# ecker-lab/TreeLearn

Hardware: AMD Instinct MI355X
Metric: Mpoints/sec through sparse U-Net fwd (0.1 m voxel, 40x40 m tile) (higher is better)
Workload: dtype bf16; 1 GPU; config2: single 40x40 m tile, voxel 0.1 m, 1890607 points/tile, 7-level 32-ch sparse U-Net fwd (30.1 M params, random init), 1 tile per GPU; points_per_tile=1890607, tiles_in_flight=4

## Files before the change

include/treelearn_hip.h:

```cpp
#ifndef TREELEARN_HIP_H
#define TREELEARN_HIP_H

#include <stdint.h>

#ifdef __cplusplus
extern "C" {
#endif

typedef void* tl_stream_t;

enum {
  TL_OK = 0,
  TL_ERR_ARG = -1,
  TL_ERR_LAUNCH = -2,
  TL_ERR_UNSUPPORTED = -3
};

enum { TL_F32 = 0, TL_BF16 = 1, TL_F16 = 2 };

int tl_version(void);
int tl_set_tuning(const char* key, int64_t value);
const char* tl_error_string(int code);


int tl_voxel_point_coords(const float* xyz, const int64_t* batch_ids, int64_t N, int B, float voxel_size,
                          uint32_t* ws_minmax, int32_t* pcoords, int32_t* maxc, tl_stream_t stream);

#define TL_POINT_COORDS_MAX_PARTS 1024
int tl_voxel_point_coords_one(const float* xyz, const int64_t* batch_ids, int64_t N, float voxel_size, uint32_t* ws, int32_t* pcoords,
                              int32_t* maxc_parts, int* n_parts, tl_stream_t stream);
int tl_bitmap_from_points(const int32_t* pcoords, int64_t N, const int32_t dims[4], uint64_t* bitmap, tl_stream_t stream);

int tl_bitmap_down(const uint64_t* fine, const int32_t fdims[4], const int32_t out_shape[3],
                   uint64_t* coarse, const int32_t cdims[4], tl_stream_t stream);

int64_t tl_scan_ws_words(int64_t nwords);
int tl_bitmap_scan(const uint64_t* bitmap, int64_t nwords, uint32_t* prefix, uint32_t* total, uint32_t* ws, tl_stream_t stream);

int tl_expand_coords(const uint64_t* bitmap, const uint32_t* prefix, const int32_t dims[4], int32_t* coords, tl_stream_t stream);

int tl_point_rank(const int32_t* pcoords, int64_t N, const uint64_t* bitmap, const uint32_t* prefix,
                  const int32_t dims[4], int64_t* v2p, tl_stream_t stream);

int tl_voxel_mean_feats(const float* pf, int C, const int64_t* v2p, int64_t N, int64_t M, int P,
                        int32_t* ws, float* out, tl_stream_t stream);
int tl_voxel_feats(const float* xyz, const float* feats, int F, const int64_t* v2p, int64_t N, int64_t M, int P, int use_coords,
                   int use_feats, int dtype, int32_t* ws, void* out, tl_stream_t stream);


int tl_rulebook_subm(const int32_t* coords, int64_t M, const uint64_t* bitmap, const uint32_t* prefix,
                     const int32_t dims[4], int32_t* nbr, int32_t* compact ,
                     tl_stream_t stream);

int tl_rulebook_down(const int32_t* ccoords, int64_t Mc, const uint64_t* fbitmap, const uint32_t* fprefix,
                     const int32_t fdims[4], int64_t Mf, int32_t* child, int32_t* parent, int32_t* inv, tl_stream_t stream);

int64_t tl_pyramid_ws_words(const int32_t dims0[4], int num_levels, int64_t* level_word_offsets);
int tl_pyramid_build(const int32_t* pcoords, int64_t N, const int32_t dims0[4], const int32_t shape0[3], int num_levels,
                     uint64_t* bitmaps, uint32_t* prefixes, uint32_t* counts, uint32_t* ws, tl_stream_t stream);

typedef struct tl_level {
  int32_t dims[4];
  int64_t n;
  const uint64_t* bitmap;
  const uint32_t* prefix;
  int32_t* coords;
  int32_t* nbr;
  int32_t* compact;
  int32_t* child;
  int32_t* parent;
  int32_t* inv;
  const int32_t* o2n;
  int32_t* inv_packed;
} tl_level;

int tl_rulebooks_build(const tl_level* levels, int num_levels, int32_t* minus_one, int64_t minus_one_words,
                       const int32_t* pcoords, int64_t N, int64_t* v2p, tl_stream_t stream);

#define TL_BLK_HALO_MAX 126
typedef struct tl_blk {
  int32_t* o2n; int32_t* perm; int32_t* coords_new;
  int32_t* unit; int32_t* counter; int32_t* halo; uint32_t* lrb; int32_t* pmask;
  int64_t cap_units;
  int32_t halo_max;
  int32_t reserved;
  int32_t* nn;
} tl_blk;
int64_t tl_blk_ws_words(const int32_t dims[4]);
int tl_blk_build(const uint64_t* bitmap, const uint32_t* prefix, const int32_t dims[4], int64_t n, const tl_blk* out, uint32_t* ws,
                 int phases, tl_stream_t stream);

int tl_rulebook_compact(const int32_t* table, int64_t n, int32_t* compact, tl_stream_t stream);

typedef struct tl_conv_args {
  const void* in;        int64_t in_ld;
  const void* weight;
  const int32_t* table;
  int64_t n_out;         int64_t n_in;
  int32_t K;             int32_t Cin;     int32_t Cout;   int32_t dtype;
  const float* in_scale; const float* in_shift;  int32_t in_relu;  int32_t out_relu;
  const void* residual;  int64_t res_ld;
  const float* out_scale; const float* out_shift;
  void* out;             int64_t out_ld;
  void* out2; int64_t out2_ld; const float* out2_scale; const float* out2_shift; int32_t out2_relu;
  void* out3; int64_t out3_ld; const float* out3_scale; const float* out3_shift; int32_t out3_relu;
  const void* weight_frag;
  int32_t table_one_hot;
  const int32_t* table_compact;
  int32_t in_all_ones;
  int32_t epi_mode;
  double* red_part;
  int32_t* red_nparts;
  const void* bn_x;      int64_t bn_x_ld;
  const float* bn_mean;  const float* bn_rstd;  const float* bn_scale;  const float* bn_shift;  int32_t bn_relu;
  const int32_t* blk_unit; const int32_t* blk_counter; const int32_t* blk_halo; const uint32_t* blk_lrb; const int32_t* blk_pmask;
  const int32_t* table_scatter;
  const void* weight_x3;
} tl_conv_args;

#define TL_EPI_NONE 0
#define TL_EPI_STATS 1
#define TL_EPI_BN_BWD 2
int64_t tl_conv_red_parts(int64_t n_out);

int tl_conv_fwd(const tl_conv_args* args, tl_stream_t stream);
int tl_conv_route(const tl_conv_args* args, char* buf, int cap);

int tl_pack_weight(const float* w_ref, int Cout, int K, int Cin, void* w_packed, int dtype, tl_stream_t stream);
int64_t tl_pack_weight_x3_bytes(int Cout, int K, int Cin);
int tl_pack_weight_x3(const float* w_ref, int Cout, int K, int Cin, void* w_x3, tl_stream_t stream);
int tl_pack_weight_dgrad(const float* w_ref, int Cout, int K, int Cin, int flip, void* w_t, int dtype, tl_stream_t stream);
typedef struct tl_pack_desc {
  const float* src;
  void* dst;
  int32_t Cout, K, Cin, form;
} tl_pack_desc;
int tl_pack_weights_batch(const tl_pack_desc* descs, const int32_t* blocks, int64_t n_blocks, int dtype, tl_stream_t stream);
int tl_pack_weight_frag(const float* w_ref, int Cout, int K, int Cin, void* w_frag, int dtype, tl_stream_t stream);

int64_t tl_conv_wgrad_ws_floats(int64_t n_out, int K, int Cin, int Cout);
int tl_conv_wgrad(const void* x, int64_t x_ld, const void* gout, int64_t g_ld, int dtype, const int32_t* table, int64_t n_out,
                  int64_t n_in, int K, int Cin, int Cout, float* gw, float* ws, tl_stream_t stream);
int tl_conv_wgrad_ref(const void* x, int64_t x_ld, const void* gout, int64_t g_ld, int dtype, const int32_t* table, int64_t n_out,
                      int64_t n_in, int K, int Cin, int Cout, float* gw, float* ws, tl_stream_t stream);

int64_t tl_conv_wgrad_blk_ws_floats(void);
int tl_conv_wgrad_blk(const void* x, int64_t x_ld, const void* gout, int64_t g_ld, int dtype, const int32_t* blk_unit, const int32_t* blk_counter,
                      const int32_t* blk_halo, const uint32_t* blk_lrb, int64_t n, int Cin, int Cout, float* gw, int ref_layout, float* ws,
                      tl_stream_t stream);

int tl_head_mlp(const void* feats, int64_t feats_ld, int dtype, int C, const int64_t* v2p, int64_t N,
                const float* pro_scale, const float* pro_shift,
                const float* w1, const float* b1, const float* w2, const float* b2,
                float* backbone, float* logits, float* offsets, tl_stream_t stream);

int tl_affine_relu(const void* in, int64_t in_ld, void* out, int64_t out_ld, int64_t n, int C, int dtype,
                   const float* scale, const float* shift, int relu, tl_stream_t stream);

int64_t tl_bn_ws_doubles(int64_t n, int C);
int tl_bn_train_stats(const void* x, int64_t ld, int64_t n, int C, int dtype, const float* gamma, const float* beta, float eps,
                      float momentum, double* ws, float* mean, float* rstd, float* scale, float* shift, float* running_mean,
                      float* running_var, int64_t* num_batches_tracked, tl_stream_t stream);
int tl_bn_train_bwd(const void* x, int64_t ld, int x_dtype, const void* dy, int64_t dld, int dy_dtype, int64_t n, int C,
                    const float* mean, const float* rstd, const float* scale, const float* shift, int relu, double* ws,
                    float* dgamma, float* dbeta, void* dx, int64_t xld, const void* dx_add, int64_t dx_add_ld, tl_stream_t stream);

int tl_bn_train_finish(const double* part, int64_t nparts, int64_t n, int C, const float* gamma, const float* beta, float eps, float momentum, float* mean,
                       float* rstd, float* scale, float* shift, float* running_mean, float* running_var, int64_t* num_batches_tracked, tl_stream_t stream);
int tl_bn_train_bwd_from_parts(const void* x, int64_t ld, int x_dtype, const void* g, int64_t gld, int g_dtype, int64_t n, int C, const float* mean,
                               const float* rstd, const float* scale, const float* shift, const double* part, int64_t nparts, float* dgamma, float* dbeta,
                               void* dx, int64_t xld, const void* dx_add, int64_t dx_add_ld, tl_stream_t stream);

int tl_linear_small_f32(const void* x, int64_t x_ld, int dtype, const void* w, int Cin, int Cout, int64_t n, float* out, int64_t out_ld,
                        tl_stream_t stream);

int tl_gather_rows(const void* in, int64_t in_ld, int dtype, int C, int64_t n_rows, const int64_t* idx, int64_t N, void* out, int64_t out_ld, tl_stream_t stream);
int tl_scatter_add_rows(const void* g, int64_t g_ld, int dtype, int C, const int64_t* order, const int64_t* sorted_idx, int64_t N, int64_t n_rows, void* gin,
                        int64_t gin_ld, tl_stream_t stream);

// ... 289 lines not shown
```

treelearn_amd/_hip.py:

```python
import ctypes
import os

import torch

_HERE = os.path.dirname(os.path.abspath(__file__))
LIB_PATH = os.path.join(_HERE, "lib", "libtreelearn_hip.so")

TL_F32, TL_BF16, TL_F16 = 0, 1, 2
TL_OK, TL_ERR_ARG, TL_ERR_UNSUPPORTED = 0, -1, -3
TL_EPI_NONE, TL_EPI_STATS, TL_EPI_BN_BWD = 0, 1, 2
_c = ctypes
_vp, _i64, _i32, _f32 = _c.c_void_p, _c.c_int64, _c.c_int32, _c.c_float


class ConvArgs(_c.Structure):
    _fields_ = [
        ("in_", _vp), ("in_ld", _i64), ("weight", _vp), ("table", _vp),
        ("n_out", _i64), ("n_in", _i64), ("K", _i32), ("Cin", _i32), ("Cout", _i32), ("dtype", _i32),
        ("in_scale", _vp), ("in_shift", _vp), ("in_relu", _i32), ("out_relu", _i32),
        ("residual", _vp), ("res_ld", _i64), ("out_scale", _vp), ("out_shift", _vp),
        ("out", _vp), ("out_ld", _i64),
        ("out2", _vp), ("out2_ld", _i64), ("out2_scale", _vp), ("out2_shift", _vp), ("out2_relu", _i32),
        ("out3", _vp), ("out3_ld", _i64), ("out3_scale", _vp), ("out3_shift", _vp), ("out3_relu", _i32),
        ("weight_frag", _vp), ("table_one_hot", _i32), ("table_compact", _vp),
# ... 63 lines not shown


class StemParams(_c.Structure):
    _fields_ = [(k, _c.c_double) for k in ("first_height", "step", "thickness", "corridor", "start_radius", "search_factor", "search_margin",
                                           "max_rmse", "min_radius", "max_radius", "max_growth", "dbh_height")] + \
               [(k, _i64) for k in ("max_slices", "min_points", "max_misses")]


class CrownParams(_c.Structure):
    _fields_ = [(k, _c.c_double) for k in ("layer", "cell", "min_height")] + [(k, _i64) for k in ("max_layers", "base_percent", "max_gap")]


class SkeletonParams(_c.Structure):
    _fields_ = [(k, _c.c_double) for k in ("voxel", "min_branch", "min_height")] + \
               [(k, _i64) for k in ("reach", "base_reach", "base_layers", "level", "max_voxels")]


class WoodParams(_c.Structure):
    _fields_ = [(k, _c.c_double) for k in ("max_rmse", "min_radius", "max_radius", "max_growth", "dbh_height")] + [("min_points", _i64)]


class LeafwoodParams(_c.Structure):
    _fields_ = [(k, _c.c_double) for k in ("radius", "linearity_min", "planarity_min", "verticality_min", "voxel")] + \
               [(k, _i64) for k in ("min_neighbours", "vote_iters", "vote_percent", "reach", "min_component", "filter")]


_I4 = _i32 * 4
_I3 = _i32 * 3

PROTOTYPES = {
    "tl_version": (_i32, []),
    "tl_error_string": (_c.c_char_p, [_i32]),
    "tl_set_tuning": (_i32, [_c.c_char_p, _i64]),
    "tl_voxel_point_coords": (_i32, [_vp, _vp, _i64, _i32, _f32, _vp, _vp, _vp, _vp]),
    "tl_voxel_point_coords_one": (_i32, [_vp, _vp, _i64, _f32, _vp, _vp, _vp, _c.POINTER(_i32), _vp]),
    "tl_bitmap_from_points": (_i32, [_vp, _i64, _I4, _vp, _vp]),
    "tl_bitmap_down": (_i32, [_vp, _I4, _I3, _vp, _I4, _vp]),
    "tl_scan_ws_words": (_i64, [_i64]),
    "tl_bitmap_scan": (_i32, [_vp, _i64, _vp, _vp, _vp, _vp]),
    "tl_expand_coords": (_i32, [_vp, _vp, _I4, _vp, _vp]),
    "tl_point_rank": (_i32, [_vp, _i64, _vp, _vp, _I4, _vp, _vp]),
    "tl_voxel_mean_feats": (_i32, [_vp, _i32, _vp, _i64, _i64, _i32, _vp, _vp, _vp]),
    "tl_voxel_feats": (_i32, [_vp, _vp, _i32, _vp, _i64, _i64, _i32, _i32, _i32, _i32, _vp, _vp, _vp]),
    "tl_rulebook_subm": (_i32, [_vp, _i64, _vp, _vp, _I4, _vp, _vp, _vp]),
    "tl_rulebook_down": (_i32, [_vp, _i64, _vp, _vp, _I4, _i64, _vp, _vp, _vp, _vp]),
    "tl_rulebook_compact": (_i32, [_vp, _i64, _vp, _vp]),
    "tl_pyramid_ws_words": (_i64, [_I4, _i32, _c.POINTER(_i64)]),
    "tl_pyramid_build": (_i32, [_vp, _i64, _I4, _I3, _i32, _vp, _vp, _vp, _vp, _vp]),
    "tl_rulebooks_build": (_i32, [_c.POINTER(Level), _i32, _vp, _i64, _vp, _i64, _vp, _vp]),
    "tl_blk_ws_words": (_i64, [_I4]),
    "tl_blk_build": (_i32, [_vp, _vp, _I4, _i64, _c.POINTER(Blk), _vp, _i32, _vp]),
    "tl_conv_fwd": (_i32, [_c.POINTER(ConvArgs), _vp]),
    "tl_conv_route": (_i32, [_c.POINTER(ConvArgs), _c.c_char_p, _i32]),
    "tl_conv_red_parts": (_i64, [_i64]),
    "tl_exec_create": (_vp, []),
    "tl_exec_destroy": (None, [_vp]),
    "tl_forward": (_i32, [_vp, _c.POINTER(NetDesc), _c.POINTER(ForwardArgs), _vp]),
    "tl_exec_check": (_i32, [_vp]),
    "tl_exec_profile": (_i32, [_vp, _i32]),
    "tl_exec_profile_read": (_i32, [_vp, _c.POINTER(LaunchRec), _i32]),
    "tl_bn_train_finish": (_i32, [_vp, _i64, _i64, _i32, _vp, _vp, _f32, _f32, _vp, _vp, _vp, _vp, _vp, _vp, _vp, _vp]),
    "tl_bn_train_bwd_from_parts": (_i32, [_vp, _i64, _i32, _vp, _i64, _i32, _i64, _i32, _vp, _vp, _vp, _vp, _vp, _i64, _vp, _vp, _vp, _i64, _vp, _i64, _vp]),
    "tl_pack_weight": (_i32, [_vp, _i32, _i32, _i32, _vp, _i32, _vp]),
    "tl_pack_weight_x3": (_i32, [_vp, _i32, _i32, _i32, _vp, _vp]),
    "tl_pack_weight_x3_bytes": (_i64, [_i32, _i32, _i32]),
    "tl_pack_weight_frag": (_i32, [_vp, _i32, _i32, _i32, _vp, _i32, _vp]),
    "tl_pack_weights_batch": (_i32, [_vp, _vp, _i64, _i32, _vp]),
    "tl_pack_weight_dgrad": (_i32, [_vp, _i32, _i32, _i32, _i32, _vp, _i32, _vp]),
    "tl_conv_wgrad_ws_floats": (_i64, [_i64, _i32, _i32, _i32]),
    "tl_conv_wgrad": (_i32, [_vp, _i64, _vp, _i64, _i32, _vp, _i64, _i64, _i32, _i32, _i32, _vp, _vp, _vp]),
    "tl_conv_wgrad_ref": (_i32, [_vp, _i64, _vp, _i64, _i32, _vp, _i64, _i64, _i32, _i32, _i32, _vp, _vp, _vp]),
    "tl_conv_wgrad_blk_ws_floats": (_i64, []),
    "tl_conv_wgrad_blk": (_i32, [_vp, _i64, _vp, _i64, _i32, _vp, _vp, _vp, _vp, _i64, _i32, _i32, _vp, _i32, _vp, _vp]),
    "tl_head_mlp": (_i32, [_vp, _i64, _i32, _i32, _vp, _i64, _vp, _vp, _vp, _vp, _vp, _vp, _vp, _vp, _vp, _vp]),
    "tl_affine_relu": (_i32, [_vp, _i64, _vp, _i64, _i64, _i32, _i32, _vp, _vp, _i32, _vp]),
    "tl_bn_ws_doubles": (_i64, [_i64, _i32]),
    "tl_bn_train_stats": (_i32, [_vp, _i64, _i64, _i32, _i32, _vp, _vp, _f32, _f32, _vp, _vp, _vp, _vp, _vp, _vp, _vp, _vp, _vp]),
    "tl_bn_train_bwd": (_i32, [_vp, _i64, _i32, _vp, _i64, _i32, _i64, _i32, _vp, _vp, _vp, _vp, _i32, _vp, _vp, _vp, _vp, _i64, _vp, _i64, _vp]),
    "tl_linear_small_f32": (_i32, [_vp, _i64, _i32, _vp, _i32, _i32, _i64, _vp, _i64, _vp]),
    "tl_gather_rows": (_i32, [_vp, _i64, _i32, _i32, _i64, _vp, _i64, _vp, _i64, _vp]),
    "tl_scatter_add_rows": (_i32, [_vp, _i64, _i32, _i32, _vp, _vp, _i64, _i64, _vp, _i64, _vp]),
    "tl_compact_ws_words": (_i64, [_i64]),
    "tl_compact_rows": (_i32, [_vp, _i32, _vp, _i64, _vp, _vp, _vp, _vp]),
    "tl_tile_crop_ws_words": (_i64, [_i64]),
    "tl_tile_crop": (_i32, [_vp, _vp, _vp, _i64, _i32, _vp, _vp, _vp, _vp, _vp, _vp, _vp, _vp, _vp, _vp]),
    "tl_cell_keys": (_i32, [_vp, _i64, _c.c_double, _c.c_double, _vp, _i32, _vp, _vp, _vp]),
    "tl_downsample_ws_words": (_i64, [_i64]),
    "tl_downsample_reduce": (_i32, [_vp, _vp, _vp, _i64, _vp, _vp, _vp, _vp, _vp, _vp]),
    "tl_downsample_reduce_r64": (_i32, [_vp, _vp, _vp, _i64, _vp, _vp, _vp, _vp, _vp, _vp]),
    "tl_group_mean": (_i32, [_vp, _i64, _i32, _vp, _vp, _vp, _vp, _vp, _vp, _vp]),
    "tl_verticality": (_i32, [_vp, _vp, _i64, _c.c_double, _vp, _vp, _vp]),
    "tl_eigen_features": (_i32, [_vp, _vp, _i64, _c.c_double, _vp, _vp, _i64, _vp, _i32, _vp, _vp]),
    "tl_eigen_features_scales": (_i32, [_vp, _vp, _i64, _vp, _i32, _vp, _vp, _i64, _vp, _i32, _vp, _vp]),
    "tl_cluster_ws_bytes": (_i64, [_i64]),
    "tl_cluster_grid": (_i32, [_vp, _i64, _c.c_double, _vp, _vp, _vp, _vp]),
    "tl_hdbscan_ws_bytes": (_i64, [_i64]),
    "tl_hdbscan_mst": (_i32, [_vp, _i64, _i32, _vp, _vp, _vp, _vp, _vp, _vp]),
    "tl_hdbscan_labels_host": (_i32, [_vp, _vp, _vp, _i64, _i32, _vp]),
    "tl_hdbscan_prim_order_host": (_i32, [_vp, _vp, _vp, _i64, _vp, _vp, _vp]),
    "tl_hdbscan_grid_plan_ws_bytes": (_i64, []),
    "tl_hdbscan_grid_plan": (_i32, [_vp, _i64, _vp, _vp, _vp]),
    "tl_hdbscan_grid_ws_bytes": (_i64, [_i64, _vp]),
    "tl_hdbscan_grid_ws_bytes_k": (_i64, [_i64, _vp, _i32]),
    "tl_hdbscan_mst_grid": (_i32, [_vp, _i64, _i32, _vp, _vp, _vp, _vp, _vp, _vp, _vp]),
    "tl_knn_vote": (_i32, [_vp, _vp, _i64, _vp, _i64, _i32, _vp, _vp]),
    "tl_knn_vote_grid": (_i32, [_vp, _vp, _vp, _i64, _vp, _vp, _i64, _c.c_float * 3, _f32, _I3, _vp, _i64, _i32, _vp, _vp]),
# ... 129 lines not shown
```

treelearn_amd/csrc/tl_blk.hip:

```cpp
#include "tl_common.h"

namespace {

constexpr int kBlock = 256;
constexpr int HASH = 2048;
constexpr uint32_t EMPTY = 0xFFFFFFFFu;
constexpr uint32_t KEYMASK = 0x01FFFFFFu;
constexpr int LIST = 128;

struct BlkGrid { int B, BX, BY, BZ, TX, TY; int64_t nblk; };

__device__ __forceinline__ void blk_decode(const BlkGrid& g, int64_t blk, int& b, int& bx, int& by, int& bz) {
  bz = (int)(blk % g.BZ); blk /= g.BZ;
  const int iy = (int)(blk & 3), ix = (int)((blk >> 2) & 3); blk >>= 4;
  const int ty = (int)(blk % g.TY); blk /= g.TY;
  const int tx = (int)(blk % g.TX);
  b = (int)(blk / g.TX);
  bx = tx * 4 + ix; by = ty * 4 + iy;
}

__device__ __forceinline__ uint32_t wg_exclusive_scan(uint32_t v, uint32_t* total) {
  __shared__ uint32_t wsum[kBlock / 64];
  const int lane = threadIdx.x & 63, wid = threadIdx.x >> 6;
  uint32_t inc = v;
// ... 59 lines not shown
  __syncthreads();
  uint32_t base = 0, tot = 0;
  for (int w = 0; w < 16; ++w) { if (w < wid) base += wsum[w]; tot += wsum[w]; }
  uint32_t run = base + inc - s;
  for (int64_t i = lo; i < hi; ++i) { const uint32_t v = in[i]; out[i] = run; run += v; }
  if (tid == 0 && total) *total = tot;
}

__global__ void __launch_bounds__(kBlock) k_blk_order(const uint64_t* __restrict__ bm, const uint32_t* __restrict__ pf, TlDims d, BlkGrid g,
                                                      const uint32_t* __restrict__ cnt, const uint32_t* __restrict__ bstart,
                                                      int32_t* __restrict__ o2n, int32_t* __restrict__ perm, int32_t* __restrict__ coords_new,
                                                      uint32_t* __restrict__ cs) {
  const int lane = threadIdx.x & 63;
  const int64_t blk = (int64_t)blockIdx.x * (kBlock / 64) + (threadIdx.x >> 6);
  if (blk >= g.nblk) return;
  if (cnt[blk] == 0) return;
  int b, bx, by, bz;
  blk_decode(g, blk, b, bx, by, bz);
  const int x = bx * 8 + (lane >> 3), y = by * 8 + (lane & 7);
  const bool valid = x < d.X && y < d.Y;
  const int sh = (bz & 7) * 8;
  uint64_t word = 0; int64_t w = 0;
  if (valid) { w = tl_col_word(d, b, x, y) + (bz >> 3); word = bm[w]; }
  uint32_t byte = (uint32_t)(word >> sh) & 0xFFu;
  const uint32_t pc = __popc(byte);
  uint32_t inc = pc;
  for (int off = 1; off < 64; off <<= 1) {
    const uint32_t t = (uint32_t)__shfl_up((int)inc, off);
    if (lane >= off) inc += t;
  }
  if (!pc) return;
  int newr = (int)(bstart[blk] + inc - pc);
  int old = (int)(pf[w] + __popcll(word & ((1ull << sh) - 1ull)));
  cs[(((int64_t)b * d.X + x) * d.Y + y) * g.BZ + bz] = (uint32_t)newr;
  while (byte) {
    const int zb = __ffs((int)byte) - 1;
    byte &= byte - 1;
    o2n[old] = newr; perm[newr] = old;
    reinterpret_cast<int4*>(coords_new)[newr] = make_int4(b, x, y, bz * 8 + zb);
    ++old; ++newr;
  }
}

struct BlkOut {
  const uint32_t* cs; int BZ;
  const int32_t* coords_new;
  int32_t* unit; int32_t* counter;
  int32_t* halo; uint32_t* lrb; int32_t* pmask; int32_t* nn_out;
  int64_t n; int64_t nchunks; int64_t cap_units; int halo_max;
};

__global__ void __launch_bounds__(kBlock) k_blk_units(const uint64_t* __restrict__ bm, TlDims d, BlkOut p) {
  __shared__ uint32_t s_tab[kBlock / 64][HASH + 64];
  __shared__ uint32_t s_list[kBlock / 64][LIST];
  __shared__ uint32_t s_lslot[kBlock / 64][LIST];
  const int lane = threadIdx.x & 63, wv = threadIdx.x >> 6;
  const int64_t chunk = (int64_t)blockIdx.x * (kBlock / 64) + wv;
  if (chunk >= p.nchunks) return;
  uint32_t* tab = s_tab[wv];
  uint32_t* list = s_list[wv];
  uint32_t* lslot = s_lslot[wv];
  const int64_t base = chunk * 64;
  const int cnt = (int)(p.n - base < 64 ? p.n - base : 64);
  const int64_t r = base + lane;
  const bool rvalid = lane < cnt;

  int nn[27];
#pragma unroll
  for (int k = 0; k < 27; ++k) nn[k] = -1;
  uint32_t pm = 0;
  {
    const int4 c = rvalid ? reinterpret_cast<const int4*>(p.coords_new)[r] : make_int4(0, 0, 0, 0);
    const int z = c.w;
    const bool hz0 = z > 0, hz2 = z + 1 < d.Z;
    const int bA = (hz0 ? z - 1 : z) >> 3, bB = (hz2 ? z + 1 : z) >> 3;
    const bool x0 = hz0 && ((z - 1) >> 6) != (z >> 6), x2 = hz2 && ((z + 1) >> 6) != (z >> 6);
    const int64_t wc0 = rvalid ? tl_col_word(d, c.x, c.y, c.z) : 0;
    const int64_t ci0 = rvalid ? (((int64_t)c.x * d.X + c.y) * d.Y + c.z) * p.BZ : 0;
    const bool xin[3] = {rvalid && c.y > 0, rvalid, rvalid && c.y + 1 < d.X}, yin[3] = {c.z > 0, true, c.z + 1 < d.Y};
    const int zw1 = rvalid ? (z >> 6) : 0, zw0 = (rvalid && x0) ? ((z - 1) >> 6) : zw1, zw2 = (rvalid && x2) ? ((z + 1) >> 6) : zw1;
    bool inb[9];
    uint64_t w1[9];
#pragma unroll
    for (int q = 0; q < 9; ++q) {
      const int dx = q / 3 - 1, dy = q % 3 - 1;
      inb[q] = xin[q / 3] && yin[q % 3];
      w1[q] = bm[wc0 + (inb[q] ? (dx * d.Y + dy) * d.Zw : 0) + zw1];
    }
    uint32_t by3[9];
#pragma unroll
    for (int q = 0; q < 9; ++q) {
      const uint32_t b1 = (uint32_t)(w1[q] >> (z & 56)) & 0xFFu;
      const uint32_t b0 = (uint32_t)(w1[q] >> ((hz0 ? z - 1 : z) & 56)) & 0xFFu, b2 = (uint32_t)(w1[q] >> ((hz2 ? z + 1 : z) & 56)) & 0xFFu;
      by3[q] = b0 | (b1 << 8) | (b2 << 16);
    }
    if (__any(x0 || x2)) {
#pragma unroll
      for (int q = 0; q < 9; ++q) {
        const int dx = q / 3 - 1, dy = q % 3 - 1;
        const int64_t wcq = wc0 + (inb[q] ? (dx * d.Y + dy) * d.Zw : 0);
        const uint64_t a0 = bm[wcq + zw0], a2 = bm[wcq + zw2];
        if (x0) by3[q] = (by3[q] & ~0xFFu) | ((uint32_t)(a0 >> ((z - 1) & 56)) & 0xFFu);
        if (x2) by3[q] = (by3[q] & ~0xFF0000u) | (((uint32_t)(a2 >> ((z + 1) & 56)) & 0xFFu) << 16);
      }
    }
    bool p0[9], p1[9], p2[9];
    uint32_t sA[9], sB[9];
#pragma unroll
    for (int q = 0; q < 9; ++q) {
      const int dx = q / 3 - 1, dy = q % 3 - 1;
      p0[q] = inb[q] && hz0 && ((by3[q] >> ((z - 1) & 7)) & 1u);
      p1[q] = inb[q] && ((by3[q] >> (8 + (z & 7))) & 1u);
      p2[q] = inb[q] && hz2 && ((by3[q] >> (16 + ((z + 1) & 7))) & 1u);
      const bool any = p0[q] || p1[q] || p2[q];
      const int64_t ciq = ci0 + (inb[q] ? (dx * d.Y + dy) * p.BZ : 0);
      sA[q] = p.cs[any ? ciq + bA : 0];
      sB[q] = p.cs[(any && bB != bA) ? ciq + bB : 0];
    }
    auto rowid = [](uint32_t byte, int zz, uint32_t start) __attribute__((always_inline)) {
      return (int)(start + __popc(byte & ((1u << (zz & 7)) - 1u)));
    };
#pragma unroll
    for (int q = 0; q < 9; ++q) {
      const uint32_t b_ = bB != bA ? sB[q] : sA[q];
      if (p0[q]) { nn[3 * q] = rowid(by3[q] & 0xFFu, z - 1, sA[q]); pm |= 1u << (3 * q); }
      if (p1[q]) { nn[3 * q + 1] = rowid((by3[q] >> 8) & 0xFFu, z, (z >> 3) == bA ? sA[q] : b_); pm |= 2u << (3 * q); }
      if (p2[q]) { nn[3 * q + 2] = rowid((by3[q] >> 16) & 0xFFu, z + 1, b_); pm |= 4u << (3 * q); }
    }
    if (rvalid) {
      p.pmask[r] = (int32_t)pm;
      if (p.nn_out) {
#pragma unroll
        for (int k = 0; k < 27; ++k) p.nn_out[(int64_t)k * p.n + r] = nn[k];
      }
    }
  }

  int nref = __popc(pm);
  for (int off = 32; off > 0; off >>= 1) nref += __shfl_xor(nref, off);
  const int TS = nref <= 360 ? 512 : (nref <= 720 ? 1024 : HASH);
  const int tshift = nref <= 360 ? 23 : (nref <= 720 ? 22 : 21);
  auto hs = [&](int v) __attribute__((always_inline)) { return ((uint32_t)v * 2654435761u) >> tshift; };

  int st_a[8], st_e[8];
  int sp = 1;
  st_a[0] = 0; st_e[0] = cnt;
  bool first = true;
  while (sp > 0) {
    --sp;
    const int a = st_a[sp], e = st_e[sp];
    const int lo = (int)base + a, hi = (int)base + e;
    for (int i = lane; i < TS; i += 64) tab[i] = EMPTY;
    __builtin_amdgcn_fence(__ATOMIC_ACQ_REL, "workgroup");
    const bool inr = lane >= a && lane < e;
    uint32_t outm = 0;
#pragma unroll
    for (int k = 0; k < 27; ++k) {
      const int v = nn[k];
      const bool out = inr && v >= 0 && (v < lo || v >= hi);
      outm |= out ? (1u << k) : 0u;
      tab[out ? hs(v) : (uint32_t)TS] = (uint32_t)v;
    }
    __builtin_amdgcn_fence(__ATOMIC_ACQ_REL, "workgroup");
    uint32_t lost = 0;
#pragma unroll
    for (int k = 0; k < 27; ++k) {
      const uint32_t cur = tab[hs(nn[k])];
      lost |= (((outm >> k) & 1u) && cur != (uint32_t)nn[k]) ? (1u << k) : 0u;
    }
    if (__any(lost != 0)) {
#pragma unroll
      for (int k = 0; k < 27; ++k) {
        bool todo = (lost >> k) & 1u;
        if (__any(todo)) {
          uint32_t s_ = hs(nn[k]);
          while (__any(todo)) {
            if (todo) {
              s_ = (s_ + 1) & (uint32_t)(TS - 1);
              if (tab[s_] == EMPTY) tab[s_] = (uint32_t)nn[k];
            }
            __builtin_amdgcn_fence(__ATOMIC_ACQ_REL, "workgroup");
            if (todo && tab[s_] == (uint32_t)nn[k]) todo = false;
            __builtin_amdgcn_fence(__ATOMIC_ACQ_REL, "workgroup");
          }
        }
      }
    }
    int H = 0;
    for (int i0 = 0; i0 < TS; i0 += 512) {
      uint32_t sv[8];
#pragma unroll
      for (int q = 0; q < 8; ++q) sv[q] = tab[i0 + q * 64 + lane];
#pragma unroll
      for (int q = 0; q < 8; ++q) {
        const unsigned long long m = __ballot(sv[q] != EMPTY);
        if (sv[q] != EMPTY) {
          const int at = H + __popcll(m & ((1ull << lane) - 1ull));
          if (at < LIST) { list[at] = sv[q]; lslot[at] = (uint32_t)(i0 + q * 64 + lane); }
        }
        H += __popcll(m);
      }
    }
    if (H > p.halo_max && e - a > 1) {
      const int mid = a + (e - a) / 2;
      st_a[sp] = mid; st_e[sp] = e; ++sp;
      st_a[sp] = a; st_e[sp] = mid; ++sp;
      continue;
    }
    int u;
    if (first) u = (int)chunk;
    else {
      int t = 0;
      if (lane == 0) t = atomicAdd(p.counter, 1);
      u = __shfl(t, 0);
    }
    first = false;
    if (u >= p.cap_units || H > LIST - 2) {
      if (lane == 0) atomicMax(p.counter + 1, 1);
      continue;
    }
    __builtin_amdgcn_fence(__ATOMIC_ACQ_REL, "workgroup");
    {
      const uint32_t k0 = lane < H ? list[lane] : EMPTY, s0 = lane < H ? lslot[lane] : (uint32_t)TS;
      int r0 = 0;
      const int H16 = (H + 15) & ~15;
      if (H <= 64) {
        for (int i = 0; i < H; ++i) r0 += (uint32_t)__builtin_amdgcn_readlane((int)k0, i) < k0 ? 1 : 0;
        if (lane < H) p.halo[(int64_t)lo * 32 + r0] = (int32_t)k0;
        tab[s0] = k0 | ((uint32_t)r0 << 25);
        if (lane >= H && lane < H16) p.halo[(int64_t)lo * 32 + lane] = -1;
      } else {
        const uint32_t k1 = lane + 64 < H ? list[lane + 64] : EMPTY, s1 = lane + 64 < H ? lslot[lane + 64] : (uint32_t)TS;
        int r1 = 0;
        for (int i = 0; i < 64; ++i) {
          const uint32_t b = (uint32_t)__builtin_amdgcn_readlane((int)k0, i);
          r0 += b < k0 ? 1 : 0; r1 += b < k1 ? 1 : 0;
        }
        for (int i = 64; i < H; ++i) {
          const uint32_t b = (uint32_t)__builtin_amdgcn_readlane((int)k1, i - 64);
          r0 += b < k0 ? 1 : 0; r1 += b < k1 ? 1 : 0;
        }
        p.halo[(int64_t)lo * 32 + r0] = (int32_t)k0;
        tab[s0] = k0 | ((uint32_t)r0 << 25);
        if (lane + 64 < H) p.halo[(int64_t)lo * 32 + r1] = (int32_t)k1;
        tab[s1] = k1 | ((uint32_t)r1 << 25);
        if (lane + 64 >= H && lane + 64 < H16) p.halo[(int64_t)lo * 32 + lane + 64] = -1;
      }
    }
    __builtin_amdgcn_fence(__ATOMIC_ACQ_REL, "workgroup");
    {
      uint32_t wds[9];
#pragma unroll
      for (int q = 0; q < 9; ++q) wds[q] = 0;
      uint32_t miss = 0;
      uint32_t cur[27];
#pragma unroll
      for (int k = 0; k < 27; ++k) cur[k] = tab[hs(nn[k])];
#pragma unroll
      for (int k = 0; k < 27; ++k) miss |= (((outm >> k) & 1u) && (cur[k] & KEYMASK) != (uint32_t)nn[k]) ? (1u << k) : 0u;
      if (__any(miss != 0)) {
#pragma unroll
        for (int k = 0; k < 27; ++k) {
          bool todo = (miss >> k) & 1u;
          if (__any(todo)) {
            uint32_t s_ = hs(nn[k]);
            while (__any(todo)) {
              if (todo) {
                s_ = (s_ + 1) & (uint32_t)(TS - 1);
                const uint32_t c_ = tab[s_];
                if ((c_ & KEYMASK) == (uint32_t)nn[k]) { cur[k] = c_; todo = false; }
              }
            }
          }
        }
      }
#pragma unroll
      for (int k = 0; k < 27; ++k) {
        const int v = nn[k];
        const bool out = (outm >> k) & 1u;
        const int pos = out ? 64 + (int)(cur[k] >> 25) : ((inr && v >= 0) ? v - lo : 191);
        const uint32_t val = (uint32_t)(pos * 4 + ((pos >> 2) & 3));
        wds[k / 3] |= val << ((k % 3) * 10);
      }
      if (inr) {
        uint32_t* dst = p.lrb + r * 9;
#pragma unroll
        for (int q = 0; q < 9; ++q) dst[q] = wds[q];
      }
    }
    if (lane == 0) reinterpret_cast<int4*>(p.unit)[u] = make_int4(lo, e - a, H, 0);
    __builtin_amdgcn_fence(__ATOMIC_ACQ_REL, "workgroup");
  }
}

__global__ void __launch_bounds__(kBlock) k_blk_tail_rank(int32_t* __restrict__ unit, const int32_t* __restrict__ counter, int nchunks, int64_t cap_units) {
  __shared__ int keys[kBlock];
  const int m = counter[0] - nchunks;
  if (m <= 1 || (int64_t)nchunks + 2 * (int64_t)m > cap_units) return;
  const int4* u = reinterpret_cast<const int4*>(unit) + nchunks;
  int4* tmp = reinterpret_cast<int4*>(unit) + (cap_units - m);
  for (int t0 = blockIdx.x * kBlock; t0 < m; t0 += gridDim.x * kBlock) {
    const int t = t0 + threadIdx.x;
    const int4 me = t < m ? u[t] : make_int4(0, 0, 0, 0);
    int rank = 0;
    for (int j0 = 0; j0 < m; j0 += kBlock) {
      keys[threadIdx.x] = j0 + (int)threadIdx.x < m ? u[j0 + threadIdx.x].x : 0x7FFFFFFF;
      __syncthreads();
      const int lim = m - j0 < kBlock ? m - j0 : kBlock;
      for (int j = 0; j < lim; ++j) rank += keys[j] < me.x ? 1 : 0;
      __syncthreads();
    }
    if (t < m) tmp[rank] = me;
  }
}
__global__ void __launch_bounds__(kBlock) k_blk_tail_copy(int32_t* __restrict__ unit, const int32_t* __restrict__ counter, int nchunks, int64_t cap_units) {
  const int m = counter[0] - nchunks;
  if (m <= 1 || (int64_t)nchunks + 2 * (int64_t)m > cap_units) return;
  const int4* tmp = reinterpret_cast<const int4*>(unit) + (cap_units - m);
  for (int t = blockIdx.x * kBlock + threadIdx.x; t < m; t += gridDim.x * kBlock) reinterpret_cast<int4*>(unit)[nchunks + t] = tmp[t];
}

__global__ void k_blk_init(int32_t* counter, int32_t nchunks) {
  if (threadIdx.x == 0) { counter[0] = nchunks; counter[1] = 0; }
}

}

extern "C" {

int64_t tl_blk_ws_words(const int32_t dims[4]) {
  if (!dims) return -1;
  const int64_t nblk = (int64_t)dims[0] * ((dims[1] + 31) / 32) * ((dims[2] + 31) / 32) * 16 * ((dims[3] + 7) / 8);
  const int64_t ncb = (int64_t)dims[0] * dims[1] * dims[2] * ((dims[3] + 7) / 8);
  return 2 * nblk + 2 * ((nblk + 255) / 256) + 8 + ncb;
}

int tl_blk_build(const uint64_t* bitmap, const uint32_t* prefix, const int32_t dims[4], int64_t n, const tl_blk* o, uint32_t* ws,
                 int phases, tl_stream_t stream) {
  if (!bitmap || !prefix || !dims || !o || !ws || n <= 0 || n >= (1 << 25) || !(phases & 3)) return TL_ERR_ARG;
  if (!o->o2n || !o->perm || !o->coords_new || !o->unit || !o->counter || !o->halo || !o->lrb || !o->pmask) return TL_ERR_ARG;
  if (o->halo_max < 26 || o->halo_max > TL_BLK_HALO_MAX || o->cap_units < (n + 63) / 64) return TL_ERR_ARG;
  if (((uintptr_t)o->unit) % 16 || ((uintptr_t)o->coords_new) % 16) return TL_ERR_ARG;
  const TlDims d = tl_dims(dims);
  BlkGrid g;
// ... 30 lines not shown
```

treelearn_amd/csrc/tl_common.h:

```cpp
#pragma once
#include <hip/hip_runtime.h>
#include <stdint.h>
#include <atomic>
#include <typeinfo>
#include "../../include/treelearn_hip.h"

#define TL_CHECK_LAUNCH()                                   \
  do {                                                      \
    if (hipGetLastError() != hipSuccess) return TL_ERR_LAUNCH; \
  } while (0)

static inline hipStream_t tl_s(tl_stream_t s) { return reinterpret_cast<hipStream_t>(s); }

struct TlAttrOnce {
  std::atomic<uint64_t> done[4];
};
static inline bool tl_lds_attr(TlAttrOnce& once, const void* kernel, int bytes) {
  int dev = 0;
  if (hipGetDevice(&dev) != hipSuccess) return false;
  std::atomic<uint64_t>& w = once.done[(dev >> 6) & 3];
  const uint64_t bit = 1ull << (dev & 63);
  if (w.load(std::memory_order_acquire) & bit) return true;
  if (hipFuncSetAttribute(kernel, hipFuncAttributeMaxDynamicSharedMemorySize, bytes) != hipSuccess) return false;
  w.fetch_or(bit, std::memory_order_release);
  return true;
}

struct TlRoute;
extern thread_local TlRoute* tl_route_armed;
template <auto Kernel> struct TlKernelTag {};
int tl_route_record(TlRoute* r, const char* tag, bool f16, dim3 grid, dim3 block, size_t lds);
#ifdef TL_F16_BUILD
constexpr bool kTlF16Build = true;
#else
constexpr bool kTlF16Build = false;
#endif

template <auto Kernel, class... A>
int tl_launch(dim3 grid, dim3 block, size_t lds, hipStream_t s, A... args) {
  if (TlRoute* r = tl_route_armed) return tl_route_record(r, typeid(TlKernelTag<Kernel>).name(), kTlF16Build, grid, block, lds);
  Kernel<<<grid, block, lds, s>>>(args...);
  return hipGetLastError() == hipSuccess ? TL_OK : TL_ERR_LAUNCH;
}
template <auto Kernel, class... A>
int tl_launch_lds(dim3 grid, dim3 block, size_t lds, hipStream_t s, A... args) {
  if (TlRoute* r = tl_route_armed) return tl_route_record(r, typeid(TlKernelTag<Kernel>).name(), kTlF16Build, grid, block, lds);
  static TlAttrOnce attr_once;
  if (!tl_lds_attr(attr_once, reinterpret_cast<const void*>(Kernel), 160 * 1024)) return TL_ERR_LAUNCH;
  Kernel<<<grid, block, lds, s>>>(args...);
  return hipGetLastError() == hipSuccess ? TL_OK : TL_ERR_LAUNCH;
}

static inline int64_t tl_cdiv(int64_t a, int64_t b) { return (a + b - 1) / b; }

static inline unsigned tl_grid(int64_t work_items, int block) {
  int64_t g = tl_cdiv(work_items, block);
  if (g < 1) g = 1;
  if (g > 256 * 16) g = 256 * 16;
  return (unsigned)g;
}

struct TlDims {
  int B, X, Y, Z, Zw;
};
static inline TlDims tl_dims(const int32_t d[4]) {
  TlDims r{d[0], d[1], d[2], d[3], (d[3] + 63) >> 6};
  return r;
}
__host__ __device__ static inline int64_t tl_nwords(const TlDims& d) { return (int64_t)d.B * d.X * d.Y * d.Zw; }

__device__ __forceinline__ int64_t tl_col_word(const TlDims& d, int b, int x, int y) {
  return (((int64_t)b * d.X + x) * d.Y + y) * d.Zw;
}

__device__ __forceinline__ int tl_rank_at(const uint64_t* __restrict__ bm, const uint32_t* __restrict__ pf,
                                          int64_t wc, int z) {
  const int64_t w = wc + (z >> 6);
  const uint64_t word = bm[w];
  const uint64_t bit = 1ull << (z & 63);
  if (!(word & bit)) return -1;
  return (int)(pf[w] + __popcll(word & (bit - 1)));
}

bool tl_conv_one_hot_direct_enabled(int64_t n_out);
// ... 1 lines not shown
```

treelearn_amd/csrc/tl_conv.hip:

```cpp
#include "tl_conv_internal.h"
#include <cxxabi.h>
#include <stdio.h>
#include <stdlib.h>
#include <string.h>

struct TlRoute {
  char text[1024] = "";
  int len = 0;
  bool truncated = false;
};
thread_local TlRoute* tl_route_armed = nullptr;

int tl_route_record(TlRoute* r, const char* tag, bool f16, dim3 grid, dim3 block, size_t lds) {
  int status = 0;
  char* full = abi::__cxa_demangle(tag, nullptr, nullptr, &status);
  struct Free { char* p; ~Free() { free(p); } } guard{full};
  const char* b = (status == 0 && full) ? strstr(full, "&(") : nullptr;
  b = b ? b + 2 : tag;
  const char* e = b;
  for (int depth = 0; *e; ++e) {
    if (!strncmp(e, "(anonymous namespace)", 21)) { e += 20; continue; }
    if (depth == 0 && (*e == ' ' || *e == ':')) b = e + 1;
    if (depth == 0 && *e == '(') break;
    depth += (*e == '<') - (*e == '>');
    if (depth == 0 && *e == '>') { ++e; break; }
  }
  char dims[2][40];
  const dim3 d[2] = {grid, block};
  for (int i = 0; i < 2; ++i) {
    if (d[i].y == 1 && d[i].z == 1) snprintf(dims[i], sizeof dims[i], "%u", d[i].x);
    else snprintf(dims[i], sizeof dims[i], "(%u, %u, %u)", d[i].x, d[i].y, d[i].z);
  }
  const int room = (int)sizeof r->text - r->len;
  const int n = snprintf(r->text + r->len, (size_t)room, "%s%.*s%s<<<%s, %s, %zu>>>", r->len ? " + " : "", (int)(e - b), b, f16 ? "/f16" : "", dims[0], dims[1], lds);
  if (n < 0 || n >= room) { r->truncated = true; r->text[r->len] = 0; return TL_OK; }
  r->len += n;
  return TL_OK;
}

static int64_t g_small_rows = 16384;
extern int g_small_mode;
extern int g_wgrad_dense;
extern int64_t g_wgrad_dense_min_rows;
extern int g_wgrad_rows;
extern int g_wgrad_dma;
static int g_stream = 1;
static int g_streamq = 1;
static int g_streamq_x3 = 1;
static int g_direct = 1;
static int g_direct_oh = 1;
static int g_blk = 1;
static int g_up = 1;

bool tl_conv_one_hot_direct_enabled(int64_t n_out) { return g_direct && g_direct_oh && n_out > g_small_rows; }

namespace {

struct ConvAlign {
  bool in16, in8;
  bool w16, w4;
  bool in_ld8, in_ld4;
  bool out_vec;
  bool in_aff16;
  bool out_aff16, out_aff4;
  bool res_ld8, res_ld4;
  bool vec_ok() const { return in_ld8 && in16 && w16; }
  bool aligned() const { return in_ld4 && in16 && w16 && in_aff16; }
};

bool ptr_al(const void* p, unsigned bytes) { return ((uintptr_t)p) % bytes == 0; }

ConvAlign conv_align(const tl_conv_args* a) {
  ConvAlign c;
  c.in16 = ptr_al(a->in, 16); c.in8 = ptr_al(a->in, 8);
  c.w16 = ptr_al(a->weight, 16); c.w4 = ptr_al(a->weight, 4);
  c.in_ld8 = a->in_ld % 8 == 0; c.in_ld4 = a->in_ld % 4 == 0;
  c.out_vec = a->out_ld % 8 == 0 && ptr_al(a->out, 16) && (!a->out2 || (a->out2_ld % 8 == 0 && ptr_al(a->out2, 16))) && (!a->out3 || (a->out3_ld % 8 == 0 && ptr_al(a->out3, 16)));
  c.in_aff16 = !a->in_scale || (ptr_al(a->in_scale, 16) && ptr_al(a->in_shift, 16));
  c.out_aff16 = !a->out_scale || (ptr_al(a->out_scale, 16) && ptr_al(a->out_shift, 16));
  c.out_aff4 = !a->out_scale || (ptr_al(a->out_scale, 4) && ptr_al(a->out_shift, 4));
  c.res_ld8 = !a->residual || (a->res_ld % 8 == 0 && ptr_al(a->residual, 16));
  c.res_ld4 = !a->residual || (a->res_ld % 4 == 0 && ptr_al(a->residual, 16));
  return c;
}

struct Conv {
  const tl_conv_args* a;
  ConvP p;
  ConvAlign al;
  const TlConvH16* L;
  int dt;
  bool f16, train, has_blk;
  hipStream_t s;
  bool mult32() const { return a->Cin % 32 == 0 && a->Cout % 32 == 0; }
  bool no_prologue() const { return !a->in_scale && !a->in_relu; }
};

constexpr int TL_NEXT = 1;
int or_next(int rc) { return rc == TL_ERR_UNSUPPORTED ? TL_NEXT : rc; }

int validate(const tl_conv_args* a, bool has_blk) {
  if (!a->table && a->K != 1 && !has_blk && !(a->in_all_ones && a->blk_pmask)) return TL_ERR_ARG;
  if ((a->in_scale == nullptr) != (a->in_shift == nullptr)) return TL_ERR_ARG;
  if ((a->out_scale == nullptr) != (a->out_shift == nullptr)) return TL_ERR_ARG;
  if (a->dtype != TL_F32 && a->dtype != TL_BF16 && a->dtype != TL_F16) return TL_ERR_ARG;
  if ((a->out2_scale == nullptr) != (a->out2_shift == nullptr) || (a->out3_scale == nullptr) != (a->out3_shift == nullptr)) return TL_ERR_ARG;
  if (a->epi_mode != TL_EPI_NONE) {
    if ((a->epi_mode != TL_EPI_STATS && a->epi_mode != TL_EPI_BN_BWD) || !a->red_part || ((uintptr_t)a->red_part) % 8) return TL_ERR_ARG;
    if (a->epi_mode == TL_EPI_BN_BWD) {
      if (!a->bn_x || !a->bn_mean || !a->bn_rstd || !a->bn_scale || !a->bn_shift) return TL_ERR_ARG;
      if (a->bn_x_ld % 8 || !ptr_al(a->bn_x, 16) || !ptr_al(a->bn_mean, 16) || !ptr_al(a->bn_rstd, 16) || !ptr_al(a->bn_scale, 16) || !ptr_al(a->bn_shift, 16)) return TL_ERR_UNSUPPORTED;
    }
  }
  return TL_OK;
}

ConvP fill_convp(const tl_conv_args* a, bool has_blk) {
  ConvP p;
  p.in = a->in; p.in_ld = a->in_ld; p.w = a->weight; p.w_frag = a->weight_frag;
  p.w_x3 = (a->dtype == TL_F32 && a->Cin % 32 == 0 && ptr_al(a->weight_x3, 16)) ? a->weight_x3 : nullptr;
  p.table = a->table; p.ctab = (a->K == 27) ? a->table_compact : nullptr; p.n_out = a->n_out; p.n_in = a->n_in;
  p.K = a->K; p.Cin = a->Cin; p.Cout = a->Cout; p.in_scale = a->in_scale; p.in_shift = a->in_shift;
  p.in_relu = a->in_relu; p.out_relu = a->out_relu; p.res = a->residual; p.res_ld = a->res_ld;
  p.out_scale = a->out_scale; p.out_shift = a->out_shift; p.out = a->out; p.out_ld = a->out_ld;
  p.out2 = a->out2; p.out2_ld = a->out2_ld; p.out2_scale = a->out2_scale; p.out2_shift = a->out2_shift; p.out2_relu = a->out2_relu;
  p.out3 = a->out3; p.out3_ld = a->out3_ld; p.out3_scale = a->out3_scale; p.out3_shift = a->out3_shift; p.out3_relu = a->out3_relu;
  p.nblk = (int)tl_cdiv(a->n_out, TL_CONV_TILE_ROWS);
  p.one_hot = a->table != nullptr ? a->table_one_hot : 0;
  p.blk_unit = has_blk ? a->blk_unit : nullptr; p.blk_counter = a->blk_counter; p.blk_halo = a->blk_halo; p.blk_lrb = a->blk_lrb;
  p.blk_pmask = a->K == 27 ? a->blk_pmask : nullptr;
  p.epi_mode = a->epi_mode; p.red_part = a->red_part; p.red_nparts = a->red_nparts; p.bn_x = a->bn_x; p.bn_x_ld = a->bn_x_ld;
  p.bn_mean = a->bn_mean; p.bn_rstd = a->bn_rstd; p.bn_scale = a->bn_scale; p.bn_shift = a->bn_shift; p.bn_relu = a->bn_relu;
  return p;
}

int rung_packed_one_hot(Conv& c) {
  if (c.p.one_hot != 2) return TL_NEXT;
  const tl_conv_args* a = c.a;
  const bool shape = a->K == 8 && a->Cin == 64 && a->Cout == 32 && !c.train && c.no_prologue() && g_direct && g_direct_oh;
  if (!shape || !(c.dt == TL_BF16 || (c.dt == TL_F32 && c.p.w_x3))) return TL_ERR_UNSUPPORTED;
  return c.L->direct(c.p, c.dt, c.s);
}

int rung_ones27(Conv& c) {
  const tl_conv_args* a = c.a;
  if (!(a->in_all_ones && !c.train && c.al.out_vec && (g_direct || !a->table) && c.al.w4 && !a->residual)) return TL_NEXT;
  return or_next(c.L->ones27(c.p, c.dt, c.s));
}

int rung_blk(Conv& c) {
  const tl_conv_args* a = c.a;
  if (!(c.has_blk && c.dt == TL_BF16 && g_blk && c.al.vec_ok() && c.al.out_vec && c.al.res_ld8 && c.al.out_aff4 && (!a->in_relu || a->in_scale))) return TL_NEXT;
  return or_next(c.L->blk(c.p, c.s));
}

int rung_blk_x3(Conv& c) {
  if (!(c.has_blk && c.a->dtype == TL_F32 && c.p.w_x3 && g_blk && !c.train)) return TL_NEXT;
  return or_next(tl_launch_conv_blk_x3(c.p, c.s));
}

int rung_needs_table(Conv& c) { return (!c.a->table && c.a->K != 1) ? TL_ERR_UNSUPPORTED : TL_NEXT; }

int rung_up(Conv& c) {
  const tl_conv_args* a = c.a;
  if (!(a->table_scatter && c.p.one_hot && g_up && !c.train && c.dt == TL_BF16 && c.al.vec_ok() && c.al.out_vec && c.al.out_aff16)) return TL_NEXT;
  return or_next(c.L->up(c.p, a->table_scatter, c.s));
}

int rung_in4(Conv& c) {
  const tl_conv_args* a = c.a;
  if (!(c.dt == TL_BF16 && a->Cin == 4 && a->Cout == 32 && g_direct && c.al.out_vec && c.al.in8 && c.al.w16 && c.al.res_ld8)) return TL_NEXT;
  return or_next(c.L->direct(c.p, TL_BF16, c.s));
}

int rung_tinycin(Conv& c) {
  const tl_conv_args* a = c.a;
  if (!(!c.train && a->Cin <= 8 && a->Cout % 8 == 0 && a->Cout <= 64 && c.no_prologue() && c.al.out_vec)) return TL_NEXT;
  return c.L->tinycin(c.p, c.dt, c.s);
}

int rung_small(Conv& c) {
  if (!c.train && c.al.vec_ok() && c.a->n_out <= g_small_rows && c.mult32()) return c.L->small(c.p, c.dt, c.s);
  if (c.train && c.a->n_out <= g_small_rows) return TL_ERR_UNSUPPORTED;
  return TL_NEXT;
}

int rung_wide_x3_split(Conv& c) {
  const tl_conv_args* a = c.a;
  if (!(c.p.w_x3 && a->Cin >= 256)) return TL_NEXT;
  const ConvP p = c.p;
  c.p.w_x3 = nullptr;
  if (!(c.dt == TL_F32 && !c.train && g_stream && c.al.aligned() && c.al.out_vec && a->Cin % 64 == 0 && a->Cout % 32 == 0 && c.no_prologue() && !a->residual &&
        !a->out2 && !a->out3 && a->n_out > g_small_rows && c.al.out_aff16))
    return TL_NEXT;
  ConvP p1 = p;
  p1.Cin = a->Cin / 2; p1.out_scale = nullptr; p1.out_shift = nullptr; p1.out_relu = 0;
  const int rc1 = c.L->stream(p1, TL_F32, c.s);
  if (rc1 != TL_OK) return or_next(rc1);
  ConvP p2 = p;
  p2.Cin = a->Cin / 2; p2.in = static_cast<const float*>(a->in) + a->Cin / 2;
  p2.w_x3 = static_cast<const char*>(p.w_x3) + (size_t)a->K * a->Cout * (a->Cin / 2) * 4;
  p2.res = a->out; p2.res_ld = a->out_ld;
  return c.L->stream(p2, TL_F32, c.s);
}

bool f32_vec(const Conv& c) { return c.dt == TL_F32 && c.al.aligned() && c.al.out_vec && c.mult32() && c.no_prologue() && c.al.res_ld4 && c.al.out_aff16; }
int rung_f32_direct(Conv& c) { return f32_vec(c) && g_direct ? or_next(c.L->direct(c.p, TL_F32, c.s)) : TL_NEXT; }
int rung_f32_streamq_x3(Conv& c) {
  if (!(f32_vec(c) && g_stream && g_streamq && g_streamq_x3 && c.p.w_x3 && !c.train && c.a->n_out > g_small_rows)) return TL_NEXT;
  return or_next(tl_launch_conv_streamq_x3(c.p, c.s));
}
int rung_f32_stream(Conv& c) { return f32_vec(c) && g_stream ? or_next(c.L->stream(c.p, TL_F32, c.s)) : TL_NEXT; }

int rung_f32_train_ends(Conv& c) { return (c.train && c.dt == TL_F32) ? TL_ERR_UNSUPPORTED : TL_NEXT; }

int rung_f32_small(Conv& c) {
  if (!(c.dt == TL_F32 && c.al.vec_ok() && c.a->n_out <= 4 * g_small_rows && c.mult32() && c.no_prologue())) return TL_NEXT;
  return c.L->small(c.p, c.dt, c.s);
}

int rung_f32_tile(Conv& c) {
  if (!(c.dt == TL_F32 && c.al.aligned() && c.mult32() && c.a->Cout <= 224)) return TL_NEXT;
  return tl_launch_conv_mfma_f32(c.p, c.s);
}

bool h16_vec(const Conv& c) {
  return c.dt == TL_BF16 && c.al.aligned() && c.al.vec_ok() && c.al.out_vec && c.mult32() && c.a->Cout <= 224 && c.al.res_ld8 && c.al.out_aff16;
}
int rung_h16_one_hot_direct(Conv& c) {
  if (!(h16_vec(c) && c.p.one_hot && g_direct && g_direct_oh && c.a->K == 8 && c.a->Cin == 64 && c.a->Cout == 32)) return TL_NEXT;
  return or_next(c.L->direct(c.p, TL_BF16, c.s));
}
int rung_h16_one_hot_stream(Conv& c) {
  return h16_vec(c) && c.p.one_hot && g_stream && c.a->K == 8 ? or_next(c.L->stream(c.p, TL_BF16, c.s)) : TL_NEXT;
}
int rung_h16_direct(Conv& c) { return h16_vec(c) && g_direct ? or_next(c.L->direct(c.p, TL_BF16, c.s)) : TL_NEXT; }
int rung_h16_streamq(Conv& c) { return h16_vec(c) && g_stream && g_streamq ? or_next(c.L->streamq(c.p, c.s)) : TL_NEXT; }
int rung_h16_stream(Conv& c) { return h16_vec(c) && g_stream ? or_next(c.L->stream(c.p, TL_BF16, c.s)) : TL_NEXT; }
int rung_h16_tile(Conv& c) {
  if (!h16_vec(c)) return TL_NEXT;
  return c.train ? TL_ERR_UNSUPPORTED : c.L->bf16(c.p, c.s);
}

int rung_scalar_only(Conv& c) { return (c.train || c.f16) ? TL_ERR_UNSUPPORTED : TL_NEXT; }
int rung_tinycout(Conv& c) { return or_next(tl_launch_conv_tinycout(c.p, c.dt, c.s)); }
int rung_generic(Conv& c) { return tl_launch_conv_generic(c.p, c.dt, c.s); }

constexpr int (*kLadder[])(Conv&) = {
    rung_packed_one_hot, rung_ones27, rung_blk, rung_blk_x3, rung_needs_table, rung_up, rung_in4, rung_tinycin, rung_small, rung_wide_x3_split,
    rung_f32_direct, rung_f32_streamq_x3, rung_f32_stream, rung_f32_train_ends, rung_f32_small, rung_f32_tile,
    rung_h16_one_hot_direct, rung_h16_one_hot_stream, rung_h16_direct, rung_h16_streamq, rung_h16_stream, rung_h16_tile,
    rung_scalar_only, rung_tinycout, rung_generic,
};

}

extern "C" {

int tl_set_tuning(const char* key, int64_t value) {
  if (!key) return TL_ERR_ARG;
  if (!strcmp(key, "direct")) { g_direct = (int)value; return TL_OK; }
  if (!strcmp(key, "blk")) { g_blk = (int)value; return TL_OK; }
  if (!strcmp(key, "up")) { g_up = (int)value; return TL_OK; }
  if (!strcmp(key, "direct_oh")) { g_direct_oh = (int)value; return TL_OK; }
  if (!strcmp(key, "stream")) { g_stream = (int)value; return TL_OK; }
  if (!strcmp(key, "streamq")) { g_streamq = (int)value; return TL_OK; }
  if (!strcmp(key, "streamq_x3")) { if (value != 0 && value != 1) return TL_ERR_ARG; g_streamq_x3 = (int)value; return TL_OK; }
  if (!strcmp(key, "small_rows")) { g_small_rows = value; return TL_OK; }
  if (!strcmp(key, "small_mode")) { g_small_mode = (int)value; return TL_OK; }
  if (!strcmp(key, "wgrad_dense")) { g_wgrad_dense = (int)value; return TL_OK; }
  if (!strcmp(key, "wgrad_rows")) { g_wgrad_rows = (int)value; return TL_OK; }
  if (!strcmp(key, "wgrad_dma")) { g_wgrad_dma = (int)value; return TL_OK; }
  if (!strcmp(key, "wgrad_dense_min_rows")) { g_wgrad_dense_min_rows = value; return TL_OK; }
  return TL_ERR_ARG;
}

int tl_conv_fwd(const tl_conv_args* a, tl_stream_t stream) {
  if (!a || !a->in || !a->weight || !a->out || a->n_out <= 0 || a->K <= 0 || a->K > 27 || a->Cin <= 0 || a->Cout <= 0) return TL_ERR_ARG;
  const bool has_blk = a->blk_unit && a->blk_counter && a->blk_halo && a->blk_lrb && a->K == 27;
  const int bad = validate(a, has_blk);
  if (bad != TL_OK) return bad;
  Conv c;
  c.a = a; c.p = fill_convp(a, has_blk); c.al = conv_align(a); c.has_blk = has_blk; c.s = tl_s(stream);
  c.f16 = a->dtype == TL_F16;
  c.dt = c.f16 ? TL_BF16 : a->dtype;
  c.L = c.f16 ? &kTlConvF16 : &kTlConvBf16;
  c.train = a->epi_mode != TL_EPI_NONE;
  if (c.train && a->red_nparts) *a->red_nparts = 0;
  for (auto rung : kLadder) {
    const int rc = rung(c);
    if (rc != TL_NEXT) return rc;
  }
  return TL_ERR_UNSUPPORTED;
}

int tl_conv_route(const tl_conv_args* a, char* buf, int cap) {
  if (!buf || cap <= 0) return TL_ERR_ARG;
  TlRoute r;
  struct Armed {
    explicit Armed(TlRoute* q) { tl_route_armed = q; }
    ~Armed() { tl_route_armed = nullptr; }
  } armed(&r);
  const int rc = tl_conv_fwd(a, nullptr);
  snprintf(buf, (size_t)cap, "%s", r.text);
  return (r.truncated || r.len >= cap) ? TL_ERR_ARG : rc;
}

int64_t tl_conv_red_parts(int64_t n_out) {
  const int64_t a = tl_cdiv(n_out > 0 ? n_out : 1, 256);
  return a > 2048 ? a : 2048;
}

}
```

treelearn_amd/csrc/tl_conv_blk.hip:

```cpp
#include "tl_conv_internal.h"
#include <atomic>

namespace {

typedef __attribute__((address_space(3))) void* lds_ptr;
static __device__ __forceinline__ u32x4 lds_r128(unsigned a) { u32x4 v; asm volatile("ds_read_b128 %0, %1" : "=v"(v) : "v"(a)); return v; }
#define TL_LGKM(N) asm volatile("s_waitcnt lgkmcnt(%0)" ::"n"(N) : "memory")
#define TL_KEEP(x) asm volatile("" : "+v"(x))
typedef int i32x4 __attribute__((ext_vector_type(4)));
static __device__ __forceinline__ i32x4 s_load4(const void* ptr) { i32x4 v; asm volatile("s_load_dwordx4 %0, %1, 0x0" : "=s"(v) : "s"(ptr)); return v; }
#define TL_SWAIT(d) asm volatile("s_waitcnt lgkmcnt(0)" : "+s"(d) : : "memory")

constexpr int WS_B = 27 * 32 * 64;
constexpr int AFF_B = 4 * 2 * 32 * 4;
constexpr int STAGE_B = 192 * 64;
constexpr int HCH = 8;
struct RbRow { u32x4 a, b; uint32_t c; };
static __device__ __forceinline__ uint32_t rb_word(const RbRow& r, int w) { return w < 4 ? r.a[w] : (w < 8 ? r.b[w - 4] : r.c); }

typedef float f32x2 __attribute__((ext_vector_type(2)));
typedef short s16x2 __attribute__((ext_vector_type(2)));

template <int W, bool RES, int NV, bool TR = false, bool PRO = false>
__global__ void __launch_bounds__(W * 64) k_conv_blk(ConvP p) {
// ... 319 lines not shown
          sc[q] = __uint_as_float(s0[q]); sc[q + 4] = __uint_as_float(s1[q]);
          sh[q] = __uint_as_float(h0[q]); sh[q + 4] = __uint_as_float(h1[q]);
        }
      }
#pragma unroll
      for (int it = 0; it < 4; ++it) {
        float z[8];
#pragma unroll
        for (int q = 0; q < 8; ++q) z[q] = y[it][q];
        if (aff_on[v]) {
#pragma unroll
          for (int q = 0; q < 8; ++q) z[q] = fmaf(z[q], sc[q], sh[q]);
        }
        if (relu_on[v]) {
#pragma unroll
          for (int q = 0; q < 8; ++q) z[q] = fmaxf(z[q], 0.f);
        }
        const u32x4 o = {pack_bf16x2(z[0], z[1]), pack_bf16x2(z[2], z[3]), pack_bf16x2(z[4], z[5]), pack_bf16x2(z[6], z[7])};
        const int rr_ = (lane >> 2) + 16 * it;
        const unsigned off = rr_ < nown ? (unsigned)(row0 + rr_) * o_ldb[v] + (unsigned)((lane & 3) * 16) : 0xFFFFFFFFu;
        __builtin_amdgcn_raw_buffer_store_b128(__builtin_bit_cast(__attribute__((__vector_size__(4 * sizeof(unsigned)))) unsigned, o), ro[v], (int)off, 0, 0);
      }
    }
    }
    dc = d1; d1 = d2; d2 = desc_fin(d3r, u + 3 * nw);
  }
  if constexpr (TR) {
    double* Ds = reinterpret_cast<double*>(smem + WS_B + AFF_B + W * STAGE_B);
    double d0[8], d1_[8];
#pragma unroll
    for (int q = 0; q < 8; ++q) { d0[q] = (double)ts0[q]; d1_[q] = (double)ts1[q]; }
#pragma unroll
    for (int off = 4; off < 64; off <<= 1)
#pragma unroll
      for (int q = 0; q < 8; ++q) { d0[q] += __shfl_xor(d0[q], off, 64); d1_[q] += __shfl_xor(d1_[q], off, 64); }
    if (lane < 4) {
#pragma unroll
      for (int q = 0; q < 8; ++q) { Ds[(wv * 2 + 0) * 32 + lane * 8 + q] = d0[q]; Ds[(wv * 2 + 1) * 32 + lane * 8 + q] = d1_[q]; }
    }
    __syncthreads();
    if (tid < 64) {
      double t = 0.0;
      for (int w = 0; w < W; ++w) t += Ds[(w * 2 + (tid >> 5)) * 32 + (tid & 31)];
      p.red_part[(int64_t)blockIdx.x * 64 + tid] = t;
    }
  }
}

template <int W, bool RES, int NV, bool TR = false, bool PRO = false>
int launch_blk(const ConvP& p, hipStream_t s) {
  constexpr size_t lds = (size_t)WS_B + AFF_B + (size_t)W * STAGE_B + (TR ? (size_t)W * 2 * 32 * 8 : 0);
  static_assert(lds <= 160 * 1024, "LDS budget");
  if (TR && p.red_nparts) *p.red_nparts = 256;
  return tl_launch_lds<k_conv_blk<W, RES, NV, TR, PRO>>(256, W * 64, lds, s, p);
}

}

int TL_H16(tl_launch_conv_blk)(const ConvP& p, hipStream_t s) {
  if (!p.blk_unit || !p.blk_counter || !p.blk_halo || !p.blk_lrb) return TL_ERR_UNSUPPORTED;
  if (p.K != 27 || p.Cin != 32 || p.Cout != 32 || p.n_in != p.n_out) return TL_ERR_UNSUPPORTED;
  const bool pro = p.in_scale || p.in_relu;
  if (p.n_out >= (1 << 25)) return TL_ERR_UNSUPPORTED;
  auto big = [&](int64_t ld) { return (p.n_out - 1) * ld * 2 + 64 >= 0x7FFFFFFFll * 2; };
  if (big(p.in_ld) || big(p.out_ld) || (p.out2 && big(p.out2_ld)) || (p.out3 && big(p.out3_ld)) || (p.res && big(p.res_ld))) return TL_ERR_UNSUPPORTED;
  if (p.out3 && !p.out2) return TL_ERR_UNSUPPORTED;
  if (p.epi_mode != TL_EPI_NONE) {
    if (p.out2 || p.out_scale || p.out_relu || p.out_ld % 8 || ((uintptr_t)p.out) % 16) return TL_ERR_UNSUPPORTED;
    if (pro && p.epi_mode != TL_EPI_STATS) return TL_ERR_UNSUPPORTED;
    return pro ? launch_blk<8, false, 1, true, true>(p, s) : launch_blk<8, false, 1, true>(p, s);
  }
  const int nv = p.out3 ? 3 : p.out2 ? 2 : 1;
  if (pro) {
    if (nv != 1) return TL_ERR_UNSUPPORTED;
    return p.res ? launch_blk<8, true, 1, false, true>(p, s) : launch_blk<8, false, 1, false, true>(p, s);
  }
  if (p.res) {
    switch (nv) {
      case 1: return launch_blk<8, true, 1>(p, s);
      case 2: return launch_blk<8, true, 2>(p, s);
      default: return launch_blk<8, true, 3>(p, s);
    }
  }
  switch (nv) {
    case 1: return launch_blk<8, false, 1>(p, s);
    case 2: return launch_blk<8, false, 2>(p, s);
    default: return launch_blk<8, false, 3>(p, s);
  }
}
```

treelearn_amd/csrc/tl_conv_blk_x3.hip:

```cpp
#include "tl_conv_internal.h"
#include <atomic>

namespace {

typedef __attribute__((address_space(3))) void* lds_ptr;
static __device__ __forceinline__ u32x4 lds_r128(unsigned a) { u32x4 v; asm volatile("ds_read_b128 %0, %1" : "=v"(v) : "v"(a)); return v; }
#define TL_LGKM(N) asm volatile("s_waitcnt lgkmcnt(%0)" ::"n"(N) : "memory")
#define TL_KEEP(x) asm volatile("" : "+v"(x))
typedef int i32x4 __attribute__((ext_vector_type(4)));
typedef uint32_t u32x2 __attribute__((ext_vector_type(2)));
static __device__ __forceinline__ i32x4 s_load4(const void* ptr) { i32x4 v; asm volatile("s_load_dwordx4 %0, %1, 0x0" : "=s"(v) : "s"(ptr)); return v; }
#define TL_SWAIT(d) asm volatile("s_waitcnt lgkmcnt(0)" : "+s"(d) : : "memory")

constexpr int WS_B = 27 * 32 * 64;
constexpr int AFF_B = 4 * 2 * 32 * 4;
constexpr int STAGE_B = 192 * 64;
constexpr int HCH = 8;
struct RbRow { u32x4 a, b; uint32_t c; };
static __device__ __forceinline__ uint32_t rb_word(const RbRow& r, int w) { return w < 4 ? r.a[w] : (w < 8 ? r.b[w - 4] : r.c); }

struct X3P {
  int slice;
  int part;
  int chunk, nchunks;
// ... 264 lines not shown
    }
    if constexpr (RES) {
#pragma unroll
      for (int it = 0; it < 4; ++it) {
        TL_KEEP(rres[it][0]); TL_KEEP(rres[it][1]);
#pragma unroll
        for (int q = 0; q < 4; ++q) { y[it][q] += __uint_as_float(rres[it][0][q]); y[it][q + 4] += __uint_as_float(rres[it][1][q]); }
      }
    }
    stage_unit(d1, hcur);
#pragma unroll
    for (int v = 0; v < NV; ++v) {
      float sc[8], sh[8];
      if (aff_on[v]) {
        const u32x4 s0 = lds_r128(aff_a + (unsigned)(v * 256)), s1 = lds_r128(aff_a + (unsigned)(v * 256 + 16));
        const u32x4 h0 = lds_r128(aff_a + (unsigned)(v * 256 + 128)), h1 = lds_r128(aff_a + (unsigned)(v * 256 + 144));
        TL_LGKM(0);
#pragma unroll
        for (int q = 0; q < 4; ++q) {
          sc[q] = __uint_as_float(s0[q]); sc[q + 4] = __uint_as_float(s1[q]);
          sh[q] = __uint_as_float(h0[q]); sh[q + 4] = __uint_as_float(h1[q]);
        }
      }
#pragma unroll
      for (int it = 0; it < 4; ++it) {
        float z[8];
#pragma unroll
        for (int q = 0; q < 8; ++q) z[q] = y[it][q];
        if (aff_on[v]) {
#pragma unroll
          for (int q = 0; q < 8; ++q) z[q] = fmaf(z[q], sc[q], sh[q]);
        }
        if (relu_on[v]) {
#pragma unroll
          for (int q = 0; q < 8; ++q) z[q] = fmaxf(z[q], 0.f);
        }
        typedef __attribute__((__vector_size__(4 * sizeof(unsigned)))) unsigned uv4;
        const uv4 o0 = {__float_as_uint(z[0]), __float_as_uint(z[1]), __float_as_uint(z[2]), __float_as_uint(z[3])};
        const uv4 o1 = {__float_as_uint(z[4]), __float_as_uint(z[5]), __float_as_uint(z[6]), __float_as_uint(z[7])};
        const int rr_ = (lane >> 2) + 16 * it;
        const unsigned off = rr_ < nown ? (unsigned)(row0 + rr_) * o_ldb[v] + (unsigned)((lane & 3) * 32) : 0xFFFFFFFFu;
        __builtin_amdgcn_raw_buffer_store_b128(o0, ro[v], (int)off, 0, 0);
        __builtin_amdgcn_raw_buffer_store_b128(o1, ro[v], (int)(off == 0xFFFFFFFFu ? off : off + 16u), 0, 0);
      }
    }
    dc = d1; d1 = d2; d2 = desc_fin(d3r, u + 3 * nw);
  }
}

template <int W, bool RES, int NV>
int launch_x3(const ConvP& p, const X3P& xp, hipStream_t s) {
  constexpr size_t lds = (size_t)WS_B + AFF_B + (size_t)W * STAGE_B;
  static_assert(lds <= 160 * 1024, "LDS budget");
  return tl_launch_lds<k_conv_blk_x3<W, RES, NV>>(256, W * 64, lds, s, p, xp);
}

}

int tl_launch_conv_blk_x3(const ConvP& p, hipStream_t s) {
  if (!p.blk_unit || !p.blk_counter || !p.blk_halo || !p.blk_lrb || !p.w_x3) return TL_ERR_UNSUPPORTED;
  if (p.K != 27 || p.Cin != 32 || p.Cout != 32 || p.n_in != p.n_out || p.epi_mode != TL_EPI_NONE || p.out3) return TL_ERR_UNSUPPORTED;
  if (p.n_out >= (1 << 25)) return TL_ERR_UNSUPPORTED;
  if (p.in_relu && !p.in_scale) return TL_ERR_UNSUPPORTED;
  auto big = [&](int64_t ld) { return (p.n_out - 1) * ld * 4 + 128 >= 0x7FFFFFFFll * 2; };
  if (big(p.in_ld) || big(p.out_ld) || (p.out2 && big(p.out2_ld)) || (p.res && big(p.res_ld))) return TL_ERR_UNSUPPORTED;
  auto al16 = [](const void* q, int64_t ld) { return ((uintptr_t)q) % 16 == 0 && ld % 4 == 0; };
  if (!al16(p.in, p.in_ld) || !al16(p.out, p.out_ld) || (p.out2 && !al16(p.out2, p.out2_ld)) || (p.res && !al16(p.res, p.res_ld)) || ((uintptr_t)p.w_x3) % 16) return TL_ERR_UNSUPPORTED;
  ConvP a = p;
  a.res = nullptr; a.res_ld = 0; a.out_scale = a.out_shift = nullptr; a.out_relu = 0; a.out2 = nullptr; a.out2_scale = a.out2_shift = nullptr; a.out2_relu = 0;
  ConvP b = p;
  b.in = static_cast<const float*>(p.in) + 16;
  if (p.in_scale) { b.in_scale = p.in_scale + 16; b.in_shift = p.in_shift + 16; }
  const int rc = launch_x3<8, false, 1>(a, X3P{0, 0, 0, 1}, s);
  if (rc != TL_OK) return rc;
  const X3P xb{1, 1, 0, 1};
  if (p.res) return p.out2 ? launch_x3<8, true, 2>(b, xb, s) : launch_x3<8, true, 1>(b, xb, s);
  return p.out2 ? launch_x3<8, false, 2>(b, xb, s) : launch_x3<8, false, 1>(b, xb, s);
}
```

treelearn_amd/csrc/tl_conv_direct.hip:

```cpp
#include "tl_conv_internal.h"
#include <atomic>

namespace {


template <bool BF16, int K, int NB, int UN, int G, int WAVES, bool CT = false, bool TR = false, bool OH = false, bool X3 = false>
__global__ void __launch_bounds__(WAVES * 64) k_conv_direct(ConvP p, int ntiles, int walk) {
  static_assert(!X3 || (!BF16 && !TR), "the split-bf16 contraction: fp32 rows, inference");
  constexpr int EB = BF16 ? 2 : 4;
  constexpr int UB = 32 * EB;
  constexpr int NJ = UB / 32;
  constexpr int SLOTS = UB / 16;
  constexpr int COUT = NB * 32;
  constexpr int NG = (K + G - 1) / G;
  constexpr int EP = COUT + 4;
  extern __shared__ __attribute__((aligned(16))) char smem[];
  char* Ws = smem;
  float* Es = reinterpret_cast<float*>(smem + (size_t)K * UN * COUT * UB);
  double* Ds = reinterpret_cast<double*>(smem + (size_t)K * UN * COUT * UB + (size_t)WAVES * 32 * EP * 4);

  const int tid = threadIdx.x, lane = tid & 63, wv = tid >> 6;
  const int fi = lane & 31, fh = lane >> 5;
  auto swz_of = [](int n) { return BF16 ? ((n >> 2) & 3) : ((n >> 1) & 7); };

// ... 368 lines not shown
__global__ void __launch_bounds__(256) k_conv_ones27(ConvP p) {
  __shared__ __attribute__((aligned(16))) float S[27][32];
  for (int e = threadIdx.x; e < 27 * 32; e += 256) {
    float t = 0.f;
    if constexpr (BF16) {
      const uint16_t* w = (const uint16_t*)p.w;
      for (int c = 0; c < p.Cin; ++c) t += bf16_lo((uint32_t)w[(int64_t)e * p.Cin + c]);
    } else {
      const float* w = (const float*)p.w;
      for (int c = 0; c < p.Cin; ++c) t += w[(int64_t)e * p.Cin + c];
    }
    S[e >> 5][e & 31] = t;
  }
  __syncthreads();
  const int32_t* mask = p.blk_pmask ? p.blk_pmask : p.ctab + (int64_t)9 * p.n_out;
  const int64_t total = p.n_out * 4;
  for (int64_t t = (int64_t)blockIdx.x * 256 + threadIdx.x; t < total; t += (int64_t)gridDim.x * 256) {
    const int64_t row = t >> 2; const int c0 = (int)(t & 3) * 8;
    uint32_t m = (uint32_t)mask[row];
    float v[8] = {0.f, 0.f, 0.f, 0.f, 0.f, 0.f, 0.f, 0.f};
    while (m) {
      const int k = __builtin_ctz(m); m &= m - 1;
      const f32x4 a = *reinterpret_cast<const f32x4*>(&S[k][c0]), b = *reinterpret_cast<const f32x4*>(&S[k][c0 + 4]);
#pragma unroll
      for (int q = 0; q < 4; ++q) { v[q] += a[q]; v[q + 4] += b[q]; }
    }
    epi_views8<BF16>(p, row, c0, v);
  }
}

template <bool BF16, int K, int NB, int UN, int G, int WAVES, bool CT = false, bool TR = false, bool OH = false, bool X3 = false>
int launch(const ConvP& p_, hipStream_t s) {
  ConvP p = p_;
  if constexpr (X3) {
    if (p.epi_mode != TL_EPI_NONE) return TL_ERR_UNSUPPORTED;
    p.w = p.w_x3;
  }
  if constexpr (!TR && BF16) {
    if (p.epi_mode != TL_EPI_NONE) return launch<BF16, K, NB, UN, G, WAVES, CT, true, OH>(p, s);
  } else if constexpr (!TR) {
    if (p.epi_mode != TL_EPI_NONE) return TL_ERR_UNSUPPORTED;
  }
  if constexpr (TR && NB >= 3) return TL_ERR_UNSUPPORTED;
  else {
  constexpr int UB = BF16 ? 64 : 128;
  const size_t lds = (size_t)K * UN * NB * 32 * UB + (size_t)WAVES * 32 * (NB * 32 + 4) * 4 + (TR ? (size_t)WAVES * 2 * NB * 32 * 8 : 0);
  if (lds > 160 * 1024) return TL_ERR_UNSUPPORTED;
  const int ntiles = (int)tl_cdiv(p.n_out, 32);
  const int per_cu = (int)((160 * 1024) / lds) < 1 ? 1 : (int)((160 * 1024) / lds);
  int grid = 256 * (per_cu > 2 ? 2 : per_cu);
  const int need = (int)tl_cdiv(ntiles, WAVES);
  if (grid > need) grid = need;
  if (p.red_nparts) *p.red_nparts = grid;
  return tl_launch_lds<k_conv_direct<BF16, K, NB, UN, G, WAVES, CT, TR, OH, X3>>(grid, WAVES * 64, lds, s, p, ntiles, 0);
  }
}

template <bool BF16, int K, int G>
int dispatch(const ConvP& p, hipStream_t s) {
  const int nb = p.Cout / 32, un = p.Cin / 32;
  const size_t wbytes = (size_t)K * p.Cout * p.Cin * (BF16 ? 2 : 4);
  if constexpr (BF16 && K == 27) {
    if (p.ctab && nb == 1 && un == 1) return launch<true, 27, 1, 1, G, 16, true>(p, s);
    if (p.ctab && nb == 1 && un == 2) return launch<true, 27, 1, 2, G, 8, true>(p, s);
  }
  if constexpr (BF16 && K == 8) {
    if (p.one_hot && nb == 1 && un == 2) return launch<true, 8, 1, 2, G, 16, false, false, true>(p, s);
  }
  if constexpr (BF16 && K == 1) {
    if (nb == 2 && un == 4) return launch<true, 1, 2, 4, 1, 16>(p, s);
    if (nb == 3 && un == 6) return launch<true, 1, 3, 6, 1, 8>(p, s);
    if (nb == 4 && un == 8) return launch<true, 1, 4, 8, 1, 8>(p, s);
  }
  if constexpr (!BF16 && K == 1) {
    if (nb == 2 && un == 4 && p.epi_mode == TL_EPI_NONE) {
      if (p.w_x3) return launch<false, 1, 2, 4, 1, 8, false, false, false, true>(p, s);
      return launch<false, 1, 2, 4, 1, 8>(p, s);
    }
  }
  if constexpr (!BF16 && K == 8) {
    if (p.one_hot && p.w_x3 && p.epi_mode == TL_EPI_NONE && nb == 1 && un == 2) return launch<false, 8, 1, 2, G, 12, false, false, true, true>(p, s);
  }
#define TL_D(NB_, UN_)                                                                                               \
  if (nb == NB_ && un == UN_) {                                                                                      \
    if constexpr (BF16) return wbytes <= 64 * 1024 ? launch<true, K, NB_, UN_, G, 16>(p, s) : launch<true, K, NB_, UN_, G, 8>(p, s); \
    else {                                                                                                           \
      if (p.w_x3 && p.epi_mode == TL_EPI_NONE)        \
        return launch<false, K, NB_, UN_, (G > 2 ? 2 : G), (K == 27 && NB_ == 1 && UN_ == 1 ? 11 : 8), false, false, false, true>(p, s);         \
      return launch<false, K, NB_, UN_, (G > 2 ? 2 : G), 8>(p, s);                                                   \
    }                                                                                                                \
  }
  TL_D(1, 1) TL_D(1, 2) TL_D(2, 1) TL_D(2, 2) TL_D(2, 3) TL_D(3, 2) TL_D(1, 3) TL_D(3, 1)
#undef TL_D
  return TL_ERR_UNSUPPORTED;
}

}

int TL_H16(tl_launch_conv_ones27)(const ConvP& p, int dtype, hipStream_t s) {
  if (p.K != 27 || p.Cout != 32 || (!p.ctab && !p.blk_pmask) || p.Cin <= 0 || p.Cin > 64 || p.in_scale || p.in_relu || p.epi_mode != TL_EPI_NONE) return TL_ERR_UNSUPPORTED;
  const unsigned g = tl_grid(p.n_out * 4, 256);
  if (dtype == TL_BF16) return tl_launch<k_conv_ones27<true>>(g, 256, 0, s, p);
  return tl_launch<k_conv_ones27<false>>(g, 256, 0, s, p);
}


int TL_H16(tl_launch_conv_direct)(const ConvP& p, int dtype, hipStream_t s) {
  if (p.in_scale || p.in_relu) return TL_ERR_UNSUPPORTED;
  if (p.one_hot == 2 && !(p.K == 8 && p.Cin == 64 && p.Cout == 32 && p.epi_mode == TL_EPI_NONE && (dtype == TL_BF16 || p.w_x3))) return TL_ERR_UNSUPPORTED;
  const int eb = dtype == TL_BF16 ? 2 : 4;
  if (dtype == TL_BF16 && p.Cin == 4 && p.Cout == 32 && p.K <= 28 && p.table && p.in_ld % 4 == 0 && (int64_t)p.n_in * p.in_ld * 2 < 0xFFFF0000ll) {
    const int ntiles = (int)tl_cdiv(p.n_out, 32);
    int grid = (int)tl_cdiv(ntiles, 8);
    if (grid > 2048) grid = 2048;
    if (p.red_nparts) *p.red_nparts = grid;
    const bool ct = p.ctab && p.K == 27;
    if (p.epi_mode != TL_EPI_NONE) return ct ? tl_launch<k_conv_in4<8, true, true>>(grid, 512, 0, s, p, ntiles) : tl_launch<k_conv_in4<8, false, true>>(grid, 512, 0, s, p, ntiles);
    return ct ? tl_launch<k_conv_in4<8, true>>(grid, 512, 0, s, p, ntiles) : tl_launch<k_conv_in4<8>>(grid, 512, 0, s, p, ntiles);
  }
  if (p.Cin % 32 || p.Cout % 32) return TL_ERR_UNSUPPORTED;
  const int64_t ld_b = p.in_ld * eb, in_bytes = (p.n_in - 1) * ld_b + (int64_t)p.Cin * eb;
  if (!(in_bytes > 0 && in_bytes + 2 * ld_b < 0xFFFFFFFFll)) return TL_ERR_UNSUPPORTED;
  if ((size_t)p.K * p.Cout * p.Cin * eb > 112 * 1024) return TL_ERR_UNSUPPORTED;
  if (dtype == TL_BF16) {
    switch (p.K) {
      case 27: return dispatch<true, 27, 3>(p, s);
      case 8: return dispatch<true, 8, 2>(p, s);
      case 1: return dispatch<true, 1, 1>(p, s);
    }
  } else {
    switch (p.K) {
      case 27: return dispatch<false, 27, 3>(p, s);
      case 8: return dispatch<false, 8, 2>(p, s);
      case 1: return dispatch<false, 1, 1>(p, s);
    }
  }
  return TL_ERR_UNSUPPORTED;
}
```

treelearn_amd/csrc/tl_conv_stream.hip:

```cpp
#include "tl_conv_internal.h"
#include <atomic>

namespace {

constexpr int WAVES = 8;
constexpr int NT = WAVES * 64;

template <bool BF16, int K, int NB, int UN, int RB, bool OH, bool X3>
constexpr int stream_epi_ahead() {
  constexpr bool exact_f32 = !BF16 && !X3;
  constexpr bool f32_64_64 = exact_f32 && K == 27 && NB == 2 && UN == 2, f32_192_96 = exact_f32 && K == 27 && NB == 3 && UN == 6;
  constexpr bool f32_96_64_k8 = exact_f32 && K == 8 && NB == 2 && UN == 3;
  constexpr bool x3_128_128 = X3 && K == 27 && NB == 4 && UN == 4, x3_64_96_k8 = X3 && K == 8 && NB == 3 && UN == 2;
  constexpr bool oh_128_96 = BF16 && OH && K == 8 && NB == 3 && UN == 4;
  if (f32_64_64 || f32_192_96 || f32_96_64_k8 || x3_128_128 || x3_64_96_k8 || oh_128_96) return 0;
  if (NB == 3 && RB == 1) return 1;
  return epi_pd<BF16>(RB * NB);
}

template <bool BF16, int K, int NB, int UN, int DA, int RB, int OCC, bool OH = false, bool X3 = false>
__global__ void __launch_bounds__(NT, OCC) k_conv_stream(ConvP p) {
  static_assert(!X3 || !BF16, "the split-bf16 contraction reads fp32 rows");
  constexpr int EB = BF16 ? 2 : 4, UB = 32 * EB, NJ = UB / 32, SLOTS = UB / 16;
  constexpr int COUT = NB * 32, CIN = UN * 32;
// ... 154 lines not shown
          const int slot = c * SLOTS + 2 * j + fh;
          const u32x4 bf = *reinterpret_cast<const u32x4*>(bl + nb * 32 * BROW + slot * 16);
#pragma unroll
          for (int rb = 0; rb < RB; ++rb) {
            if constexpr (OH) {
              const u32x4 z = {0u, 0u, 0u, 0u};
              mma16<BF16>(acc[rb][nb], idx[k][rb] >= 0 ? a1[rb][c][j] : z, bf);
            } else mma16<BF16>(acc[rb][nb], a[k % DA][rb][c][j], bf);
          }
        }
      }
    if constexpr (!OH) { if (k + DA < K) issue_a(k + DA, a[k % DA]); }
    if (k + 1 < K) __syncthreads();
  }

  if constexpr (PD > 0) {
    if (p.epi_mode == TL_EPI_NONE) {
      epi_wave_tail_lds<BF16, WAVES, EP, NB, RB, false, PD>(p, Es, Af, tid, r0, acc);
      return;
    }
  }
  __syncthreads();
  float* ew = Es + wv * 32 * EP;
  float red0[NB], red1[NB];
#pragma unroll
  for (int nb = 0; nb < NB; ++nb) { red0[nb] = 0.f; red1[nb] = 0.f; }
#pragma unroll
  for (int rb = 0; rb < RB; ++rb)
#pragma unroll
    for (int nb = 0; nb < NB; ++nb) {
#pragma unroll
      for (int r = 0; r < 16; ++r) ew[((r & 3) + 8 * (r >> 2) + 4 * fh) * EP + fi] = acc[rb][nb][r];
      __builtin_amdgcn_fence(__ATOMIC_RELEASE, "wavefront");
      __builtin_amdgcn_wave_barrier();
      epi_block32<BF16, EP>(p, ew, lane, r0 + rb * 32, nb * 32, red0[nb], red1[nb]);
      __builtin_amdgcn_fence(__ATOMIC_RELEASE, "wavefront");
      __builtin_amdgcn_wave_barrier();
    }
  if (p.epi_mode != TL_EPI_NONE) epi_finish_wg<WAVES, EP, NB>(p, Es, tid, red0, red1);
}

template <bool BF16, int K, int NB, int UN, int DA, int RB, bool OH = false, bool X3 = false>
int launch(ConvP p, hipStream_t s) {
  if constexpr (X3) p.w = p.w_x3;
  constexpr int EB = BF16 ? 2 : 4;
  constexpr int BPTL = (NB * 32 * UN * (BF16 ? 4 : 8) + NT - 1) / NT;
  constexpr int VG = RB * NB * 16 + DA * RB * UN * (BF16 ? 8 : 16) + (K <= 8 ? 8 : 27) * RB + 4 * BPTL * (DA > 2 ? DA - 1 : 1) + 20;
  constexpr int OCC = (OH && X3) ? 2 : ((VG <= 120 || (X3 && NB * UN <= 4)) ? 4 : 2);
  const size_t wt = 2 * (size_t)NB * 32 * (UN * 32 * EB + 16), ep = (size_t)WAVES * 32 * 36 * 4;
  const size_t lds = (wt > ep ? wt : ep) + (stream_epi_ahead<BF16, K, NB, UN, RB, OH, X3>() > 0 ? 6 * (size_t)NB * 32 * 4 : 0);
  if (lds > 160 * 1024) return TL_ERR_UNSUPPORTED;
  p.nblk = (int)tl_cdiv(p.n_out, WAVES * 32 * RB);
  if (p.red_nparts) *p.red_nparts = p.nblk;
  return tl_launch_lds<k_conv_stream<BF16, K, NB, UN, DA, RB, OCC, OH, X3>>(p.nblk, NT, lds, s, p);
}

template <bool BF16, int K>
int dispatch(const ConvP& p, hipStream_t s) {
  const int nb = p.Cout / 32, un = p.Cin / 32;
  if constexpr (BF16 && K == 8) {
    if (p.one_hot) {
      if (nb == 2 && un == 3) return launch<true, 8, 2, 3, 1, 1, true>(p, s);
      if (nb == 1 && un == 2) return launch<true, 8, 1, 2, 1, 1, true>(p, s);
      if (nb == 3 && un == 4) return launch<true, 8, 3, 4, 1, 1, true>(p, s);
    }
  }
  if constexpr (!BF16 && K == 8) {
    if (p.one_hot == 1 && p.w_x3 && p.epi_mode == TL_EPI_NONE) {
      if (nb == 2 && un == 3) return launch<false, 8, 2, 3, 1, 1, true, true>(p, s);
      if (nb == 3 && un == 4) return launch<false, 8, 3, 4, 1, 1, true, true>(p, s);
    }
  }
  if constexpr (BF16 && K == 8) {
    if (!p.one_hot && nb == 2 && un == 1) return launch<true, 8, 2, 1, 3, 2>(p, s);
  }
#define TL_S(NB_, UN_, DB_, RB_, DF_)                                                                \
  if (nb == NB_ && un == UN_) {                                                                      \
    if constexpr (BF16) return launch<true, K, NB_, UN_, DB_, RB_>(p, s);                            \
    else {                                                                                           \
      if (p.w_x3) return launch<false, K, NB_, UN_, 1, 1, false, true>(p, s);    \
      return launch<false, K, NB_, UN_, DF_, 1>(p, s);                                               \
    }                                                                                                \
  }
  TL_S(2, 2, 3, 1, 2) TL_S(2, 4, 2, 1, 1) TL_S(3, 3, 1, 2, 1) TL_S(3, 6, 1, 1, 1) TL_S(4, 4, 2, 1, 1) TL_S(2, 3, 3, 1, 1) TL_S(3, 2, 3, 1, 2)
  TL_S(3, 4, 2, 1, 1) TL_S(4, 3, 2, 1, 1) TL_S(1, 2, 3, 1, 2) TL_S(2, 1, 3, 1, 2) TL_S(1, 1, 3, 1, 2)
#undef TL_S
  return TL_ERR_UNSUPPORTED;
}

}

int TL_H16(tl_launch_conv_stream)(const ConvP& p, int dtype, hipStream_t s) {
  if (p.in_scale || p.in_relu) return TL_ERR_UNSUPPORTED;
  const int eb = dtype == TL_BF16 ? 2 : 4;
  const int64_t ld_b = p.in_ld * eb, in_bytes = (p.n_in - 1) * ld_b + (int64_t)p.Cin * eb;
  if (!(in_bytes > 0 && in_bytes + 2 * ld_b < 0xFFFFFFFFll)) return TL_ERR_UNSUPPORTED;
  if (dtype == TL_BF16) {
    switch (p.K) {
      case 27: return dispatch<true, 27>(p, s);
      case 8: return dispatch<true, 8>(p, s);
    }
  } else {
    switch (p.K) {
      case 27: return dispatch<false, 27>(p, s);
      case 8: return dispatch<false, 8>(p, s);
    }
// ... 4 lines not shown
```

treelearn_amd/csrc/tl_conv_streamq.hip:

```cpp
#include "tl_conv_internal.h"
#include <atomic>
#include <type_traits>

namespace {

template <int CTRL>
static __device__ __forceinline__ uint32_t qperm(uint32_t v) {
  return (uint32_t)__builtin_amdgcn_mov_dpp((int)v, CTRL, 0xf, 0xf, true);
}

static __device__ __forceinline__ void quad_transpose(const u32x4 (&S)[4], u32x4 (&F)[4], bool o0, bool o1) {
  u32x4 T[4];
#pragma unroll
  for (int i1 = 0; i1 < 2; ++i1)
#pragma unroll
    for (int d = 0; d < 4; ++d) {
      const uint32_t P = S[2 * i1][d], Q = S[2 * i1 + 1][d];
      const uint32_t Pn = qperm<0xB1>(P), Qn = qperm<0xB1>(Q);
      T[2 * i1][d] = o0 ? Qn : P;
      T[2 * i1 + 1][d] = o0 ? Q : Pn;
    }
#pragma unroll
  for (int x0 = 0; x0 < 2; ++x0)
#pragma unroll
// ... 203 lines not shown
    const char* bl = Bs + (k & 1) * COUT * BROW + fi * BROW + fh * 64;
#pragma unroll
    for (int pp = 0; pp < PN; ++pp)
#pragma unroll
      for (int s = 0; s < 4; ++s)
#pragma unroll
        for (int nb = 0; nb < NB; ++nb) {
          const u32x4 bf = *reinterpret_cast<const u32x4*>(bl + nb * 32 * BROW + (pp * 8 + s) * 16);
#pragma unroll
          for (int rb = 0; rb < RB; ++rb) {
            mma16<true>(acc[rb][nb], F[rb][pp][s], bf);
          }
        }
    if (k + DA < KV) { issue_a(k + DA, a[k % DA]); if (k + DA + 1 < KV) read_idx(k + DA + 1); }
    if (k + 1 < KV) __syncthreads();
  }
  }

  if constexpr (PD > 0) {
    if (p.epi_mode == TL_EPI_NONE) {
      epi_wave_tail_lds<!X3, W, EP, NB, RB, true, PD>(p, Es, Af, tid, r0, acc);
      return;
    }
  }
  __syncthreads();
  float* ew = Es + wv * 32 * EP;
  float red0[NB], red1[NB];
#pragma unroll
  for (int nb = 0; nb < NB; ++nb) { red0[nb] = 0.f; red1[nb] = 0.f; }
#pragma unroll
  for (int rb = 0; rb < RB; ++rb)
#pragma unroll
    for (int nb = 0; nb < NB; ++nb) {
#pragma unroll
      for (int r = 0; r < 16; ++r) ew[(2 * (r >> 2) + fh + 8 * (r & 3)) * EP + fi] = acc[rb][nb][r];
      __builtin_amdgcn_fence(__ATOMIC_RELEASE, "wavefront");
      __builtin_amdgcn_wave_barrier();
      epi_block32<!X3, EP>(p, ew, lane, r0 + rb * 32, nb * 32, red0[nb], red1[nb]);
      __builtin_amdgcn_fence(__ATOMIC_RELEASE, "wavefront");
      __builtin_amdgcn_wave_barrier();
    }
  if (p.epi_mode != TL_EPI_NONE) epi_finish_wg<W, EP, NB>(p, Es, tid, red0, red1);
}

template <int K, int NB, int PN, int DA, int W = 8, int RB = 1, int SP = 1, bool X3 = false, bool UL = false>
int launch(ConvP p, hipStream_t s) {
  constexpr int OCC = 2;
  if constexpr (X3) p.w = p.w_x3;
  const size_t wt = 2 * (size_t)NB * 32 * (PN * 128 + 16) + (size_t)W * K * 32 * RB * 4, ep = (size_t)W * 32 * 36 * 4;
  const size_t lds = (wt > ep ? wt : ep) + (streamq_epi_ahead<K, NB, PN, RB, X3>() > 0 ? 6 * (size_t)NB * 32 * 4 : 0);
  if (lds > 160 * 1024) return TL_ERR_UNSUPPORTED;
  p.nblk = (int)tl_cdiv(p.n_out, W * 32 * RB);
  if (p.red_nparts) *p.red_nparts = p.nblk;
  return tl_launch_lds<k_conv_streamq<K, NB, PN, DA, W, RB, OCC, SP, X3, UL>>(p.nblk, W * 64, lds, s, p);
}

}

int TL_H16(tl_launch_conv_streamq)(const ConvP& p, hipStream_t s) {
  if (p.in_scale || p.in_relu || p.Cin % 64 || p.Cout % 32) return TL_ERR_UNSUPPORTED;
  const int64_t ld_b = p.in_ld * 2, in_bytes = (p.n_in - 1) * ld_b + (int64_t)p.Cin * 2;
  if (!(in_bytes > 0 && in_bytes + 2 * ld_b < 0xFFFFFFFFll)) return TL_ERR_UNSUPPORTED;
  const int nb = p.Cout / 32, pn = p.Cin / 64;
  if (p.K == 27) {
    if (nb == 2 && pn == 1) return launch<27, 2, 1, 2>(p, s);
    if (nb == 2 && pn == 2) return launch<27, 2, 2, 2>(p, s);
    if (nb == 4 && pn == 2) return launch<27, 4, 2, 2>(p, s);
    if (nb == 4 && pn == 1) return launch<27, 4, 1, 2>(p, s);
    if (nb == 3 && pn == 3) return launch<27, 3, 3, 2>(p, s);
    if (nb == 4 && pn == 4) return launch<27, 4, 2, 2, 8, 1, 2>(p, s);
  } else if (p.K == 8) {
    if (nb == 3 && pn == 1) return launch<8, 3, 1, 2>(p, s);
  }
  return TL_ERR_UNSUPPORTED;
}

#ifndef TL_F16_BUILD
int tl_launch_conv_streamq_x3(const ConvP& p, hipStream_t s) {
  if (!p.w_x3 || p.in_scale || p.in_relu || p.Cin % 32 || p.Cout % 32 || p.K != 27 || p.epi_mode != TL_EPI_NONE || p.Cin >= 256) return TL_ERR_UNSUPPORTED;
  const int64_t ld_b = p.in_ld * 4, in_bytes = (p.n_in - 1) * ld_b + (int64_t)p.Cin * 4;
  if (!(in_bytes > 0 && in_bytes + 2 * ld_b < 0xFFFFFFFFll) || ((uintptr_t)p.w_x3) % 16) return TL_ERR_UNSUPPORTED;
  const int nb = p.Cout / 32, pn = p.Cin / 32;
  if (nb == 2 && pn == 2) return launch<27, 2, 2, 1, 8, 1, 1, true, true>(p, s);
  if (nb == 2 && pn == 4) return launch<27, 2, 2, 1, 8, 1, 2, true>(p, s);
  if (nb == 3 && pn == 6) return launch<27, 3, 3, 2, 8, 1, 2, true>(p, s);
  return TL_ERR_UNSUPPORTED;
}
#endif
```

treelearn_amd/csrc/tl_exec.hip:

```cpp
#include <string.h>
#include <vector>

#include "tl_common.h"
#include "tl_arena.h"

namespace {

constexpr int64_t kCompactMinRows = 65536;
constexpr int64_t kBlkMinRows = 16384;
constexpr int64_t kBlkMaxRows = (1 << 25) - 64;
constexpr size_t kHostBytes = 64 + (size_t)TL_POINT_COORDS_MAX_PARTS * 16;

struct Ten {
  int64_t off = -1;
  int64_t ld = 0, n = 0;
  int C = 0;
  int64_t own_off = -1, own_bytes = 0;
};

struct ViewReq {
  const Ten* dst = nullptr;
  tl_affine aff{nullptr, nullptr};
  int relu = 0;
};

struct Table {
  const int32_t* table = nullptr;
  const int32_t* compact = nullptr;
  const int32_t* scatter = nullptr;
  bool blk = false;
  int one_hot = 0;
};

struct LevelG {
  int32_t dims[4];
  int64_t n = 0;
  int64_t coords = -1, nbr = -1, ct = -1, child = -1, inv = -1, invp = -1;
};

}

struct tl_exec {
  int32_t* host = nullptr;
  hipEvent_t ev_main = nullptr, ev_side = nullptr, ev_flag = nullptr;
  bool flag_in_flight = false;
  bool profile = false;
  std::vector<hipEvent_t> pev;
  std::vector<tl_launch_rec> recs;
  hipStream_t prof_stream = nullptr;
};

namespace {

struct Run {
  tl_exec* ex;
  const tl_net_desc* net;
  tl_forward_args* a;
  hipStream_t s;
  Arena ar;
  int esize;
  int rc = TL_OK;
  int launches = 0;
  int nl;
  LevelG lv[TL_MAX_LEVELS];
  bool blocked = false;
  int64_t g0 = 0;
  int64_t o_unit = -1, o_counter = -1, o_halo = -1, o_lrb = -1, o_pmask = -1, o_nn = -1;

  const int32_t* gw(int64_t word_off) const { return word_off < 0 ? nullptr : reinterpret_cast<const int32_t*>(ar.at(g0 + 4 * word_off)); }

  Ten alloc(int64_t n, int C) {
    Ten t;
    t.n = n; t.C = C; t.ld = C; t.own_bytes = n * C * esize; t.own_off = t.off = ar.take(t.own_bytes);
    return t;
  }
  void release(Ten& t) {
    if (t.own_off >= 0) ar.give(t.own_off, t.own_bytes);
    t.own_off = -1;
  }
  Ten cols(const Ten& t, int c0, int C) const {
    Ten v;
    v.off = t.off + (int64_t)c0 * esize; v.ld = t.ld; v.n = t.n; v.C = C;
    return v;
  }

  Table subm(int li) const {
    Table t;
    if (li == 0 && blocked) { t.blk = true; return t; }
    t.table = gw(lv[li].nbr); t.compact = gw(lv[li].ct);
    return t;
  }
  Table down(int li) const { Table t; t.table = gw(lv[li].child); return t; }
  Table up(int li) const {
    Table t;
    t.scatter = gw(lv[li].child);
    if (lv[li].invp >= 0) { t.table = gw(lv[li].invp); t.one_hot = 2; }
    else { t.table = gw(lv[li].inv); t.one_hot = 1; }
    return t;
  }

  void conv(int level, int kind, const Ten& x, const tl_weight& w, const Table& tb, int64_t n_out, const ViewReq* views, int nviews, Ten* outs,
            const Ten* residual = nullptr, tl_affine in_aff = {nullptr, nullptr}, int in_relu = 0, int all_ones = 0, int split_part = -1, int split_cin = 0) {
    for (int i = 0; i < nviews; ++i) outs[i] = views[i].dst ? *views[i].dst : alloc(n_out, w.Cout);
    if (rc != TL_OK) return;
    ++launches;
    if (ar.dry) return;
    tl_conv_args c{};
    c.in = ar.at(x.off); c.in_ld = x.ld; c.weight = w.w; c.weight_frag = w.frag; c.weight_x3 = w.x3;
    c.table = tb.table; c.table_compact = tb.compact; c.table_one_hot = tb.one_hot; c.table_scatter = tb.scatter;
    if (tb.blk) {
      c.blk_unit = gw(o_unit); c.blk_counter = gw(o_counter); c.blk_halo = gw(o_halo);
      c.blk_lrb = reinterpret_cast<const uint32_t*>(gw(o_lrb)); c.blk_pmask = gw(o_pmask);
    }
    c.in_all_ones = all_ones;
    c.n_out = n_out; c.n_in = x.n; c.K = w.K; c.Cin = w.Cin; c.Cout = w.Cout; c.dtype = net->dtype;
    c.in_scale = in_aff.scale; c.in_shift = in_aff.shift; c.in_relu = in_relu;
    if (residual) { c.residual = ar.at(residual->off); c.res_ld = residual->ld; }
    c.out = ar.at(outs[0].off); c.out_ld = outs[0].ld; c.out_scale = views[0].aff.scale; c.out_shift = views[0].aff.shift; c.out_relu = views[0].relu;
    if (nviews > 1) { c.out2 = ar.at(outs[1].off); c.out2_ld = outs[1].ld; c.out2_scale = views[1].aff.scale; c.out2_shift = views[1].aff.shift; c.out2_relu = views[1].relu; }
    if (nviews > 2) { c.out3 = ar.at(outs[2].off); c.out3_ld = outs[2].ld; c.out3_scale = views[2].aff.scale; c.out3_shift = views[2].aff.shift; c.out3_relu = views[2].relu; }
    const bool prof = ex->profile;
    if (prof) {
      hipEvent_t e0 = nullptr, e1 = nullptr;
      if (hipEventCreate(&e0) != hipSuccess || hipEventCreate(&e1) != hipSuccess) { rc = TL_ERR_LAUNCH; return; }
      ex->pev.push_back(e0); ex->pev.push_back(e1);
      tl_launch_rec r{};
      r.level = level; r.kind = kind; r.K = w.K; r.Cin = w.Cin; r.Cout = w.Cout; r.residual = residual != nullptr; r.esize = esize;
      r.split_part = split_part; r.split_cin = split_cin; r.in_prologue = in_aff.scale != nullptr || in_relu; r.n_out = n_out; r.n_in = x.n;
      ex->recs.push_back(r);
      if (hipEventRecord(e0, s) != hipSuccess) rc = TL_ERR_LAUNCH;
    }
    const int r = tl_conv_fwd(&c, s);
    if (prof && hipEventRecord(ex->pev.back(), s) != hipSuccess) rc = TL_ERR_LAUNCH;
    if (r != TL_OK) rc = r;
  }

  static ViewReq RAW(const Ten* dst = nullptr) { ViewReq v; v.dst = dst; return v; }
  static ViewReq ACT(const tl_affine& aff, const Ten* dst = nullptr) { ViewReq v; v.dst = dst; v.aff = aff; v.relu = 1; return v; }

  void res_block(int li, const tl_res_desc& b, const Ten& x_raw, const Ten& x_act, const ViewReq* views, int nviews, Ten* outs) {
    const Table nb = subm(li);
    const int64_t n = lv[li].n;
    Ten t, res;
    const ViewReq v1 = ACT(b.bn3);
    conv(li, 0, x_act, b.w1, nb, n, &v1, 1, &t);
    const bool has1x1 = b.w1x1.w != nullptr;
    if (has1x1) { const ViewReq vr = RAW(); conv(li, 3, x_raw, b.w1x1, Table{}, n, &vr, 1, &res); }
    conv(li, 0, t, b.w2, nb, n, views, nviews, outs, has1x1 ? &res : &x_raw);
    release(t);
    if (has1x1) release(res);
  }

  void ublock(int li, Ten x_raw, Ten x_act, const ViewReq* views, int nviews, Ten* outs) {
    const tl_ublock_desc& u = net->u[li];
    const int64_t n = lv[li].n;
    const int C = u.C;
    Ten o2[3];
    { const ViewReq v[2] = {RAW(), ACT(u.blocks[1].bn0)}; res_block(li, u.blocks[0], x_raw, x_act, v, 2, o2); }
    release(x_raw); release(x_act);
    x_raw = o2[0]; x_act = o2[1];
    if (!u.deeper) {
      res_block(li, u.blocks[1], x_raw, x_act, views, nviews, outs);
      release(x_raw); release(x_act);
      return;
    }
    Ten cat_raw = alloc(n, 2 * C), cat_act = alloc(n, 2 * C);
    const Ten cr_l = cols(cat_raw, 0, C), cr_r = cols(cat_raw, C, C), ca_l = cols(cat_act, 0, C), ca_r = cols(cat_act, C, C);
    Ten o3[3];
    { const ViewReq v[3] = {RAW(&cr_l), ACT(u.bn_cat_l, &ca_l), ACT(u.bn_down)}; res_block(li, u.blocks[1], x_raw, x_act, v, 3, o3); }
    release(x_raw); release(x_act);
    Ten xd = o3[2], d[2];
    { const ViewReq v[2] = {RAW(), ACT(net->u[li + 1].blocks[0].bn0)}; conv(li, 1, xd, u.wd, down(li), lv[li + 1].n, v, 2, d); }
    release(xd);
// ... 5 lines not shown
    { const ViewReq v[2] = {RAW(), ACT(u.tail[1].bn0)}; res_block(li, u.tail[0], cat_raw, cat_act, v, 2, y); }
    release(cat_raw); release(cat_act);
    res_block(li, u.tail[1], y[0], y[1], views, nviews, outs);
    release(y[0]); release(y[1]);
  }

  void l1_block(const tl_res_desc& b, const Ten& x, const tl_affine& in_aff, const ViewReq* views, int nviews, Ten* outs) {
    const Table nb = subm(0);
    const int64_t n = lv[0].n;
    Ten t, res;
    const ViewReq v1 = ACT(b.bn3);
    conv(0, 0, x, b.w1, nb, n, &v1, 1, &t, nullptr, in_aff, 1);
    const bool has1x1 = b.w1x1.w != nullptr;
    if (has1x1) { const ViewReq vr = RAW(); conv(0, 3, x, b.w1x1, Table{}, n, &vr, 1, &res); }
    conv(0, 0, t, b.w2, nb, n, views, nviews, outs, has1x1 ? &res : &x);
    release(t);
    if (has1x1) release(res);
  }
  void l1_staged(Ten x_raw, const ViewReq* views, int nviews, Ten* outs) {
    const tl_ublock_desc& u = net->u[0];
    const int64_t n = lv[0].n;
    const int C = u.C;
    const Table nb = subm(0);
    Ten x1;
    { const ViewReq v = RAW(); l1_block(u.blocks[0], x_raw, u.blocks[0].bn0, &v, 1, &x1); }
    release(x_raw);
    Ten cat_raw = alloc(n, 2 * C);
    const Ten cr_l = cols(cat_raw, 0, C), cr_r = cols(cat_raw, C, C);
    Ten o2[2];
    { const ViewReq v[2] = {RAW(&cr_l), ACT(u.bn_down)}; l1_block(u.blocks[1], x1, u.blocks[1].bn0, v, 2, o2); }
    release(x1);
    Ten xd = o2[1], d[2];
    { const ViewReq v[2] = {RAW(), ACT(net->u[1].blocks[0].bn0)}; conv(0, 1, xd, u.wd, down(0), lv[1].n, v, 2, d); }
    release(xd);
    Ten e_act;
    { const ViewReq v = ACT(u.bn_up); ublock(1, d[0], d[1], &v, 1, &e_act); }
    { const ViewReq v = RAW(&cr_r); Ten o; conv(0, 2, e_act, u.wu, up(0), n, &v, 1, &o); }
    release(e_act);
    const tl_res_desc& b = u.tail[0];
    Ten part, t, res, y;
    { const ViewReq v = RAW(); conv(0, 0, cr_l, b.w1_half[0], nb, n, &v, 1, &part, nullptr, u.bn_cat_l, 1, 0, 0, 2 * C); }
    { const ViewReq v = ACT(b.bn3); conv(0, 0, cr_r, b.w1_half[1], nb, n, &v, 1, &t, &part, u.bn_cat_r, 1, 0, 1, 2 * C); }
    release(part);
    { const ViewReq v = RAW(); conv(0, 3, cat_raw, b.w1x1, Table{}, n, &v, 1, &res); }
    { const ViewReq v = RAW(); conv(0, 0, t, b.w2, nb, n, &v, 1, &y, &res); }
    release(t); release(res); release(cat_raw);
    l1_block(u.tail[1], y, u.tail[1].bn0, views, nviews, outs);
    release(y);
  }

  void network() {
    const int64_t n1 = lv[0].n;
    const bool feats = net->use_coords || net->use_feats;
    Ten ones = alloc(n1, net->in_channels);
    if (feats) {
      const int64_t ws_bytes = 4 * n1 * net->max_points_per_voxel, o_ws = ar.take(ws_bytes);
      if (!ar.dry) {
        const int r = tl_voxel_feats(a->xyz, a->point_feats, net->in_channels - 3, reinterpret_cast<const int64_t*>(gw(o_v2p)), a->N, n1, net->max_points_per_voxel,
                                     net->use_coords, net->use_feats, net->dtype, reinterpret_cast<int32_t*>(ar.at(o_ws)), ar.at(ones.off), s);
        if (r != TL_OK) rc = r;
      }
      ar.give(o_ws, ws_bytes);
    } else if (!ar.dry) {
      hipError_t e;
      if (net->dtype == TL_F32) e = hipMemsetD32Async((hipDeviceptr_t)ar.at(ones.off), 0x3F800000, n1 * net->in_channels, s);
      else e = hipMemsetD16Async((hipDeviceptr_t)ar.at(ones.off), net->dtype == TL_BF16 ? 0x3F80 : 0x3C00, n1 * net->in_channels, s);
      if (e != hipSuccess) rc = TL_ERR_LAUNCH;
    }
    Ten xs[2], x;
    const ViewReq out = RAW();
    if (blocked) {
      const ViewReq v = RAW();
      Table tin = subm(0);
      if (feats) { tin = Table{}; tin.table = gw(o_nn); }
      conv(0, 4, ones, net->w_in, tin, n1, &v, 1, xs, nullptr, {nullptr, nullptr}, 0, feats ? 0 : 1);
      release(ones);
      l1_staged(xs[0], &out, 1, &x);
    } else {
      const ViewReq v[2] = {RAW(), ACT(net->u[0].blocks[0].bn0)};
      conv(0, 4, ones, net->w_in, subm(0), n1, v, 2, xs, nullptr, {nullptr, nullptr}, 0, feats ? 0 : 1);
      release(ones);
      ublock(0, xs[0], xs[1], &out, 1, &x);
    }
    if (rc == TL_OK && !ar.dry) {
      const int r = tl_head_mlp(ar.at(x.off), x.ld, net->dtype, x.C, reinterpret_cast<const int64_t*>(gw(o_v2p)), a->N, net->out_bn.scale, net->out_bn.shift,
                                net->head_w1, net->head_b1, net->head_w2, net->head_b2, a->backbone, a->logits, a->offsets, s);
      if (r != TL_OK) rc = r;
    }
    release(x);
  }
  int64_t o_v2p = -1;
};

inline int64_t al64(int64_t w) { return (w + 63) & ~int64_t(63); }

inline bool weight_is(const tl_weight& w, int K, int Cin, int Cout) { return w.w && w.K == K && w.Cin == Cin && w.Cout == Cout; }
inline bool affine_ok(const tl_affine& a) { return a.scale && a.shift; }

inline bool res_ok(const tl_res_desc& b, int Cin, int C) {
  if (!affine_ok(b.bn0) || !affine_ok(b.bn3) || !weight_is(b.w1, 27, Cin, C) || !weight_is(b.w2, 27, C, C)) return false;
  if (Cin != C ? !weight_is(b.w1x1, 1, Cin, C) : b.w1x1.w != nullptr) return false;
  for (int h = 0; h < 2; ++h)
    if (b.w1_half[h].w && !(Cin == 2 * C && weight_is(b.w1_half[h], 27, C, C))) return false;
  return (b.w1_half[0].w == nullptr) == (b.w1_half[1].w == nullptr);
}

inline bool net_ok(const tl_net_desc* net) {
  const int nl = net->num_levels;
  if (!weight_is(net->w_in, 27, net->in_channels, net->u[0].C)) return false;
  if (net->u[0].C != 8 && net->u[0].C != 16 && net->u[0].C != 32 && net->u[0].C != 64) return false;
  if (!affine_ok(net->out_bn) || !net->head_w1 || !net->head_b1 || !net->head_w2 || !net->head_b2) return false;
  for (int l = 0; l < nl; ++l) {
    const tl_ublock_desc& u = net->u[l];
    if (u.C <= 0 || (u.deeper != 0) != (l + 1 < nl)) return false;
    if (!res_ok(u.blocks[0], u.C, u.C) || !res_ok(u.blocks[1], u.C, u.C)) return false;
    if (!u.deeper) continue;
    const int Cd = net->u[l + 1].C;
    if (!affine_ok(u.bn_down) || !affine_ok(u.bn_up) || !affine_ok(u.bn_cat_l) || !affine_ok(u.bn_cat_r)) return false;
    if (!weight_is(u.wd, 8, u.C, Cd) || !weight_is(u.wu, 8, Cd, u.C)) return false;
    if (!res_ok(u.tail[0], 2 * u.C, u.C) || !res_ok(u.tail[1], u.C, u.C)) return false;
  }
  return true;
}

}

extern "C" {

tl_exec* tl_exec_create(void) {
  tl_exec* ex = new (std::nothrow) tl_exec();
  if (!ex) return nullptr;
  if (hipHostMalloc(reinterpret_cast<void**>(&ex->host), kHostBytes, hipHostMallocDefault) != hipSuccess || (memset(ex->host, 0, kHostBytes), false) ||
      hipEventCreateWithFlags(&ex->ev_main, hipEventDisableTiming) != hipSuccess || hipEventCreateWithFlags(&ex->ev_side, hipEventDisableTiming) != hipSuccess ||
      hipEventCreateWithFlags(&ex->ev_flag, hipEventDisableTiming) != hipSuccess) {
    tl_exec_destroy(ex);
    return nullptr;
  }
// ... 80 lines not shown
  ex->flag_in_flight = false;
  if (ex->host[3]) return TL_ERR_EXTENT;
  if (ex->host[8]) {
    ex->host[8] = 0;
    return TL_ERR_BLK;
  }
  const int32_t extent[3] = {ex->host[0] + 1, ex->host[1] + 1, ex->host[2] + 1};
  int32_t shape[TL_MAX_LEVELS][3];
  for (int j = 0; j < 3; ++j) {
    shape[0][j] = net->has_shape ? net->spatial_shape[j] : extent[j];
    if (extent[j] > shape[0][j]) return TL_ERR_EXTENT;
  }
  for (int l = 1; l < nl; ++l)
    for (int j = 0; j < 3; ++j) {
      shape[l][j] = shape[l - 1][j] / 2;
      if (shape[l][j] <= 0) return TL_ERR_REACH_ZERO;
    }

  int64_t nw[TL_MAX_LEVELS], woff[TL_MAX_LEVELS + 1];
  {
    int32_t d[4] = {a->B, extent[0], extent[1], extent[2]};
    woff[0] = 0;
    for (int l = 0; l < nl; ++l) {
      for (int j = 0; j < 4; ++j) R.lv[l].dims[j] = d[j];
      nw[l] = tl_nwords(tl_dims(d));
      woff[l + 1] = woff[l] + nw[l];
      for (int j = 1; j < 4; ++j) d[j] = (d[j] + 1) / 2;
    }
  }
  const int64_t tw = woff[nl];
  const int64_t n_ws = tl_pyramid_ws_words(R.lv[0].dims, nl, nullptr);
  if (n_ws < 0) return TL_ERR_ARG;
  const int64_t o_pyr = R.ar.take(4 * (3 * tw + 8 + n_ws));
  if (R.ar.peak > R.ar.cap) { a->needed_bytes = R.ar.peak * 2; return TL_ERR_ARENA; }
  char* p0 = R.ar.at(o_pyr);
  rc = tl_pyramid_build(pcoords, N, R.lv[0].dims, shape[0], nl, reinterpret_cast<uint64_t*>(p0), reinterpret_cast<uint32_t*>(p0 + 8 * tw),
                        reinterpret_cast<uint32_t*>(p0 + 12 * tw), reinterpret_cast<uint32_t*>(p0 + 12 * tw + 32), stream);
  if (rc != TL_OK) return rc;
  if (hipMemcpyAsync(ex->host, p0 + 12 * tw, 4 * nl, hipMemcpyDeviceToHost, s) != hipSuccess || hipStreamSynchronize(s) != hipSuccess) return TL_ERR_LAUNCH;
  for (int l = 0; l < nl; ++l) {
    R.lv[l].n = a->level_n[l] = (int64_t)(uint32_t)ex->host[l];
    if (R.lv[l].n <= 0) return TL_ERR_REACH_ZERO;
  }

  const int64_t n1 = R.lv[0].n;
  const tl_ublock_desc& u0 = net->u[0];
  const bool x3_l1 = u0.blocks[0].w1.x3 && u0.blocks[0].w2.x3 && u0.blocks[1].w1.x3 && u0.blocks[1].w2.x3 && u0.tail[0].w1_half[0].x3 && u0.tail[0].w1_half[1].x3 &&
                     u0.tail[0].w2.x3 && u0.tail[1].w1.x3 && u0.tail[1].w2.x3;
  R.blocked = net->blocked && (net->dtype != TL_F32 || x3_l1) && u0.C == 32 && u0.deeper && u0.tail[0].w1_half[0].w && u0.tail[0].w1_half[1].w &&
              n1 >= kBlkMinRows && n1 <= kBlkMaxRows;
  a->blocked_used = R.blocked;
  int64_t cur = 0;
  auto take = [&](int64_t words) { const int64_t o = cur; cur += al64(words); return o; };
  R.o_v2p = take(2 * N);
  for (int l = 0; l < nl; ++l) {
    LevelG& v = R.lv[l];
    const bool skip = R.blocked && l == 0;
    if (!skip) { v.coords = take(4 * v.n); v.nbr = take(27 * v.n); }
    if (!skip && v.n >= kCompactMinRows) v.ct = take(10 * v.n);
    if (l + 1 < nl) v.child = take(8 * R.lv[l + 1].n);
  }
  int64_t o_o2n = -1, o_perm = -1, o_cnew = -1, o_bws = -1;
  if (R.blocked) {
    const int64_t nbws = tl_blk_ws_words(R.lv[0].dims);
    o_o2n = take(n1); o_perm = take(n1); o_cnew = take(4 * n1); R.o_unit = take(4 * n1); R.o_counter = take(64); R.o_halo = take(32 * n1);
    R.o_lrb = take(9 * n1); R.o_pmask = take(n1); o_bws = take(nbws);
    if (feats) R.o_nn = take(27 * n1);
  }
  const bool packed0 = nl > 1 && net->u[0].C == 32 && net->u[1].C == 64 && (net->dtype != TL_F32 || net->u[0].wu.x3) && tl_conv_one_hot_direct_enabled(n1);
  const int64_t o_m1 = cur;
  for (int l = 0; l + 1 < nl; ++l) {
    if (l == 0 && packed0) R.lv[l].invp = take(R.lv[l].n);
    else R.lv[l].inv = take(8 * R.lv[l].n);
  }
  const int64_t o_m1_end = cur;
  R.g0 = R.ar.take(4 * cur);

  {
    Run D = R;
    D.ar.dry = true; D.ar.base = nullptr;
    D.network();
    a->needed_bytes = D.ar.peak;
    if (D.ar.peak > R.ar.cap) return TL_ERR_ARENA;
  }

  auto W = [&](int64_t word_off) { return word_off < 0 ? nullptr : reinterpret_cast<int32_t*>(R.ar.at(R.g0 + 4 * word_off)); };
  tl_level arr[TL_MAX_LEVELS];
  for (int l = 0; l < nl; ++l) {
    LevelG& v = R.lv[l];
    tl_level& t = arr[l];
    for (int j = 0; j < 4; ++j) t.dims[j] = v.dims[j];
    t.n = v.n;
    t.bitmap = reinterpret_cast<const uint64_t*>(p0 + 8 * woff[l]); t.prefix = reinterpret_cast<const uint32_t*>(p0 + 8 * tw + 4 * woff[l]);
    t.coords = W(v.coords); t.nbr = W(v.nbr); t.compact = W(v.ct); t.child = W(v.child); t.parent = nullptr; t.inv = W(v.inv); t.inv_packed = W(v.invp); t.o2n = nullptr;
  }
  hipStream_t side = s;
  struct Join {
    tl_exec* ex; hipStream_t s; hipStream_t* side; bool done = false;
    int join() {
      if (done || *side == s) return TL_OK;
      done = true;
      return (hipEventRecord(ex->ev_side, *side) == hipSuccess && hipStreamWaitEvent(s, ex->ev_side, 0) == hipSuccess) ? TL_OK : TL_ERR_LAUNCH;
    }
    ~Join() { (void)join(); }
  } joiner{ex, s, &side};
  if (R.blocked) {
    tl_blk bk{};
    bk.o2n = W(o_o2n); bk.perm = W(o_perm); bk.coords_new = W(o_cnew); bk.unit = W(R.o_unit); bk.counter = W(R.o_counter); bk.halo = W(R.o_halo);
    bk.lrb = reinterpret_cast<uint32_t*>(W(R.o_lrb)); bk.pmask = W(R.o_pmask); bk.cap_units = n1; bk.halo_max = TL_BLK_HALO_MAX; bk.nn = W(R.o_nn);
    rc = tl_blk_build(arr[0].bitmap, arr[0].prefix, R.lv[0].dims, n1, &bk, reinterpret_cast<uint32_t*>(W(o_bws)), 1, stream);
    if (rc != TL_OK) return rc;
    arr[0].o2n = bk.o2n;
    if (a->side_stream && tl_s(a->side_stream) != s) {
      side = tl_s(a->side_stream);
      if (hipEventRecord(ex->ev_main, s) != hipSuccess || hipStreamWaitEvent(side, ex->ev_main, 0) != hipSuccess) return TL_ERR_LAUNCH;
    }
    rc = tl_blk_build(arr[0].bitmap, arr[0].prefix, R.lv[0].dims, n1, &bk, reinterpret_cast<uint32_t*>(W(o_bws)), 2, reinterpret_cast<tl_stream_t>(side));
    if (rc != TL_OK) return rc;
  }
  rc = tl_rulebooks_build(arr, nl, W(o_m1), o_m1_end - o_m1, pcoords, N, reinterpret_cast<int64_t*>(W(R.o_v2p)), stream);
  if (rc != TL_OK) return rc;
  if (joiner.join() != TL_OK) return TL_ERR_LAUNCH;
  if (R.blocked) {
    if (hipMemcpyAsync(ex->host + 8, W(R.o_counter) + 1, 4, hipMemcpyDeviceToHost, s) != hipSuccess || hipEventRecord(ex->ev_flag, s) != hipSuccess) return TL_ERR_LAUNCH;
    ex->flag_in_flight = true;
  }

  R.network();
// ... 6 lines not shown
```

treelearn_amd/csrc/tl_voxel.hip:

```cpp
#include "tl_scan.h"

namespace {

constexpr int kBlock = 256;

__device__ __forceinline__ uint32_t enc_f32(float f) {
  uint32_t u = __float_as_uint(f);
  return u ^ ((u >> 31) ? 0xFFFFFFFFu : 0x80000000u);
}
__device__ __forceinline__ float dec_f32(uint32_t u) {
  return __uint_as_float((u & 0x80000000u) ? (u ^ 0x80000000u) : ~u);
}

__global__ void k_init_minmax(uint32_t* __restrict__ mm, int B, int32_t* __restrict__ maxc) {
  const int i = blockIdx.x * blockDim.x + threadIdx.x;
  if (i < B * 6) mm[i] = ((i % 6) < 3) ? 0xFFFFFFFFu : 0u;
  if (i < 4) maxc[i] = 0;
}

__global__ void __launch_bounds__(kBlock) k_minmax(const float* __restrict__ xyz, const int64_t* __restrict__ bid,
                                                   int64_t N_all, int B, uint32_t* __restrict__ mm) {
  uint32_t lo[3] = {0xFFFFFFFFu, 0xFFFFFFFFu, 0xFFFFFFFFu}, hi[3] = {0u, 0u, 0u};
  int cb = -1;
  auto flush = [&]() {
// ... 381 lines not shown
    int64_t row = pf[i];
    while (w) {
      const int bit = __ffsll((unsigned long long)w) - 1;
      reinterpret_cast<int4*>(coords)[row++] = make_int4(b, x, y, zw * 64 + bit);
      w &= w - 1;
    }
  }
}

__global__ void __launch_bounds__(kBlock) k_expand_coords(const uint64_t* __restrict__ bm, const uint32_t* __restrict__ pf, TlDims d,
                                                          int32_t* __restrict__ coords) {
  expand_coords_body(bm, pf, d, coords, (int64_t)blockIdx.x * blockDim.x + threadIdx.x, (int64_t)gridDim.x * blockDim.x);
}

__global__ void __launch_bounds__(kBlock) k_point_rank(const int32_t* __restrict__ pc, int64_t N, const uint64_t* __restrict__ bm,
                                                       const uint32_t* __restrict__ pf, TlDims d, int64_t* __restrict__ v2p,
                                                       const int32_t* __restrict__ o2n) {
  for (int64_t i = (int64_t)blockIdx.x * blockDim.x + threadIdx.x; i < N; i += (int64_t)gridDim.x * blockDim.x) {
    const int4 c = reinterpret_cast<const int4*>(pc)[i];
    int r = -1;
    if (c.x >= 0 && c.x < d.B && c.y < d.X && c.z < d.Y && c.w < d.Z) r = tl_rank_at(bm, pf, tl_col_word(d, c.x, c.y, c.z), c.w);
    if (o2n && r >= 0) r = o2n[r];
    v2p[i] = r;
  }
}

__device__ __forceinline__ void rulebook_subm_body(const int32_t* __restrict__ coords, int64_t M, const uint64_t* __restrict__ bm,
                                                   const uint32_t* __restrict__ pf, const TlDims& d, int32_t* __restrict__ nbr,
                                                   int32_t* __restrict__ compact, int64_t first, int64_t stride) {
  for (int64_t i = first; i < M; i += stride) {
    const int4 c = reinterpret_cast<const int4*>(coords)[i];
    uint32_t cmask = 0;
#pragma unroll
    for (int dx = -1; dx <= 1; ++dx) {
#pragma unroll
      for (int dy = -1; dy <= 1; ++dy) {
        const int x = c.y + dx, y = c.z + dy;
        const int tap0 = (dx + 1) * 9 + (dy + 1) * 3;
        int r0 = -1, r1 = -1, r2 = -1;
        if (x >= 0 && x < d.X && y >= 0 && y < d.Y) {
          const int64_t wc = tl_col_word(d, c.x, x, y);
          const int z = c.w;
          const int64_t w = wc + (z >> 6);
          const uint64_t word = bm[w];
          const uint32_t base = pf[w];
          const int bit = z & 63;
          const uint64_t below = (1ull << bit) - 1;
          if (word & (1ull << bit)) r1 = (int)(base + __popcll(word & below));
          if (bit > 0) { if (word & (1ull << (bit - 1))) r0 = (int)(base + __popcll(word & (below >> 1))); }
          else if (z > 0) r0 = tl_rank_at(bm, pf, wc, z - 1);
          if (bit < 63) { if (word & (2ull << bit)) r2 = (int)(base + __popcll(word & ((below << 1) | 1ull))); }
          else if (z + 1 < d.Z) r2 = tl_rank_at(bm, pf, wc, z + 1);
        }
        nbr[(int64_t)(tap0 + 0) * M + i] = r0;
        nbr[(int64_t)(tap0 + 1) * M + i] = r1;
        nbr[(int64_t)(tap0 + 2) * M + i] = r2;
        if (compact) {
          compact[(int64_t)(tap0 / 3) * M + i] = r0 >= 0 ? r0 : (r1 >= 0 ? r1 : r2);
          cmask |= ((r0 >= 0 ? 1u : 0u) | (r1 >= 0 ? 2u : 0u) | (r2 >= 0 ? 4u : 0u)) << tap0;
        }
      }
    }
    if (compact) compact[(int64_t)9 * M + i] = (int32_t)cmask;
  }
}

__global__ void __launch_bounds__(kBlock) k_rulebook_subm(const int32_t* __restrict__ coords, int64_t M, const uint64_t* __restrict__ bm,
                                                          const uint32_t* __restrict__ pf, TlDims d, int32_t* __restrict__ nbr,
                                                          int32_t* __restrict__ compact) {
  rulebook_subm_body(coords, M, bm, pf, d, nbr, compact, (int64_t)blockIdx.x * blockDim.x + threadIdx.x, (int64_t)gridDim.x * blockDim.x);
}

__device__ __forceinline__ void rulebook_down_body(const int32_t* __restrict__ cc, int64_t Mc, const uint64_t* __restrict__ fbm,
                                                   const uint32_t* __restrict__ fpf, const TlDims& f, int64_t Mf, int32_t* __restrict__ child,
                                                   int32_t* __restrict__ parent, int32_t* __restrict__ inv, int64_t first, int64_t stride,
                                                   const int32_t* __restrict__ fo2n = nullptr, int32_t* __restrict__ invp = nullptr) {
  for (int64_t q = first; q < Mc; q += stride) {
    const int4 c = reinterpret_cast<const int4*>(cc)[q];
#pragma unroll
    for (int k = 0; k < 8; ++k) {
      const int x = 2 * c.y + (k >> 2), y = 2 * c.z + ((k >> 1) & 1), z = 2 * c.w + (k & 1);
      int r = -1;
      if (x < f.X && y < f.Y && z < f.Z) r = tl_rank_at(fbm, fpf, tl_col_word(f, c.x, x, y), z);
      if (fo2n && r >= 0) r = fo2n[r];
      child[(int64_t)k * Mc + q] = r;
      if (r >= 0) {
        if (parent) parent[r] = (int)q;
        if (inv) inv[(int64_t)k * Mf + r] = (int)q;
        if (invp) invp[r] = (int)((q << 3) | k);
      }
    }
  }
}

__global__ void __launch_bounds__(kBlock) k_rulebook_down(const int32_t* __restrict__ cc, int64_t Mc, const uint64_t* __restrict__ fbm,
                                                          const uint32_t* __restrict__ fpf, TlDims f, int64_t Mf,
                                                          int32_t* __restrict__ child, int32_t* __restrict__ parent, int32_t* __restrict__ inv,
                                                          const int32_t* __restrict__ fo2n, int32_t* __restrict__ invp) {
  rulebook_down_body(cc, Mc, fbm, fpf, f, Mf, child, parent, inv, (int64_t)blockIdx.x * blockDim.x + threadIdx.x, (int64_t)gridDim.x * blockDim.x, fo2n, invp);
}

struct LevelPack {
  int nl;
  int first[kPyrMaxLevels + 1];
  TlDims d[kPyrMaxLevels];
  int64_t n[kPyrMaxLevels];
  const uint64_t* bm[kPyrMaxLevels];
  const uint32_t* pf[kPyrMaxLevels];
  int32_t* coords[kPyrMaxLevels];
// ... 153 lines not shown
  ScanPack sp;
  sp.nl = 1; sp.first[0] = 0; sp.first[1] = (int)tl_cdiv(nwords, kScanTile); sp.off[0] = 0; sp.nw[0] = nwords;
  hipStream_t s = tl_s(stream);
  k_scan_partials_multi<<<(unsigned)sp.first[1], kBlock, 0, s>>>(bitmap, sp, ws);
  k_scan_blocks_multi<<<1, kBlock, 0, s>>>(ws, sp, total);
  k_scan_final_multi<<<(unsigned)sp.first[1], kBlock, 0, s>>>(bitmap, sp, ws, prefix);
  TL_CHECK_LAUNCH();
  return TL_OK;
}

int tl_expand_coords(const uint64_t* bitmap, const uint32_t* prefix, const int32_t dims[4], int32_t* coords, tl_stream_t stream) {
  if (!bitmap || !prefix || !dims || !coords) return TL_ERR_ARG;
  const TlDims d = tl_dims(dims);
  k_expand_coords<<<tl_grid(tl_nwords(d), kBlock), kBlock, 0, tl_s(stream)>>>(bitmap, prefix, d, coords);
  TL_CHECK_LAUNCH();
  return TL_OK;
}

int tl_point_rank(const int32_t* pcoords, int64_t N, const uint64_t* bitmap, const uint32_t* prefix, const int32_t dims[4],
                  int64_t* v2p, tl_stream_t stream) {
  if (!pcoords || !bitmap || !prefix || !dims || !v2p || N <= 0) return TL_ERR_ARG;
  k_point_rank<<<tl_grid(N, kBlock), kBlock, 0, tl_s(stream)>>>(pcoords, N, bitmap, prefix, tl_dims(dims), v2p, nullptr);
  TL_CHECK_LAUNCH();
  return TL_OK;
}

int tl_voxel_mean_feats(const float* pf, int C, const int64_t* v2p, int64_t N, int64_t M, int P, int32_t* ws, float* out,
                        tl_stream_t stream) {
  if (!pf || !v2p || !ws || !out || C <= 0 || C > 64 || N <= 0 || M <= 0 || P <= 0 || N > 0x7FFFFFFE) return TL_ERR_ARG;
  hipStream_t s = tl_s(stream);
  k_fill_i32<<<tl_grid(M * P, kBlock), kBlock, 0, s>>>(ws, M * P, 0x7FFFFFFF);
  for (int r = 0; r < P; ++r) k_first_points<<<tl_grid(N, kBlock), kBlock, 0, s>>>(v2p, N, P, r, ws);
  k_mean_feats<<<tl_grid(M * C, kBlock), kBlock, 0, s>>>(pf, C, M, P, ws, out);
  TL_CHECK_LAUNCH();
  return TL_OK;
}

int tl_voxel_feats(const float* xyz, const float* feats, int F, const int64_t* v2p, int64_t N, int64_t M, int P, int use_coords, int use_feats,
                   int dtype, int32_t* ws, void* out, tl_stream_t stream) {
  if (!xyz || !feats || !v2p || !ws || !out || F <= 0 || F > 5 || N <= 0 || M <= 0 || P <= 0 || N > 0x7FFFFFFE) return TL_ERR_ARG;
  hipStream_t s = tl_s(stream);
  k_fill_i32<<<tl_grid(M * P, kBlock), kBlock, 0, s>>>(ws, M * P, 0x7FFFFFFF);
  for (int r = 0; r < P; ++r) k_first_points<<<tl_grid(N, kBlock), kBlock, 0, s>>>(v2p, N, P, r, ws);
  if (dtype == TL_F32) k_voxel_feats<float><<<tl_grid(M, kBlock), kBlock, 0, s>>>(xyz, feats, F, M, P, ws, use_coords, use_feats, static_cast<float*>(out));
  else if (dtype == TL_BF16) k_voxel_feats<__bf16><<<tl_grid(M, kBlock), kBlock, 0, s>>>(xyz, feats, F, M, P, ws, use_coords, use_feats, static_cast<__bf16*>(out));
  else if (dtype == TL_F16) k_voxel_feats<_Float16><<<tl_grid(M, kBlock), kBlock, 0, s>>>(xyz, feats, F, M, P, ws, use_coords, use_feats, static_cast<_Float16*>(out));
  else return TL_ERR_ARG;
  TL_CHECK_LAUNCH();
  return TL_OK;
}

int tl_rulebook_subm(const int32_t* coords, int64_t M, const uint64_t* bitmap, const uint32_t* prefix, const int32_t dims[4],
                     int32_t* nbr, int32_t* compact, tl_stream_t stream) {
  if (!coords || !bitmap || !prefix || !dims || !nbr || M <= 0) return TL_ERR_ARG;
  k_rulebook_subm<<<tl_grid(M, kBlock), kBlock, 0, tl_s(stream)>>>(coords, M, bitmap, prefix, tl_dims(dims), nbr, compact);
  TL_CHECK_LAUNCH();
  return TL_OK;
}

int tl_rulebook_down(const int32_t* ccoords, int64_t Mc, const uint64_t* fbitmap, const uint32_t* fprefix, const int32_t fdims[4],
                     int64_t Mf, int32_t* child, int32_t* parent, int32_t* inv, tl_stream_t stream) {
  if (!ccoords || !fbitmap || !fprefix || !fdims || !child || !parent || !inv || Mc <= 0 || Mf <= 0) return TL_ERR_ARG;
  hipStream_t s = tl_s(stream);
  if (hipMemsetAsync(parent, 0xFF, Mf * 4, s) != hipSuccess) return TL_ERR_LAUNCH;
  if (hipMemsetAsync(inv, 0xFF, Mf * 8 * 4, s) != hipSuccess) return TL_ERR_LAUNCH;
  k_rulebook_down<<<tl_grid(Mc, kBlock), kBlock, 0, s>>>(ccoords, Mc, fbitmap, fprefix, tl_dims(fdims), Mf, child, parent, inv, nullptr, nullptr);
  TL_CHECK_LAUNCH();
  return TL_OK;
}

int64_t tl_pyramid_ws_words(const int32_t dims0[4], int num_levels, int64_t* level_word_offsets) {
  if (!dims0 || num_levels < 1 || num_levels > kPyrMaxLevels) return -1;
  int32_t d[4] = {dims0[0], dims0[1], dims0[2], dims0[3]};
  int64_t off = 0, ws = 0;
  for (int l = 0; l < num_levels; ++l) {
    const int64_t nw = tl_nwords(tl_dims(d));
    if (level_word_offsets) level_word_offsets[l] = off;
    off += nw;
    ws += tl_scan_ws_words(nw);
    for (int j = 1; j < 4; ++j) d[j] = (d[j] + 1) / 2;
  }
  if (level_word_offsets) level_word_offsets[num_levels] = off;
  {
    int32_t d0[4] = {dims0[0], dims0[1], dims0[2], dims0[3]};
    ws += 4 + 16 * tl_nwords(tl_dims(d0));
  }
  return ws;
}

int tl_pyramid_build(const int32_t* pcoords, int64_t N, const int32_t dims0[4], const int32_t shape0[3], int num_levels,
                     uint64_t* bitmaps, uint32_t* prefixes, uint32_t* counts, uint32_t* ws, tl_stream_t stream) {
  if (!pcoords || !dims0 || !shape0 || !bitmaps || !prefixes || !counts || !ws || N <= 0 || num_levels < 1 || num_levels > kPyrMaxLevels)
    return TL_ERR_ARG;
  hipStream_t s = tl_s(stream);
  TlDims d[kPyrMaxLevels];
  int out[kPyrMaxLevels][3];
  int64_t off[kPyrMaxLevels + 1];
  int32_t dd[4] = {dims0[0], dims0[1], dims0[2], dims0[3]};
  int sh[3] = {shape0[0], shape0[1], shape0[2]};
  off[0] = 0;
  for (int l = 0; l < num_levels; ++l) {
    d[l] = tl_dims(dd);
    for (int j = 0; j < 3; ++j) out[l][j] = sh[j];
    off[l + 1] = off[l] + tl_nwords(d[l]);
    for (int j = 1; j < 4; ++j) dd[j] = (dd[j] + 1) / 2;
    for (int j = 0; j < 3; ++j) sh[j] /= 2;
  }
  {
    int64_t scan_ws = 0;
    for (int l2 = 0; l2 < num_levels; ++l2) scan_ws += tl_scan_ws_words(tl_nwords(d[l2]));
    uint8_t* bytes = reinterpret_cast<uint8_t*>((reinterpret_cast<uintptr_t>(ws + scan_ws) + 15) & ~uintptr_t(15));
    const int64_t nw0 = tl_nwords(d[0]);
    if (hipMemsetAsync(bytes, 0, nw0 * 64, s) != hipSuccess) return TL_ERR_LAUNCH;
    k_set_bytes<<<tl_grid(N, kBlock), kBlock, 0, s>>>(pcoords, N, d[0], bytes);
    k_bytes_to_bits<<<tl_grid(nw0, kBlock), kBlock, 0, s>>>(bytes, nw0, bitmaps);
  }
  int l = 0;
  ScanPack sp;
  sp.first[0] = 0;
  for (; l < num_levels; ++l) {
    const int64_t nw = tl_nwords(d[l]);
    if (l > 0 && nw <= kPyrSmallWords) break;
    if (l > 0)
      k_bitmap_down<<<tl_grid(nw, kBlock), kBlock, 0, s>>>(bitmaps + off[l - 1], d[l - 1], out[l][0], out[l][1], out[l][2], bitmaps + off[l], d[l]);
    sp.off[l] = off[l]; sp.nw[l] = nw; sp.first[l + 1] = sp.first[l] + (int)tl_cdiv(nw, kScanTile);
  }
  sp.nl = l;
  k_scan_partials_multi<<<(unsigned)sp.first[l], kBlock, 0, s>>>(bitmaps, sp, ws);
  k_scan_blocks_multi<<<1, kBlock, 0, s>>>(ws, sp, counts);
  k_scan_final_multi<<<(unsigned)sp.first[l], kBlock, 0, s>>>(bitmaps, sp, ws, prefixes);
  if (l < num_levels) {
    PyrSmall p;
    p.nl = num_levels - l; p.first = l;
    p.d[0] = d[l - 1]; p.off[0] = off[l - 1];
    for (int j = 0; j < p.nl; ++j) {
      p.d[j + 1] = d[l + j]; p.off[j + 1] = off[l + j];
      for (int k = 0; k < 3; ++k) p.out[j][k] = out[l + j][k];
    }
    k_pyramid_small<<<1, kPyrBlock, 0, s>>>(bitmaps, prefixes, counts, p);
  }
  TL_CHECK_LAUNCH();
  return TL_OK;
}

int tl_rulebooks_build(const tl_level* lv, int num_levels, int32_t* minus_one, int64_t minus_one_words,
                       const int32_t* pcoords, int64_t N, int64_t* v2p, tl_stream_t stream) {
  if (!lv || num_levels < 1 || num_levels > kPyrMaxLevels) return TL_ERR_ARG;
  for (int l = 0; l < num_levels; ++l) {
    if (!lv[l].bitmap || !lv[l].prefix || lv[l].n <= 0) return TL_ERR_ARG;
    if ((!lv[l].coords || !lv[l].nbr) && !lv[l].o2n) return TL_ERR_ARG;
    if (lv[l].nbr && !lv[l].coords) return TL_ERR_ARG;
    if (l > 0 && !lv[l].coords) return TL_ERR_ARG;
    if (l + 1 < num_levels && (!lv[l].child || (!lv[l].inv && !lv[l].inv_packed))) return TL_ERR_ARG;
    if (lv[l].inv_packed && lv[l].n >= (1ll << 28)) return TL_ERR_ARG;
  }
  hipStream_t s = tl_s(stream);
  auto inside = [&](const int32_t* q, int64_t words) { return minus_one && q >= minus_one && q + words <= minus_one + minus_one_words; };
  if (minus_one && minus_one_words > 0 && hipMemsetAsync(minus_one, 0xFF, minus_one_words * 4, s) != hipSuccess) return TL_ERR_LAUNCH;
  for (int l = 0; l + 1 < num_levels; ++l) {
    if (lv[l].parent && !inside(lv[l].parent, lv[l].n) && hipMemsetAsync(lv[l].parent, 0xFF, lv[l].n * 4, s) != hipSuccess) return TL_ERR_LAUNCH;
    if (lv[l].inv && !inside(lv[l].inv, lv[l].n * 8) && hipMemsetAsync(lv[l].inv, 0xFF, lv[l].n * 32, s) != hipSuccess) return TL_ERR_LAUNCH;
    if (lv[l].inv_packed && !inside(lv[l].inv_packed, lv[l].n) && hipMemsetAsync(lv[l].inv_packed, 0xFF, lv[l].n * 4, s) != hipSuccess) return TL_ERR_LAUNCH;
  }
  int small = num_levels;
  for (int l = num_levels - 1; l >= 1; --l) {
    if (tl_nwords(tl_dims(lv[l].dims)) <= kPyrSmallWords && lv[l].n <= 64 * kPyrSmallWords && !lv[l].compact && !lv[l].o2n && !lv[l - 1].o2n &&
        !lv[l].inv_packed && !lv[l - 1].inv_packed) small = l; else break;
  }
  if (num_levels - small < 2) small = num_levels;
  for (int l = 0; l < small; ++l) {
    const TlDims d = tl_dims(lv[l].dims);
    if (lv[l].coords) k_expand_coords<<<tl_grid(tl_nwords(d), kBlock), kBlock, 0, s>>>(lv[l].bitmap, lv[l].prefix, d, lv[l].coords);
    if (lv[l].nbr) k_rulebook_subm<<<tl_grid(lv[l].n, kBlock), kBlock, 0, s>>>(lv[l].coords, lv[l].n, lv[l].bitmap, lv[l].prefix, d, lv[l].nbr, lv[l].compact);
  }
  LevelPack p;
  p.nl = num_levels - small;
  if (p.nl > 0) {
    for (int j = 0; j < p.nl; ++j) {
      const tl_level& v = lv[small + j];
      p.d[j] = tl_dims(v.dims); p.n[j] = v.n; p.bm[j] = v.bitmap; p.pf[j] = v.prefix; p.coords[j] = v.coords; p.nbr[j] = v.nbr;
      p.child[j] = v.child; p.parent[j] = v.parent; p.inv[j] = v.inv;
    }
    p.first[0] = 0;
    for (int j = 0; j < p.nl; ++j) p.first[j + 1] = p.first[j] + (int)tl_cdiv(tl_nwords(p.d[j]), kBlock);
    k_expand_coords_multi<<<p.first[p.nl], kBlock, 0, s>>>(p);
    for (int j = 0; j < p.nl; ++j) p.first[j + 1] = p.first[j] + (int)tl_cdiv(p.n[j], kBlock);
    k_rulebook_subm_multi<<<p.first[p.nl], kBlock, 0, s>>>(p);
  }
  for (int l = 0; l + 1 < num_levels && l < small; ++l) {
    const tl_level &f = lv[l], &c = lv[l + 1];
    k_rulebook_down<<<tl_grid(c.n, kBlock), kBlock, 0, s>>>(c.coords, c.n, f.bitmap, f.prefix, tl_dims(f.dims), f.n, f.child, f.parent, f.inv, f.o2n, f.inv_packed);
  }
  if (p.nl > 1) {
    p.nl -= 1;
    for (int j = 0; j < p.nl; ++j) p.first[j + 1] = p.first[j] + (int)tl_cdiv(p.n[j + 1], kBlock);
    k_rulebook_down_multi<<<p.first[p.nl], kBlock, 0, s>>>(p);
  }
  if (v2p) {
    if (!pcoords || N <= 0) return TL_ERR_ARG;
    k_point_rank<<<tl_grid(N, kBlock), kBlock, 0, s>>>(pcoords, N, lv[0].bitmap, lv[0].prefix, tl_dims(lv[0].dims), v2p, lv[0].o2n);
  }
  TL_CHECK_LAUNCH();
  return TL_OK;
}

int tl_rulebook_compact(const int32_t* table, int64_t n, int32_t* compact, tl_stream_t stream) {
  if (!table || !compact || n <= 0) return TL_ERR_ARG;
  k_table_compact<<<tl_grid(n, kBlock), kBlock, 0, tl_s(stream)>>>(table, n, compact);
  TL_CHECK_LAUNCH();
  return TL_OK;
}

}
```

treelearn_amd/model/engine.py:

```python
import os

import torch
from torch import nn

from .. import ops
from ..geometry import BlockedRulebook, TileGeometry


def _bn_affine(bn: nn.BatchNorm1d):
    scale = bn.weight.detach().float() / torch.sqrt(bn.running_var.detach().float() + bn.eps)
    shift = bn.bias.detach().float() - bn.running_mean.detach().float() * scale
    return scale.contiguous(), shift.contiguous()


class View:
    __slots__ = ("buf", "scale", "shift", "relu")

    def __init__(self, scale=None, shift=None, relu=False, buf=None):
        self.buf, self.scale, self.shift, self.relu = buf, scale, shift, relu


RAW = lambda buf=None: View(buf=buf)
ACT = lambda aff, buf=None: View(aff[0], aff[1], True, buf)

# ... 70 lines not shown
        t = ops.conv_fwd(cat_raw[:, C:], b.w1_halves[1], nbr, n, in_scale=self.bn_cat_r[0], in_shift=self.bn_cat_r[1], in_relu=True, residual=part,
                         out_scale=b.bn3[0], out_shift=b.bn3[1], out_relu=True, split=(1, 2 * C))
        res = ops.conv_fwd(cat_raw, b.w1x1, None, n)
        (y,) = _conv_views(t, b.w2, nbr, n, [RAW()], residual=res)
        return block(self.tail[1], y, self.tail[1].bn0, views)

    def run(self, x_raw, x_act, geom: TileGeometry, li, views):
        lv = geom.levels[li]
        n, C = lv.n, self.C
        nb = len(self.blocks)
        for i, b in enumerate(self.blocks[:-1]):
            x_raw, x_act = b.run(x_raw, x_act, lv.nbr, n, [RAW(), ACT(self.blocks[i + 1].bn0)])
        if not self.deeper:
            return self.blocks[-1].run(x_raw, x_act, lv.nbr, n, views)
        cat_raw = torch.empty((n, 2 * C), dtype=x_raw.dtype, device=x_raw.device)
        cat_act = torch.empty((n, 2 * C), dtype=x_raw.dtype, device=x_raw.device)
        _, _, xd = self.blocks[-1].run(x_raw, x_act, lv.nbr, n,
                                       [RAW(cat_raw[:, :C]), ACT(self.bn_cat_l, cat_act[:, :C]), ACT(self.bn_down)])
        nxt = geom.levels[li + 1]
        d_raw, d_act = _conv_views(xd, self.wd, lv.child, nxt.n, [RAW(), ACT(self.u.blocks[0].bn0)])
        (e_act,) = self.u.run(d_raw, d_act, geom, li + 1, [ACT(self.bn_up)])
        _conv_views(e_act, self.wu, lv.inv, n, [RAW(cat_raw[:, C:]), ACT(self.bn_cat_r, cat_act[:, C:])], one_hot=True, scatter=lv.child)
        y_raw, y_act = self.tail[0].run(cat_raw, cat_act, lv.nbr, n, [RAW(), ACT(self.tail[1].bn0)])
        return self.tail[1].run(y_raw, y_act, lv.nbr, n, views)


class InferencePlan:
    def __init__(self, model, dtype, x3=False):
        self.dtype = dtype
        self.device = model.input_conv[0].weight.device
        self.x3 = bool(x3) and dtype == torch.float32
        self._exec = None
        prev, ops.PACK_X3 = ops.PACK_X3, self.x3
        try:
            self.w_in = ops.pack_weight(model.input_conv[0].weight, dtype)
            self.unet = _U(model.unet, dtype)
        finally:
            ops.PACK_X3 = prev
        self.so, self.ho = _bn_affine(model.output_layer[0])
        w1, b1 = [], []
        for mlp in (model.semantic_linear, model.offset_linear):
            lin, bn = mlp[0], mlp[1]
            s, h = _bn_affine(bn)
            w1.append(lin.weight.detach().float() * s[:, None])
            b1.append(lin.bias.detach().float() * s + h)
        self.w1 = torch.stack(w1).contiguous(); self.b1 = torch.stack(b1).contiguous()
        self.w2 = torch.cat([model.semantic_linear[3].weight.detach().float(), model.offset_linear[3].weight.detach().float()]).contiguous()
        self.b2 = torch.cat([model.semantic_linear[3].bias.detach().float(), model.offset_linear[3].bias.detach().float()]).contiguous()

    def supports_blocked(self):
        ok_dtype = self.dtype != torch.float32 or (self.x3 and os.environ.get("TL_BLK_X3", "1") != "0")
        return ok_dtype and self.unet.C == 32 and os.environ.get("TL_BLK", "1") != "0"

    def run(self, voxel_feats, geom: TileGeometry, want_backbone=True, all_ones=False):
        lv = geom.levels[0]
        vf = voxel_feats.to(self.dtype).contiguous()
        ones = all_ones and (os.environ.get("TL_NO_ONES_TABLE") != "1" or (geom.blocked and lv.nbr_ref is None))
        staged = (geom.blocked and self.unet.deeper and self.unet.C == 32 and self.unet.tail[0].w1_halves is not None
                  and os.environ.get("TL_BLK_PRO", "1") != "0")
        in_views = [RAW()] if staged else [RAW(), ACT(self.unet.blocks[0].bn0)]
        if geom.blocked and not ones:
            if lv.nbr_ref is None:
                raise RuntimeError("a blocked geometry needs ref_table=True when the input features are not all ones")
            xs = _conv_views(vf.index_select(0, lv.nbr.o2n.long()), self.w_in, lv.nbr_ref, lv.n, in_views)
            perm = lv.nbr.perm.long()
            xs = [t.index_select(0, perm) for t in xs]
        else:
            xs = _conv_views(vf, self.w_in, lv.nbr, lv.n, in_views, all_ones=ones)
        if staged:
            (x,) = self.unet.run_l1_staged(xs[0], geom, [RAW()])
        else:
            (x,) = self.unet.run(xs[0], xs[1], geom, 0, [RAW()])
        if x.shape[1] in ops.HEAD_WIDTHS:
            return ops.head_mlp(x, geom.v2p, self.so, self.ho, self.w1, self.b1, self.w2, self.b2, want_backbone)
        bb = ops.affine_relu(x, self.so, self.ho, True).float().index_select(0, geom.v2p)
        h = torch.relu(torch.einsum("nc,moc->mno", bb, self.w1) + self.b1[:, None, :])
        logits = h[0] @ self.w2[:2].T + self.b2[:2]
        offsets = h[1] @ self.w2[2:].T + self.b2[2:]
        return (bb if want_backbone else None), logits, offsets
```

treelearn_amd/ops.py:

```python
import ctypes

import os

import torch

from . import _hip
from .geometry import BlockedRulebook

PROFILE = None
BLK_LAUNCHES = 0

HEAD_WIDTHS = (8, 16, 32, 64)
PACK_X3 = False


def pack_weight(w_ref: torch.Tensor, dtype: torch.dtype) -> torch.Tensor:
    L = _hip.lib()
    w = w_ref.detach().contiguous().float()
    _hip.require_cuda(w, "weight")
    co, ci = w.shape[0], w.shape[-1]
    K = w.numel() // (co * ci)
    out = torch.empty((K, co, ci), dtype=dtype, device=w.device)
    _hip.check(L.tl_pack_weight(_hip.ptr(w), co, K, ci, _hip.ptr(out), _hip.dtype_code(dtype), _hip.stream()), "tl_pack_weight")
    if co % 32 == 0 and ci % 32 == 0 and K > 1:
# ... 69 lines not shown
    a.table_compact = _hip.ptr(getattr(table, "_tl_compact", None)) if (table is not None and os.environ.get("TL_NO_COMPACT") != "1") else None
    a.n_out = n_out; a.n_in = x.shape[0]
    a.K = K; a.Cin = Cin; a.Cout = Cout; a.dtype = _hip.dtype_code(x.dtype)
    a.in_scale = in_scale.data_ptr() if in_scale is not None else None
    a.in_shift = in_shift.data_ptr() if in_shift is not None else None
    a.in_relu = int(bool(in_relu)); a.out_relu = int(bool(out_relu))
    if residual is not None:
        if residual.dtype != x.dtype or residual.stride(1) != 1:
            raise ValueError("bad residual view")
        a.residual = residual.data_ptr(); a.res_ld = residual.stride(0)
    else:
        a.residual = None; a.res_ld = 0
    a.out_scale = out_scale.data_ptr() if out_scale is not None else None
    a.out_shift = out_shift.data_ptr() if out_shift is not None else None
    a.out = out.data_ptr(); a.out_ld = out.stride(0)
    for name, spec in (("out2", out2), ("out3", out3)):
        if spec is None:
            setattr(a, name, None); setattr(a, name + "_ld", 0); setattr(a, name + "_scale", None); setattr(a, name + "_shift", None); setattr(a, name + "_relu", 0)
            continue
        t, sc, sh, relu = spec
        if t.dtype != x.dtype or t.stride(1) != 1 or t.shape[0] != n_out or t.shape[1] != Cout:
            raise ValueError(f"bad {name} view")
        setattr(a, name, t.data_ptr()); setattr(a, name + "_ld", t.stride(0))
        setattr(a, name + "_scale", sc.data_ptr() if sc is not None else None)
        setattr(a, name + "_shift", sh.data_ptr() if sh is not None else None)
        setattr(a, name + "_relu", int(bool(relu)))
    parts = nparts = None
    if epi is not None:
        parts = torch.empty((int(L.tl_conv_red_parts(n_out)), 2, Cout), dtype=torch.float64, device=x.device)
        nparts = ctypes.c_int32(0)
        a.red_part = parts.data_ptr(); a.red_nparts = ctypes.pointer(nparts)
        if epi == "stats":
            a.epi_mode = _hip.TL_EPI_STATS
        else:
            _, xb, st, relu = epi
            if xb.dtype != x.dtype or xb.stride(1) != 1 or xb.shape[0] != n_out or xb.shape[1] != Cout:
                raise ValueError("bad BatchNorm input view for the bn_bwd epilogue")
            a.epi_mode = _hip.TL_EPI_BN_BWD
            a.bn_x = xb.data_ptr(); a.bn_x_ld = xb.stride(0)
            a.bn_mean = st[0].data_ptr(); a.bn_rstd = st[1].data_ptr(); a.bn_scale = st[2].data_ptr(); a.bn_shift = st[3].data_ptr()
            a.bn_relu = int(bool(relu))
    return a, out, parts, nparts, blk


def conv_route(*args, **kwargs) -> str:
    a = _conv_args(*args, **kwargs)[0]
    buf = ctypes.create_string_buffer(1024)
    rc = _hip.lib().tl_conv_route(ctypes.byref(a), buf, len(buf))
    if rc != _hip.TL_ERR_UNSUPPORTED or a.epi_mode == _hip.TL_EPI_NONE:
        _hip.check(rc, "tl_conv_route")
    return buf.value.decode()


def conv_fwd(x: torch.Tensor, w_packed: torch.Tensor, table, n_out: int, out: torch.Tensor = None,
             in_scale=None, in_shift=None, in_relu=False, residual=None, out_scale=None, out_shift=None, out_relu=False,
             out2=None, out3=None, one_hot=False, epi=None, all_ones=False, split=None, scatter=None):
    L = _hip.lib()
    a, out, parts, nparts, blk = _conv_args(x, w_packed, table, n_out, out, in_scale, in_shift, in_relu, residual, out_scale, out_shift, out_relu,
                                            out2, out3, one_hot, epi, all_ones, split, scatter)
    K, Cout, Cin = w_packed.shape
    if blk is not None:
        global BLK_LAUNCHES
        BLK_LAUNCHES += 1
    if epi is not None:
        rc = L.tl_conv_fwd(ctypes.byref(a), _hip.stream())
        if rc == _hip.TL_ERR_UNSUPPORTED:
            return None
        _hip.check(rc, "tl_conv_fwd")
        return out, parts, int(nparts.value)
    if PROFILE is not None:
        e0 = torch.cuda.Event(enable_timing=True); e1 = torch.cuda.Event(enable_timing=True)
        e0.record()
        _hip.check(L.tl_conv_fwd(ctypes.byref(a), _hip.stream()), "tl_conv_fwd")
        e1.record()
        PROFILE.append((e0, e1, dict(K=K, Cin=Cin, Cout=Cout, n_out=n_out, n_in=x.shape[0], table=blk if blk is not None else table,
                                     residual=residual is not None, esize=x.element_size(), split=split,
                                     in_scale=in_scale is not None or bool(in_relu))))
        return out
    _hip.check(L.tl_conv_fwd(ctypes.byref(a), _hip.stream()), "tl_conv_fwd")
    return out


WGRAD_BLK = True


def _conv_wgrad_blk(x, g, rb, ref_layout):
    L = _hip.lib()
    ws = torch.empty(int(L.tl_conv_wgrad_blk_ws_floats()), dtype=torch.float32, device=x.device)
    parts = []
    for c0 in range(0, x.shape[1], 32):
        xs = x[:, c0:c0 + 32]
        gw = torch.empty((32, 27, 32) if ref_layout else (27, 32, 32), dtype=torch.float32, device=x.device)
        rc = L.tl_conv_wgrad_blk(_hip.ptr(xs), xs.stride(0), _hip.ptr(g), g.stride(0), _hip.dtype_code(x.dtype), _hip.ptr(rb.unit), _hip.ptr(rb.counter), _hip.ptr(rb.halo),
                                 _hip.ptr(rb.lrb), rb.n, 32, 32, _hip.ptr(gw), int(bool(ref_layout)), _hip.ptr(ws), _hip.stream())
        if rc == _hip.TL_ERR_UNSUPPORTED:
            return None
        _hip.check(rc, "tl_conv_wgrad_blk")
        parts.append(gw)
    out = parts[0] if len(parts) == 1 else torch.cat(parts, dim=2)
    out._tl_ref_layout = bool(ref_layout)
    return out


def conv_wgrad(x: torch.Tensor, grad_out: torch.Tensor, table, n_out: int, K: int, ref_layout: bool = False) -> torch.Tensor:
    L = _hip.lib()
    if x.dtype in (torch.bfloat16, torch.float16) and grad_out.dtype == x.dtype:
# ... 186 lines not shown
```

Measured before the change: 265.4 Mpoints/s.

## Skip full neighbor tables when convs only need compact columns; tighten blocked-unit kernel

Adds a probe pass through the network that records, per level, whether any chosen conv kernel actually reads the full 27-column neighbour table. Levels that don't need it skip allocating and writing that table, using only the compact form. The all-ones input path avoids converting the voxel feature tensor when the route is the ones kernel. Separately, the blocked-unit build kernel is reworked with bitmask predicates, a bit-packed split stack, LDS vector rank counting, and serialized hash-collision probing. The changes add a dry-run probe and a more complex layout computation at setup.

Measured after the change: 266.7 Mpoints/s, median of 2. About the same (+0.5%).

```diff
diff --git a/include/treelearn_hip.h b/include/treelearn_hip.h
--- a/include/treelearn_hip.h
+++ b/include/treelearn_hip.h
@@ -49,8 +49,8 @@
 
 
 int tl_rulebook_subm(const int32_t* coords, int64_t M, const uint64_t* bitmap, const uint32_t* prefix,
-                     const int32_t dims[4], int32_t* nbr, int32_t* compact ,
-                     tl_stream_t stream);
+                     const int32_t dims[4], int32_t* nbr ,
+                     int32_t* compact , tl_stream_t stream);
 
 int tl_rulebook_down(const int32_t* ccoords, int64_t Mc, const uint64_t* fbitmap, const uint32_t* fprefix,
                      const int32_t fdims[4], int64_t Mf, int32_t* child, int32_t* parent, int32_t* inv, tl_stream_t stream);
@@ -125,6 +125,7 @@
 
 int tl_conv_fwd(const tl_conv_args* args, tl_stream_t stream);
 int tl_conv_route(const tl_conv_args* args, char* buf, int cap);
+int tl_conv_reads_table(const tl_conv_args* args);
 
 int tl_pack_weight(const float* w_ref, int Cout, int K, int Cin, void* w_packed, int dtype, tl_stream_t stream);
 int64_t tl_pack_weight_x3_bytes(int Cout, int K, int Cin);
diff --git a/treelearn_amd/_hip.py b/treelearn_amd/_hip.py
--- a/treelearn_amd/_hip.py
+++ b/treelearn_amd/_hip.py
@@ -139,6 +139,7 @@
     "tl_blk_build": (_i32, [_vp, _vp, _I4, _i64, _c.POINTER(Blk), _vp, _i32, _vp]),
     "tl_conv_fwd": (_i32, [_c.POINTER(ConvArgs), _vp]),
     "tl_conv_route": (_i32, [_c.POINTER(ConvArgs), _c.c_char_p, _i32]),
+    "tl_conv_reads_table": (_i32, [_c.POINTER(ConvArgs)]),
     "tl_conv_red_parts": (_i64, [_i64]),
     "tl_exec_create": (_vp, []),
     "tl_exec_destroy": (None, [_vp]),
diff --git a/treelearn_amd/csrc/tl_blk.hip b/treelearn_amd/csrc/tl_blk.hip
--- a/treelearn_amd/csrc/tl_blk.hip
+++ b/treelearn_amd/csrc/tl_blk.hip
@@ -135,9 +135,9 @@
 
 __global__ void __launch_bounds__(kBlock) k_blk_units(const uint64_t* __restrict__ bm, TlDims d, BlkOut p) {
   __shared__ uint32_t s_tab[kBlock / 64][HASH + 64];
-  __shared__ uint32_t s_list[kBlock / 64][LIST];
+  __shared__ __attribute__((aligned(16))) uint32_t s_list[kBlock / 64][LIST + 4];
   __shared__ uint32_t s_lslot[kBlock / 64][LIST];
-  const int lane = threadIdx.x & 63, wv = threadIdx.x >> 6;
+  const int lane = threadIdx.x & 63, wv = __builtin_amdgcn_readfirstlane((int)(threadIdx.x >> 6));
   const int64_t chunk = (int64_t)blockIdx.x * (kBlock / 64) + wv;
   if (chunk >= p.nchunks) return;
   uint32_t* tab = s_tab[wv];
@@ -162,41 +162,46 @@
     const int64_t ci0 = rvalid ? (((int64_t)c.x * d.X + c.y) * d.Y + c.z) * p.BZ : 0;
     const bool xin[3] = {rvalid && c.y > 0, rvalid, rvalid && c.y + 1 < d.X}, yin[3] = {c.z > 0, true, c.z + 1 < d.Y};
     const int zw1 = rvalid ? (z >> 6) : 0, zw0 = (rvalid && x0) ? ((z - 1) >> 6) : zw1, zw2 = (rvalid && x2) ? ((z + 1) >> 6) : zw1;
-    bool inb[9];
+    uint32_t inbm = 0;
+#pragma unroll
+    for (int q = 0; q < 9; ++q) inbm |= (xin[q / 3] && yin[q % 3]) ? (1u << q) : 0u;
     uint64_t w1[9];
 #pragma unroll
     for (int q = 0; q < 9; ++q) {
       const int dx = q / 3 - 1, dy = q % 3 - 1;
-      inb[q] = xin[q / 3] && yin[q % 3];
-      w1[q] = bm[wc0 + (inb[q] ? (dx * d.Y + dy) * d.Zw : 0) + zw1];
-    }
+      w1[q] = bm[wc0 + (((inbm >> q) & 1u) ? (dx * d.Y + dy) * d.Zw : 0) + zw1];
+    }
+    const int sh1 = z & 56, sh0 = (hz0 ? z - 1 : z) & 56, sh2 = (hz2 ? z + 1 : z) & 56;
     uint32_t by3[9];
 #pragma unroll
     for (int q = 0; q < 9; ++q) {
-      const uint32_t b1 = (uint32_t)(w1[q] >> (z & 56)) & 0xFFu;
-      const uint32_t b0 = (uint32_t)(w1[q] >> ((hz0 ? z - 1 : z) & 56)) & 0xFFu, b2 = (uint32_t)(w1[q] >> ((hz2 ? z + 1 : z) & 56)) & 0xFFu;
+      const uint32_t b1 = (uint32_t)(w1[q] >> sh1) & 0xFFu;
+      const uint32_t b0 = (uint32_t)(w1[q] >> sh0) & 0xFFu, b2 = (uint32_t)(w1[q] >> sh2) & 0xFFu;
       by3[q] = b0 | (b1 << 8) | (b2 << 16);
     }
     if (__any(x0 || x2)) {
+      const int zwo = x0 ? zw0 : zw2;
 #pragma unroll
       for (int q = 0; q < 9; ++q) {
         const int dx = q / 3 - 1, dy = q % 3 - 1;
-        const int64_t wcq = wc0 + (inb[q] ? (dx * d.Y + dy) * d.Zw : 0);
-        const uint64_t a0 = bm[wcq + zw0], a2 = bm[wcq + zw2];
-        if (x0) by3[q] = (by3[q] & ~0xFFu) | ((uint32_t)(a0 >> ((z - 1) & 56)) & 0xFFu);
-        if (x2) by3[q] = (by3[q] & ~0xFF0000u) | (((uint32_t)(a2 >> ((z + 1) & 56)) & 0xFFu) << 16);
-      }
-    }
-    bool p0[9], p1[9], p2[9];
+        const uint64_t ao = bm[wc0 + (((inbm >> q) & 1u) ? (dx * d.Y + dy) * d.Zw : 0) + zwo];
+        if (x0) by3[q] = (by3[q] & ~0xFFu) | (uint32_t)(ao >> 56);
+        if (x2) by3[q] = (by3[q] & ~0xFF0000u) | (((uint32_t)ao & 0xFFu) << 16);
+      }
+    }
+    const uint32_t zok = (hz0 ? 1u : 0u) | 2u | (hz2 ? 4u : 0u);
+    const int s0 = (z - 1) & 7, s1 = 8 + (z & 7), s2 = 16 + ((z + 1) & 7);
+#pragma unroll
+    for (int q = 0; q < 9; ++q) {
+      const uint32_t t = ((by3[q] >> s0) & 1u) | (((by3[q] >> s1) & 1u) << 1) | (((by3[q] >> s2) & 1u) << 2);
+      pm |= (t & zok & (0u - ((inbm >> q) & 1u))) << (3 * q);
+    }
     uint32_t sA[9], sB[9];
 #pragma unroll
     for (int q = 0; q < 9; ++q) {
       const int dx = q / 3 - 1, dy = q % 3 - 1;
-      p0[q] = inb[q] && hz0 && ((by3[q] >> ((z - 1) & 7)) & 1u);
-      p1[q] = inb[q] && ((by3[q] >> (8 + (z & 7))) & 1u);
-      p2[q] = inb[q] && hz2 && ((by3[q] >> (16 + ((z + 1) & 7))) & 1u);
-      const bool any = p0[q] || p1[q] || p2[q];
-      const int64_t ciq = ci0 + (inb[q] ? (dx * d.Y + dy) * p.BZ : 0);
+      const bool any = ((pm >> (3 * q)) & 7u) != 0;
+      const int64_t ciq = ci0 + (((inbm >> q) & 1u) ? (dx * d.Y + dy) * p.BZ : 0);
       sA[q] = p.cs[any ? ciq + bA : 0];
       sB[q] = p.cs[(any && bB != bA) ? ciq + bB : 0];
     }
@@ -206,67 +211,74 @@
 #pragma unroll
     for (int q = 0; q < 9; ++q) {
       const uint32_t b_ = bB != bA ? sB[q] : sA[q];
-      if (p0[q]) { nn[3 * q] = rowid(by3[q] & 0xFFu, z - 1, sA[q]); pm |= 1u << (3 * q); }
-      if (p1[q]) { nn[3 * q + 1] = rowid((by3[q] >> 8) & 0xFFu, z, (z >> 3) == bA ? sA[q] : b_); pm |= 2u << (3 * q); }
-      if (p2[q]) { nn[3 * q + 2] = rowid((by3[q] >> 16) & 0xFFu, z + 1, b_); pm |= 4u << (3 * q); }
+      nn[3 * q] = ((pm >> (3 * q)) & 1u) ? rowid(by3[q] & 0xFFu, z - 1, sA[q]) : -1;
+      nn[3 * q + 1] = ((pm >> (3 * q + 1)) & 1u) ? rowid((by3[q] >> 8) & 0xFFu, z, (z >> 3) == bA ? sA[q] : b_) : -1;
+      nn[3 * q + 2] = ((pm >> (3 * q + 2)) & 1u) ? rowid((by3[q] >> 16) & 0xFFu, z + 1, b_) : -1;
     }
     if (rvalid) {
       p.pmask[r] = (int32_t)pm;
       if (p.nn_out) {
-#pragma unroll
-        for (int k = 0; k < 27; ++k) p.nn_out[(int64_t)k * p.n + r] = nn[k];
+        int32_t* q = p.nn_out + r;
+#pragma unroll
+        for (int k = 0; k < 27; ++k, q += p.n) *q = nn[k];
       }
     }
   }
 
   int nref = __popc(pm);
   for (int off = 32; off > 0; off >>= 1) nref += __shfl_xor(nref, off);
+  nref = __builtin_amdgcn_readfirstlane(nref);
   const int TS = nref <= 360 ? 512 : (nref <= 720 ? 1024 : HASH);
   const int tshift = nref <= 360 ? 23 : (nref <= 720 ? 22 : 21);
   auto hs = [&](int v) __attribute__((always_inline)) { return ((uint32_t)v * 2654435761u) >> tshift; };
 
-  int st_a[8], st_e[8];
-  int sp = 1;
-  st_a[0] = 0; st_e[0] = cnt;
-  bool first = true;
-  while (sp > 0) {
-    --sp;
-    const int a = st_a[sp], e = st_e[sp];
-    const int lo = (int)base + a, hi = (int)base + e;
+  auto pick = [&](int k) __attribute__((always_inline)) {
+    int v = 0;
+#pragma unroll
+    for (int j = 0; j < 27; ++j) v |= k == j ? nn[j] : 0;
+    return v;
+  };
+
+  int a = 0, e = cnt, depth = 0;
+  uint64_t ends = 0;
+  bool first = true, more = true;
+  auto next_piece = [&]() __attribute__((always_inline)) {
+    if (depth == 0) { more = false; return; }
+    a = e; e = (int)(ends & 127u); ends >>= 7; --depth;
+  };
+  for (; more; ) {
+    const int lo = (int)base + a;
     for (int i = lane; i < TS; i += 64) tab[i] = EMPTY;
     __builtin_amdgcn_fence(__ATOMIC_ACQ_REL, "workgroup");
     const bool inr = lane >= a && lane < e;
     uint32_t outm = 0;
 #pragma unroll
-    for (int k = 0; k < 27; ++k) {
-      const int v = nn[k];
-      const bool out = inr && v >= 0 && (v < lo || v >= hi);
-      outm |= out ? (1u << k) : 0u;
-      tab[out ? hs(v) : (uint32_t)TS] = (uint32_t)v;
-    }
+    for (int k = 0; k < 27; ++k) outm |= (uint32_t)(nn[k] - lo) >= (uint32_t)(e - a) ? (1u << k) : 0u;
+    outm = inr ? (outm & pm) : 0u;
+    const uint32_t ownm = inr ? (pm & ~outm) : 0u;
+#pragma unroll
+    for (int k = 0; k < 27; ++k) tab[((outm >> k) & 1u) ? hs(nn[k]) : (uint32_t)TS] = (uint32_t)nn[k];
     __builtin_amdgcn_fence(__ATOMIC_ACQ_REL, "workgroup");
     uint32_t lost = 0;
 #pragma unroll
     for (int k = 0; k < 27; ++k) {
       const uint32_t cur = tab[hs(nn[k])];
-      lost |= (((outm >> k) & 1u) && cur != (uint32_t)nn[k]) ? (1u << k) : 0u;
-    }
+      lost |= cur != (uint32_t)nn[k] ? (1u << k) : 0u;
+    }
+    lost &= outm;
     if (__any(lost != 0)) {
-#pragma unroll
-      for (int k = 0; k < 27; ++k) {
-        bool todo = (lost >> k) & 1u;
-        if (__any(todo)) {
-          uint32_t s_ = hs(nn[k]);
-          while (__any(todo)) {
-            if (todo) {
-              s_ = (s_ + 1) & (uint32_t)(TS - 1);
-              if (tab[s_] == EMPTY) tab[s_] = (uint32_t)nn[k];
-            }
-            __builtin_amdgcn_fence(__ATOMIC_ACQ_REL, "workgroup");
-            if (todo && tab[s_] == (uint32_t)nn[k]) todo = false;
-            __builtin_amdgcn_fence(__ATOMIC_ACQ_REL, "workgroup");
-          }
+      bool act = false;
+      uint32_t key = 0, s_ = 0;
+      for (;;) {
+        if (!act && lost) { key = (uint32_t)pick(__ffs((int)lost) - 1); s_ = hs((int)key); act = true; }
+        if (!__any(act)) break;
+        if (act) {
+          s_ = (s_ + 1) & (uint32_t)(TS - 1);
+          if (tab[s_] == EMPTY) tab[s_] = key;
         }
+        __builtin_amdgcn_fence(__ATOMIC_ACQ_REL, "workgroup");
+        if (act && tab[s_] == key) { act = false; lost &= lost - 1; }
+        __builtin_amdgcn_fence(__ATOMIC_ACQ_REL, "workgroup");
       }
     }
     int H = 0;
@@ -285,9 +297,8 @@
       }
     }
     if (H > p.halo_max && e - a > 1) {
-      const int mid = a + (e - a) / 2;
-      st_a[sp] = mid; st_e[sp] = e; ++sp;
-      st_a[sp] = a; st_e[sp] = mid; ++sp;
+      ends = (ends << 7) | (uint64_t)e; ++depth;
+      e = a + (e - a) / 2;
       continue;
     }
     int u;
@@ -295,33 +306,35 @@
     else {
       int t = 0;
       if (lane == 0) t = atomicAdd(p.counter, 1);
-      u = __shfl(t, 0);
+      u = __builtin_amdgcn_readfirstlane(t);
     }
     first = false;
     if (u >= p.cap_units || H > LIST - 2) {
       if (lane == 0) atomicMax(p.counter + 1, 1);
+      next_piece();
       continue;
     }
+    if (lane < 4) list[H + lane] = EMPTY;
     __builtin_amdgcn_fence(__ATOMIC_ACQ_REL, "workgroup");
     {
       const uint32_t k0 = lane < H ? list[lane] : EMPTY, s0 = lane < H ? lslot[lane] : (uint32_t)TS;
       int r0 = 0;
       const int H16 = (H + 15) & ~15;
       if (H <= 64) {
-        for (int i = 0; i < H; ++i) r0 += (uint32_t)__builtin_amdgcn_readlane((int)k0, i) < k0 ? 1 : 0;
+        for (int i = 0; i < H; i += 4) {
+          const uint4 b = *reinterpret_cast<const uint4*>(list + i);
+          r0 += (b.x < k0 ? 1 : 0) + (b.y < k0 ? 1 : 0) + (b.z < k0 ? 1 : 0) + (b.w < k0 ? 1 : 0);
+        }
         if (lane < H) p.halo[(int64_t)lo * 32 + r0] = (int32_t)k0;
         tab[s0] = k0 | ((uint32_t)r0 << 25);
         if (lane >= H && lane < H16) p.halo[(int64_t)lo * 32 + lane] = -1;
       } else {
         const uint32_t k1 = lane + 64 < H ? list[lane + 64] : EMPTY, s1 = lane + 64 < H ? lslot[lane + 64] : (uint32_t)TS;
         int r1 = 0;
-        for (int i = 0; i < 64; ++i) {
-          const uint32_t b = (uint32_t)__builtin_amdgcn_readlane((int)k0, i);
-          r0 += b < k0 ? 1 : 0; r1 += b < k1 ? 1 : 0;
-        }
-        for (int i = 64; i < H; ++i) {
-          const uint32_t b = (uint32_t)__builtin_amdgcn_readlane((int)k1, i - 64);
-          r0 += b < k0 ? 1 : 0; r1 += b < k1 ? 1 : 0;
+        for (int i = 0; i < H; i += 4) {
+          const uint4 b = *reinterpret_cast<const uint4*>(list + i);
+          r0 += (b.x < k0 ? 1 : 0) + (b.y < k0 ? 1 : 0) + (b.z < k0 ? 1 : 0) + (b.w < k0 ? 1 : 0);
+          r1 += (b.x < k1 ? 1 : 0) + (b.y < k1 ? 1 : 0) + (b.z < k1 ? 1 : 0) + (b.w < k1 ? 1 : 0);
         }
         p.halo[(int64_t)lo * 32 + r0] = (int32_t)k0;
         tab[s0] = k0 | ((uint32_t)r0 << 25);
@@ -340,31 +353,34 @@
 #pragma unroll
       for (int k = 0; k < 27; ++k) cur[k] = tab[hs(nn[k])];
 #pragma unroll
-      for (int k = 0; k < 27; ++k) miss |= (((outm >> k) & 1u) && (cur[k] & KEYMASK) != (uint32_t)nn[k]) ? (1u << k) : 0u;
+      for (int k = 0; k < 27; ++k) miss |= (cur[k] & KEYMASK) != (uint32_t)nn[k] ? (1u << k) : 0u;
+      miss &= outm;
+      auto entry = [](int pos) __attribute__((always_inline)) { return (uint32_t)(pos * 4 + ((pos >> 2) & 3)); };
+#pragma unroll
+      for (int k = 0; k < 27; ++k) {
+        const int mo = __builtin_amdgcn_sbfe((int)(outm & ~miss), k, 1), mw = __builtin_amdgcn_sbfe((int)ownm, k, 1);
+        const int pos = 191 + (mo & ((int)(cur[k] >> 25) - 127)) + (mw & (nn[k] - lo - 191));
+        wds[k / 3] |= entry(pos) << ((k % 3) * 10);
+      }
       if (__any(miss != 0)) {
-#pragma unroll
-        for (int k = 0; k < 27; ++k) {
-          bool todo = (miss >> k) & 1u;
-          if (__any(todo)) {
-            uint32_t s_ = hs(nn[k]);
-            while (__any(todo)) {
-              if (todo) {
-                s_ = (s_ + 1) & (uint32_t)(TS - 1);
-                const uint32_t c_ = tab[s_];
-                if ((c_ & KEYMASK) == (uint32_t)nn[k]) { cur[k] = c_; todo = false; }
-              }
+        bool act = false;
+        int k = 0;
+        uint32_t key = 0, s_ = 0;
+        for (;;) {
+          if (!act && miss) { k = __ffs((int)miss) - 1; key = (uint32_t)pick(k); s_ = hs((int)key); act = true; }
+          if (!__any(act)) break;
+          if (act) {
+            s_ = (s_ + 1) & (uint32_t)(TS - 1);
+            const uint32_t c_ = tab[s_];
+            if ((c_ & KEYMASK) == key) {
+              const uint32_t val = (entry(64 + (int)(c_ >> 25)) ^ entry(191)) << ((k % 3) * 10);
+#pragma unroll
+              for (int q = 0; q < 9; ++q) wds[q] ^= q == k / 3 ? val : 0u;
+              act = false; miss &= miss - 1;
             }
           }
         }
       }
-#pragma unroll
-      for (int k = 0; k < 27; ++k) {
-        const int v = nn[k];
-        const bool out = (outm >> k) & 1u;
-        const int pos = out ? 64 + (int)(cur[k] >> 25) : ((inr && v >= 0) ? v - lo : 191);
-        const uint32_t val = (uint32_t)(pos * 4 + ((pos >> 2) & 3));
-        wds[k / 3] |= val << ((k % 3) * 10);
-      }
       if (inr) {
         uint32_t* dst = p.lrb + r * 9;
 #pragma unroll
@@ -373,6 +389,7 @@
     }
     if (lane == 0) reinterpret_cast<int4*>(p.unit)[u] = make_int4(lo, e - a, H, 0);
     __builtin_amdgcn_fence(__ATOMIC_ACQ_REL, "workgroup");
+    next_piece();
   }
 }
 
diff --git a/treelearn_amd/csrc/tl_common.h b/treelearn_amd/csrc/tl_common.h
--- a/treelearn_amd/csrc/tl_common.h
+++ b/treelearn_amd/csrc/tl_common.h
@@ -30,6 +30,8 @@
 extern thread_local TlRoute* tl_route_armed;
 template <auto Kernel> struct TlKernelTag {};
 int tl_route_record(TlRoute* r, const char* tag, bool f16, dim3 grid, dim3 block, size_t lds);
+void tl_route_table_free(TlRoute* r);
+static inline void tl_launch_table_free() { if (TlRoute* r = tl_route_armed) tl_route_table_free(r); }
 #ifdef TL_F16_BUILD
 constexpr bool kTlF16Build = true;
 #else
diff --git a/treelearn_amd/csrc/tl_conv.hip b/treelearn_amd/csrc/tl_conv.hip
--- a/treelearn_amd/csrc/tl_conv.hip
+++ b/treelearn_amd/csrc/tl_conv.hip
@@ -8,10 +8,18 @@
   char text[1024] = "";
   int len = 0;
   bool truncated = false;
+  bool names = true;
+  bool table_free_next = false;
+  bool reads_table = false;
 };
 thread_local TlRoute* tl_route_armed = nullptr;
 
+void tl_route_table_free(TlRoute* r) { r->table_free_next = true; }
+
 int tl_route_record(TlRoute* r, const char* tag, bool f16, dim3 grid, dim3 block, size_t lds) {
+  r->reads_table |= !r->table_free_next;
+  r->table_free_next = false;
+  if (!r->names) return TL_OK;
   int status = 0;
   char* full = abi::__cxa_demangle(tag, nullptr, nullptr, &status);
   struct Free { char* p; ~Free() { free(p); } } guard{full};
@@ -99,8 +107,10 @@
 constexpr int TL_NEXT = 1;
 int or_next(int rc) { return rc == TL_ERR_UNSUPPORTED ? TL_NEXT : rc; }
 
+bool column_only(const tl_conv_args* a) { return !a->table && a->K == 27 && a->table_compact; }
+
 int validate(const tl_conv_args* a, bool has_blk) {
-  if (!a->table && a->K != 1 && !has_blk && !(a->in_all_ones && a->blk_pmask)) return TL_ERR_ARG;
+  if (!a->table && a->K != 1 && !has_blk && !(a->in_all_ones && a->blk_pmask) && !column_only(a)) return TL_ERR_ARG;
   if ((a->in_scale == nullptr) != (a->in_shift == nullptr)) return TL_ERR_ARG;
   if ((a->out_scale == nullptr) != (a->out_shift == nullptr)) return TL_ERR_ARG;
   if (a->dtype != TL_F32 && a->dtype != TL_BF16 && a->dtype != TL_F16) return TL_ERR_ARG;
@@ -159,7 +169,7 @@
   return or_next(tl_launch_conv_blk_x3(c.p, c.s));
 }
 
-int rung_needs_table(Conv& c) { return (!c.a->table && c.a->K != 1) ? TL_ERR_UNSUPPORTED : TL_NEXT; }
+int rung_needs_table(Conv& c) { return (!c.a->table && c.a->K != 1 && !column_only(c.a)) ? TL_ERR_UNSUPPORTED : TL_NEXT; }
 
 int rung_up(Conv& c) {
   const tl_conv_args* a = c.a;
@@ -252,6 +262,23 @@
     rung_h16_one_hot_direct, rung_h16_one_hot_stream, rung_h16_direct, rung_h16_streamq, rung_h16_stream, rung_h16_tile,
     rung_scalar_only, rung_tinycout, rung_generic,
 };
+
+int walk(Conv& c) {
+  for (auto rung : kLadder) {
+    const int rc = rung(c);
+    if (rc != TL_NEXT) return rc;
+    if (TlRoute* r = tl_route_armed) r->table_free_next = false;
+  }
+  return TL_ERR_UNSUPPORTED;
+}
+
+int walk_armed(Conv& c, TlRoute* r) {
+  TlRoute* const outer = tl_route_armed;
+  tl_route_armed = r;
+  const int rc = walk(c);
+  tl_route_armed = outer;
+  return rc;
+}
 
 }
 
@@ -287,11 +314,29 @@
   c.L = c.f16 ? &kTlConvF16 : &kTlConvBf16;
   c.train = a->epi_mode != TL_EPI_NONE;
   if (c.train && a->red_nparts) *a->red_nparts = 0;
-  for (auto rung : kLadder) {
-    const int rc = rung(c);
-    if (rc != TL_NEXT) return rc;
-  }
-  return TL_ERR_UNSUPPORTED;
+  if (!a->table && a->K != 1) {
+    TlRoute probe;
+    probe.names = false;
+    Conv w = c;
+    const int rc = walk_armed(w, &probe);
+    if (rc == TL_OK && probe.reads_table) return TL_ERR_ARG;
+  }
+  return walk(c);
+}
+
+int tl_conv_reads_table(const tl_conv_args* a) {
+  if (!a) return TL_ERR_ARG;
+  tl_conv_args q = *a;
+  static const int32_t kSomeTable[4] = {0, 0, 0, 0};
+  if (!q.table && q.K != 1) q.table = kSomeTable;
+  TlRoute probe;
+  probe.names = false;
+  TlRoute* const outer = tl_route_armed;
+  tl_route_armed = &probe;
+  const int rc = tl_conv_fwd(&q, nullptr);
+  tl_route_armed = outer;
+  if (rc != TL_OK) return rc;
+  return probe.reads_table ? 1 : 0;
 }
 
 int tl_conv_route(const tl_conv_args* a, char* buf, int cap) {
diff --git a/treelearn_amd/csrc/tl_conv_blk.hip b/treelearn_amd/csrc/tl_conv_blk.hip
--- a/treelearn_amd/csrc/tl_conv_blk.hip
+++ b/treelearn_amd/csrc/tl_conv_blk.hip
@@ -395,6 +395,7 @@
   constexpr size_t lds = (size_t)WS_B + AFF_B + (size_t)W * STAGE_B + (TR ? (size_t)W * 2 * 32 * 8 : 0);
   static_assert(lds <= 160 * 1024, "LDS budget");
   if (TR && p.red_nparts) *p.red_nparts = 256;
+  tl_launch_table_free();
   return tl_launch_lds<k_conv_blk<W, RES, NV, TR, PRO>>(256, W * 64, lds, s, p);
 }
 
diff --git a/treelearn_amd/csrc/tl_conv_blk_x3.hip b/treelearn_amd/csrc/tl_conv_blk_x3.hip
--- a/treelearn_amd/csrc/tl_conv_blk_x3.hip
+++ b/treelearn_amd/csrc/tl_conv_blk_x3.hip
@@ -340,6 +340,7 @@
 int launch_x3(const ConvP& p, const X3P& xp, hipStream_t s) {
   constexpr size_t lds = (size_t)WS_B + AFF_B + (size_t)W * STAGE_B;
   static_assert(lds <= 160 * 1024, "LDS budget");
+  tl_launch_table_free();
   return tl_launch_lds<k_conv_blk_x3<W, RES, NV>>(256, W * 64, lds, s, p, xp);
 }
 
diff --git a/treelearn_amd/csrc/tl_conv_direct.hip b/treelearn_amd/csrc/tl_conv_direct.hip
--- a/treelearn_amd/csrc/tl_conv_direct.hip
+++ b/treelearn_amd/csrc/tl_conv_direct.hip
@@ -444,6 +444,7 @@
   const int need = (int)tl_cdiv(ntiles, WAVES);
   if (grid > need) grid = need;
   if (p.red_nparts) *p.red_nparts = grid;
+  if constexpr (K == 27 && CT) tl_launch_table_free();
   return tl_launch_lds<k_conv_direct<BF16, K, NB, UN, G, WAVES, CT, TR, OH, X3>>(grid, WAVES * 64, lds, s, p, ntiles, 0);
   }
 }
@@ -492,6 +493,7 @@
 int TL_H16(tl_launch_conv_ones27)(const ConvP& p, int dtype, hipStream_t s) {
   if (p.K != 27 || p.Cout != 32 || (!p.ctab && !p.blk_pmask) || p.Cin <= 0 || p.Cin > 64 || p.in_scale || p.in_relu || p.epi_mode != TL_EPI_NONE) return TL_ERR_UNSUPPORTED;
   const unsigned g = tl_grid(p.n_out * 4, 256);
+  tl_launch_table_free();
   if (dtype == TL_BF16) return tl_launch<k_conv_ones27<true>>(g, 256, 0, s, p);
   return tl_launch<k_conv_ones27<false>>(g, 256, 0, s, p);
 }
diff --git a/treelearn_amd/csrc/tl_conv_stream.hip b/treelearn_amd/csrc/tl_conv_stream.hip
--- a/treelearn_amd/csrc/tl_conv_stream.hip
+++ b/treelearn_amd/csrc/tl_conv_stream.hip
@@ -230,6 +230,7 @@
   if (lds > 160 * 1024) return TL_ERR_UNSUPPORTED;
   p.nblk = (int)tl_cdiv(p.n_out, WAVES * 32 * RB);
   if (p.red_nparts) *p.red_nparts = p.nblk;
+  if (K == 27 && p.ctab) tl_launch_table_free();
   return tl_launch_lds<k_conv_stream<BF16, K, NB, UN, DA, RB, OCC, OH, X3>>(p.nblk, NT, lds, s, p);
 }
 
diff --git a/treelearn_amd/csrc/tl_conv_streamq.hip b/treelearn_amd/csrc/tl_conv_streamq.hip
--- a/treelearn_amd/csrc/tl_conv_streamq.hip
+++ b/treelearn_amd/csrc/tl_conv_streamq.hip
@@ -279,6 +279,7 @@
   if (lds > 160 * 1024) return TL_ERR_UNSUPPORTED;
   p.nblk = (int)tl_cdiv(p.n_out, W * 32 * RB);
   if (p.red_nparts) *p.red_nparts = p.nblk;
+  if (K == 27 && p.ctab) tl_launch_table_free();
   return tl_launch_lds<k_conv_streamq<K, NB, PN, DA, W, RB, OCC, SP, X3, UL>>(p.nblk, W * 64, lds, s, p);
 }
 
diff --git a/treelearn_amd/csrc/tl_exec.hip b/treelearn_amd/csrc/tl_exec.hip
--- a/treelearn_amd/csrc/tl_exec.hip
+++ b/treelearn_amd/csrc/tl_exec.hip
@@ -65,6 +65,9 @@
   LevelG lv[TL_MAX_LEVELS];
   bool blocked = false;
   int64_t g0 = 0;
+  bool probe = false;
+  bool need_table[TL_MAX_LEVELS];
+  bool ones_route = false;
   int64_t o_unit = -1, o_counter = -1, o_halo = -1, o_lrb = -1, o_pmask = -1, o_nn = -1;
 
   const int32_t* gw(int64_t word_off) const { return word_off < 0 ? nullptr : reinterpret_cast<const int32_t*>(ar.at(g0 + 4 * word_off)); }
@@ -119,6 +122,14 @@
     c.out = ar.at(outs[0].off); c.out_ld = outs[0].ld; c.out_scale = views[0].aff.scale; c.out_shift = views[0].aff.shift; c.out_relu = views[0].relu;
     if (nviews > 1) { c.out2 = ar.at(outs[1].off); c.out2_ld = outs[1].ld; c.out2_scale = views[1].aff.scale; c.out2_shift = views[1].aff.shift; c.out2_relu = views[1].relu; }
     if (nviews > 2) { c.out3 = ar.at(outs[2].off); c.out3_ld = outs[2].ld; c.out3_scale = views[2].aff.scale; c.out3_shift = views[2].aff.shift; c.out3_relu = views[2].relu; }
+    if (probe) {
+      if (all_ones) {
+        char route[256];
+        ones_route = tl_conv_route(&c, route, (int)sizeof route) == TL_OK && !strncmp(route, "k_conv_ones27<", 14);
+      }
+      if (w.K == 27 && tb.compact && tl_conv_reads_table(&c) != 0) need_table[level] = true;
+      return;
+    }
     const bool prof = ex->profile;
     if (prof) {
       hipEvent_t e0 = nullptr, e1 = nullptr;
@@ -230,16 +241,19 @@
   void network() {
     const int64_t n1 = lv[0].n;
     const bool feats = net->use_coords || net->use_feats;
-    Ten ones = alloc(n1, net->in_channels);
+    const bool no_input = !feats && ones_route && !probe;
+    Ten ones;
+    if (no_input) { ones.off = 0; ones.n = n1; ones.C = ones.ld = net->in_channels; }
+    else ones = alloc(n1, net->in_channels);
     if (feats) {
       const int64_t ws_bytes = 4 * n1 * net->max_points_per_voxel, o_ws = ar.take(ws_bytes);
-      if (!ar.dry) {
+      if (!ar.dry && !probe) {
         const int r = tl_voxel_feats(a->xyz, a->point_feats, net->in_channels - 3, reinterpret_cast<const int64_t*>(gw(o_v2p)), a->N, n1, net->max_points_per_voxel,
                                      net->use_coords, net->use_feats, net->dtype, reinterpret_cast<int32_t*>(ar.at(o_ws)), ar.at(ones.off), s);
         if (r != TL_OK) rc = r;
       }
       ar.give(o_ws, ws_bytes);
-    } else if (!ar.dry) {
+    } else if (!ar.dry && !probe && !no_input) {
       hipError_t e;
       if (net->dtype == TL_F32) e = hipMemsetD32Async((hipDeviceptr_t)ar.at(ones.off), 0x3F800000, n1 * net->in_channels, s);
       else e = hipMemsetD16Async((hipDeviceptr_t)ar.at(ones.off), net->dtype == TL_BF16 ? 0x3F80 : 0x3C00, n1 * net->in_channels, s);
@@ -260,7 +274,7 @@
       release(ones);
       ublock(0, xs[0], xs[1], &out, 1, &x);
     }
-    if (rc == TL_OK && !ar.dry) {
+    if (rc == TL_OK && !ar.dry && !probe) {
       const int r = tl_head_mlp(ar.at(x.off), x.ld, net->dtype, x.C, reinterpret_cast<const int64_t*>(gw(o_v2p)), a->N, net->out_bn.scale, net->out_bn.shift,
                                 net->head_w1, net->head_b1, net->head_w2, net->head_b2, a->backbone, a->logits, a->offsets, s);
       if (r != TL_OK) rc = r;
@@ -447,28 +461,46 @@
   a->blocked_used = R.blocked;
   int64_t cur = 0;
   auto take = [&](int64_t words) { const int64_t o = cur; cur += al64(words); return o; };
-  R.o_v2p = take(2 * N);
-  for (int l = 0; l < nl; ++l) {
-    LevelG& v = R.lv[l];
-    const bool skip = R.blocked && l == 0;
-    if (!skip) { v.coords = take(4 * v.n); v.nbr = take(27 * v.n); }
-    if (!skip && v.n >= kCompactMinRows) v.ct = take(10 * v.n);
-    if (l + 1 < nl) v.child = take(8 * R.lv[l + 1].n);
-  }
-  int64_t o_o2n = -1, o_perm = -1, o_cnew = -1, o_bws = -1;
-  if (R.blocked) {
-    const int64_t nbws = tl_blk_ws_words(R.lv[0].dims);
-    o_o2n = take(n1); o_perm = take(n1); o_cnew = take(4 * n1); R.o_unit = take(4 * n1); R.o_counter = take(64); R.o_halo = take(32 * n1);
-    R.o_lrb = take(9 * n1); R.o_pmask = take(n1); o_bws = take(nbws);
-    if (feats) R.o_nn = take(27 * n1);
-  }
+  int64_t o_o2n = -1, o_perm = -1, o_cnew = -1, o_bws = -1, o_m1 = 0, o_m1_end = 0;
   const bool packed0 = nl > 1 && net->u[0].C == 32 && net->u[1].C == 64 && (net->dtype != TL_F32 || net->u[0].wu.x3) && tl_conv_one_hot_direct_enabled(n1);
-  const int64_t o_m1 = cur;
-  for (int l = 0; l + 1 < nl; ++l) {
-    if (l == 0 && packed0) R.lv[l].invp = take(R.lv[l].n);
-    else R.lv[l].inv = take(8 * R.lv[l].n);
-  }
-  const int64_t o_m1_end = cur;
+  auto layout = [&]() {
+    cur = 0;
+    R.o_v2p = take(2 * N);
+    for (int l = 0; l < nl; ++l) {
+      LevelG& v = R.lv[l];
+      const bool skip = R.blocked && l == 0;
+      const bool ct = !skip && v.n >= kCompactMinRows;
+      v.nbr = -1;
+      if (!skip) { v.coords = take(4 * v.n); if (!ct || R.need_table[l]) v.nbr = take(27 * v.n); }
+      if (ct) v.ct = take(10 * v.n);
+      if (l + 1 < nl) v.child = take(8 * R.lv[l + 1].n);
+    }
+    if (R.blocked) {
+      const int64_t nbws = tl_blk_ws_words(R.lv[0].dims);
+      o_o2n = take(n1); o_perm = take(n1); o_cnew = take(4 * n1); R.o_unit = take(4 * n1); R.o_counter = take(64); R.o_halo = take(32 * n1);
+      R.o_lrb = take(9 * n1); R.o_pmask = take(n1); o_bws = take(nbws);
+      if (feats) R.o_nn = take(27 * n1);
+    }
+    o_m1 = cur;
+    for (int l = 0; l + 1 < nl; ++l) {
+      if (l == 0 && packed0) R.lv[l].invp = take(R.lv[l].n);
+      else R.lv[l].inv = take(8 * R.lv[l].n);
+    }
+    o_m1_end = cur;
+  };
+  for (int l = 0; l < nl; ++l) R.need_table[l] = true;
+  layout();
+  {
+    Run P = R;
+    P.probe = true;
+    P.g0 = P.ar.take(4 * cur);
+    for (int l = 0; l < nl; ++l) P.need_table[l] = R.lv[l].ct < 0;
+    P.network();
+    if (P.rc != TL_OK) return P.rc;
+    for (int l = 0; l < nl; ++l) R.need_table[l] = P.need_table[l];
+    R.ones_route = P.ones_route;
+  }
+  layout();
   R.g0 = R.ar.take(4 * cur);
 
   {
diff --git a/treelearn_amd/csrc/tl_voxel.hip b/treelearn_amd/csrc/tl_voxel.hip
--- a/treelearn_amd/csrc/tl_voxel.hip
+++ b/treelearn_amd/csrc/tl_voxel.hip
@@ -457,9 +457,11 @@
           if (bit < 63) { if (word & (2ull << bit)) r2 = (int)(base + __popcll(word & ((below << 1) | 1ull))); }
           else if (z + 1 < d.Z) r2 = tl_rank_at(bm, pf, wc, z + 1);
         }
-        nbr[(int64_t)(tap0 + 0) * M + i] = r0;
-        nbr[(int64_t)(tap0 + 1) * M + i] = r1;
-        nbr[(int64_t)(tap0 + 2) * M + i] = r2;
+        if (nbr) {
+          nbr[(int64_t)(tap0 + 0) * M + i] = r0;
+          nbr[(int64_t)(tap0 + 1) * M + i] = r1;
+          nbr[(int64_t)(tap0 + 2) * M + i] = r2;
+        }
         if (compact) {
           compact[(int64_t)(tap0 / 3) * M + i] = r0 >= 0 ? r0 : (r1 >= 0 ? r1 : r2);
           cmask |= ((r0 >= 0 ? 1u : 0u) | (r1 >= 0 ? 2u : 0u) | (r2 >= 0 ? 4u : 0u)) << tap0;
@@ -719,7 +721,7 @@
 
 int tl_rulebook_subm(const int32_t* coords, int64_t M, const uint64_t* bitmap, const uint32_t* prefix, const int32_t dims[4],
                      int32_t* nbr, int32_t* compact, tl_stream_t stream) {
-  if (!coords || !bitmap || !prefix || !dims || !nbr || M <= 0) return TL_ERR_ARG;
+  if (!coords || !bitmap || !prefix || !dims || (!nbr && !compact) || M <= 0) return TL_ERR_ARG;
   k_rulebook_subm<<<tl_grid(M, kBlock), kBlock, 0, tl_s(stream)>>>(coords, M, bitmap, prefix, tl_dims(dims), nbr, compact);
   TL_CHECK_LAUNCH();
   return TL_OK;
@@ -815,8 +817,8 @@
   if (!lv || num_levels < 1 || num_levels > kPyrMaxLevels) return TL_ERR_ARG;
   for (int l = 0; l < num_levels; ++l) {
     if (!lv[l].bitmap || !lv[l].prefix || lv[l].n <= 0) return TL_ERR_ARG;
-    if ((!lv[l].coords || !lv[l].nbr) && !lv[l].o2n) return TL_ERR_ARG;
-    if (lv[l].nbr && !lv[l].coords) return TL_ERR_ARG;
+    if ((!lv[l].coords || (!lv[l].nbr && !lv[l].compact)) && !lv[l].o2n) return TL_ERR_ARG;
+    if ((lv[l].nbr || lv[l].compact) && !lv[l].coords) return TL_ERR_ARG;
     if (l > 0 && !lv[l].coords) return TL_ERR_ARG;
     if (l + 1 < num_levels && (!lv[l].child || (!lv[l].inv && !lv[l].inv_packed))) return TL_ERR_ARG;
     if (lv[l].inv_packed && lv[l].n >= (1ll << 28)) return TL_ERR_ARG;
@@ -838,7 +840,7 @@
   for (int l = 0; l < small; ++l) {
     const TlDims d = tl_dims(lv[l].dims);
     if (lv[l].coords) k_expand_coords<<<tl_grid(tl_nwords(d), kBlock), kBlock, 0, s>>>(lv[l].bitmap, lv[l].prefix, d, lv[l].coords);
-    if (lv[l].nbr) k_rulebook_subm<<<tl_grid(lv[l].n, kBlock), kBlock, 0, s>>>(lv[l].coords, lv[l].n, lv[l].bitmap, lv[l].prefix, d, lv[l].nbr, lv[l].compact);
+    if (lv[l].nbr || lv[l].compact) k_rulebook_subm<<<tl_grid(lv[l].n, kBlock), kBlock, 0, s>>>(lv[l].coords, lv[l].n, lv[l].bitmap, lv[l].prefix, d, lv[l].nbr, lv[l].compact);
   }
   LevelPack p;
   p.nl = num_levels - small;
diff --git a/treelearn_amd/model/engine.py b/treelearn_amd/model/engine.py
--- a/treelearn_amd/model/engine.py
+++ b/treelearn_amd/model/engine.py
@@ -146,13 +146,23 @@
         ok_dtype = self.dtype != torch.float32 or (self.x3 and os.environ.get("TL_BLK_X3", "1") != "0")
         return ok_dtype and self.unet.C == 32 and os.environ.get("TL_BLK", "1") != "0"
 
+    def _ones_route(self, voxel_feats, lv, in_views):
+        dev, C = voxel_feats.device, voxel_feats.shape[1]
+        row = lambda c: torch.empty((1, c), dtype=self.dtype, device=dev).expand(lv.n, -1)
+        extra = [(row(self.w_in.shape[1]), v.scale, v.shift, v.relu) for v in in_views[1:]]
+        route = ops.conv_route(row(C), self.w_in, lv.nbr, lv.n, out=row(self.w_in.shape[1]), out2=extra[0] if extra else None, all_ones=True)
+        return route.startswith("k_conv_ones27<")
+
     def run(self, voxel_feats, geom: TileGeometry, want_backbone=True, all_ones=False):
         lv = geom.levels[0]
-        vf = voxel_feats.to(self.dtype).contiguous()
         ones = all_ones and (os.environ.get("TL_NO_ONES_TABLE") != "1" or (geom.blocked and lv.nbr_ref is None))
         staged = (geom.blocked and self.unet.deeper and self.unet.C == 32 and self.unet.tail[0].w1_halves is not None
                   and os.environ.get("TL_BLK_PRO", "1") != "0")
         in_views = [RAW()] if staged else [RAW(), ACT(self.unet.blocks[0].bn0)]
+        if ones and self._ones_route(voxel_feats, lv, in_views):
+            vf = torch.ones((1, voxel_feats.shape[1]), dtype=self.dtype, device=voxel_feats.device).expand(lv.n, -1)
+        else:
+            vf = voxel_feats.to(self.dtype).contiguous()
         if geom.blocked and not ones:
             if lv.nbr_ref is None:
                 raise RuntimeError("a blocked geometry needs ref_table=True when the input features are not all ones")
diff --git a/treelearn_amd/ops.py b/treelearn_amd/ops.py
--- a/treelearn_amd/ops.py
+++ b/treelearn_amd/ops.py
@@ -145,6 +145,14 @@
     return buf.value.decode()
 
 
+def conv_reads_table(*args, **kwargs) -> bool:
+    a = _conv_args(*args, **kwargs)[0]
+    rc = _hip.lib().tl_conv_reads_table(ctypes.byref(a))
+    if rc < 0:
+        _hip.check(rc, "tl_conv_reads_table")
+    return bool(rc)
+
+
 def conv_fwd(x: torch.Tensor, w_packed: torch.Tensor, table, n_out: int, out: torch.Tensor = None,
              in_scale=None, in_shift=None, in_relu=False, residual=None, out_scale=None, out_shift=None, out_relu=False,
              out2=None, out3=None, one_hot=False, epi=None, all_ones=False, split=None, scatter=None):
```
